# microsoft/UniVL

Measured on NVIDIA H100. Metric: video-text samples/sec, higher is better.
Workload: dtype bf16

## Files before the change

include/univl_b200.h:

```cpp
#ifndef UNIVL_B200_H_
#define UNIVL_B200_H_

#ifdef __cplusplus
extern "C" {
#endif

const char* univl_last_error_string(void);
int univl_abi_version(void);
int univl_set_reserved_sms(int n);
int univl_partials_reduce(const float* part, int nparts, long long rows, long long cols, float* dst, long long ld,
                          void* stream);

int univl_gemm_bf16(const void* A, long long lda, int a_mn_major, const void* B, long long ldb, int b_mn_major,
                    int M, int N, int Kc, void* out, long long ldo, int epilogue, const float* bias,
                    const void* aux_in, long long ld_aux_in, void* aux_out, long long ld_aux_out, float alpha,
                    int block_n, int split_k, void* stream);
int univl_gemm_plan(int M, int N, int Kc, int epilogue, int block_n, int split_k);

int univl_quantize_e4m3_rows(const void* x, long long ldx, void* q, long long ldq, float* scale, int M, int K,
                             void* stream);
int univl_quantize_e4m3_blocks(const float* w, long long ldw, void* q, long long ldq, float* scale, int N, int K,
                               void* stream);
int univl_gemm_fp8(const void* A, long long lda, const float* a_scale, const void* B, long long ldb,
                   const float* b_scale, int M, int N, int Kc, int epilogue, const float* bias, void* out,
                   long long ldo, float* out_scale, void* stream);

int univl_layernorm_fwd(const void* x, const void* res, const float* gamma, const float* beta, void* y, float* mean,
                        float* rstd, int rows, int cols, float eps, float p_drop, int drop_mode,
                        const unsigned long long* rng_state, unsigned long long stream_id, void* stream);
int univl_layernorm_bwd(const void* dy, const void* dy2, const void* x, const void* res, const float* gamma,
                        const float* mean, const float* rstd, void* dx_res, void* dx_dense, float* dgamma,
                        float* dbeta, float* dbias, int rows, int cols, float p_drop, int drop_mode,
                        const unsigned long long* rng_state, unsigned long long stream_id, void* stream);
int univl_layernorm_f32_fwd(const float* x, const float* gamma, const float* beta, void* y, float* mean, float* rstd,
                            int rows, int cols, float eps, void* stream);
int univl_layernorm_f32_bwd(const void* dy, const float* x, const float* gamma, const float* mean, const float* rstd,
                            float* dgamma, float* dbeta, int rows, int cols, void* stream);

int univl_embed_text_fwd(const long long* ids, const long long* type_ids, const float* word, const float* pos,
                         const float* type, const float* gamma, const float* beta, void* y, float* mean, float* rstd,
                         int n_seq, int S, int H, int vocab, float eps, float p_drop, const unsigned long long* rng_state,
                         unsigned long long stream_id, void* stream);
int univl_embed_text_bwd(const void* dy, const long long* ids, const long long* type_ids, const float* word,
                         const float* pos, const float* type, const float* gamma, const float* mean,
                         const float* rstd, float* dword, float* dpos, float* dtype, float* dgamma, float* dbeta,
                         int n_seq, int S, int H, int vocab, float p_drop, const unsigned long long* rng_state,
                         unsigned long long stream_id, void* stream);
int univl_embed_src_fwd(const void* a, const void* b, const float* pos, const float* type, const float* gamma,
                        const float* beta, void* y, float* mean, float* rstd, int Na, int Wa, int Nb, int Fb,
                        int all_pairs, int H, float eps, float p_drop, const unsigned long long* rng_state,
                        unsigned long long stream_id, void* stream);
int univl_embed_src_bwd(const void* dy, const void* a, const void* b, const float* pos, const float* type,
                        const float* gamma, const float* mean, const float* rstd, void* da, void* db, float* dpos,
                        float* dtype, float* dgamma, float* dbeta, int Na, int Wa, int Nb, int Fb, int all_pairs,
                        int H, float p_drop, const unsigned long long* rng_state, unsigned long long stream_id, void* stream);

int univl_attention_fwd(const void* q, long long ldq, const void* k, long long ldk, const void* v, long long ldv,
                        void* o, long long ldo, float* lse, const long long* mask_a, const long long* mask_b, int Wa,
                        int Fb, int Nb, int all_pairs, int n_seq, int heads, int Sq, int Sk, int causal, float scale,
                        float p_drop, const unsigned long long* rng_state, unsigned long long stream_id, void* stream);
int univl_attention_bwd(const void* q, long long ldq, const void* k, long long ldk, const void* v, long long ldv,
                        const void* o, long long ldo, const float* lse, const void* d_o, long long lddo, void* dq,
                        long long lddq, void* dk, long long lddk, void* dv, long long lddv, const long long* mask_a,
                        const long long* mask_b, int Wa, int Fb, int Nb, int all_pairs, int n_seq, int heads, int Sq,
                        int Sk, int causal, float scale, float p_drop, const unsigned long long* rng_state,
                        unsigned long long stream_id, int rng_layout, float* dbq, float* dbk, float* dbv, void* stream);
int univl_attention_long_fwd(const void* q, long long ldq, const void* k, long long ldk, const void* v, long long ldv,
                             void* o, long long ldo, float* lse, const long long* mask_a, const long long* mask_b,
                             int Wa, int Fb, int Nb, int all_pairs, int n_seq, int heads, int Sq, int Sk, int causal,
                             float scale, float p_drop, const unsigned long long* rng_state,
                             unsigned long long stream_id, void* stream);
int univl_attention_long_bwd(const void* q, long long ldq, const void* k, long long ldk, const void* v, long long ldv,
                             const void* o, long long ldo, const float* lse, const void* d_o, long long lddo, void* dq,
                             long long lddq, void* dk, long long lddk, void* dv, long long lddv,
                             const long long* mask_a, const long long* mask_b, int Wa, int Fb, int Nb, int all_pairs,
                             int n_seq, int heads, int Sq, int Sk, int causal, float scale, float p_drop,
                             const unsigned long long* rng_state, unsigned long long stream_id, int rng_layout,
                             float* dbq, float* dbk, float* dbv, void* stream);
int univl_attention_pair_fwd(const void* qa, long long ldqa, const void* ka, long long ldka, const void* va,
                             long long ldva, const void* qb, long long ldqb, const void* kb, long long ldkb,
                             const void* vb, long long ldvb, void* o, long long ldo, float* lse,
                             const long long* mask_a, const long long* mask_b, int Na, int Wa, int Nb, int Fb,
                             int heads, int Sq, float scale, void* stream);
int univl_fused_qkv_attention_supported(int n_seq, int heads, int S, int H);
int univl_fused_qkv_attention_fwd(const void* x, long long ldx, const void* wqkv, long long ldw, const float* bias,
                                  void* qkv_out, long long ld_qkv, void* o, long long ldo, float* lse,
                                  const long long* mask_a, const long long* mask_b, int Wa, int Fb, int Nb,
                                  int all_pairs, int n_seq, int heads, int S, int causal, float scale, float p_drop,
                                  const unsigned long long* rng_state, unsigned long long stream_id, void* stream);
int univl_fused_attention_bwd(const void* qkv, long long ld_qkv, const void* o, long long ldo, const float* lse,
                              const void* d_o, long long lddo, void* dqkv, long long ld_dqkv, float* dbias,
                              const long long* mask_a, const long long* mask_b, int Wa, int Fb, int Nb, int all_pairs,
                              int n_seq, int heads, int S, int causal, float scale, float p_drop,
                              const unsigned long long* rng_state, unsigned long long stream_id, void* stream);

int univl_colsum_bf16(const void* x, long long ld, float* out, int rows, int cols, void* stream);
int univl_cast_f32_to_bf16(const float* src, void* dst, long long n, void* stream);
int univl_cast_bf16_to_f32(const void* src, float* dst, long long n, void* stream);
int univl_multi_cast_f32_to_bf16(const unsigned long long* device_table, int n_tensors, int blocks_per_tensor,
                                 void* stream);
int univl_fill_f32(float* p, float value, long long n, void* stream);
int univl_rng_advance(unsigned long long* rng_state, void* stream);
int univl_gelu_fwd_bf16(const void* x, void* out, long long n, void* stream);
int univl_gelu_bwd_bf16(const void* dy, const void* pre, void* out, long long n, void* stream);
int univl_tanh_fwd_bf16(const void* x, void* out, long long n, void* stream);
int univl_tanh_bwd_bf16(const void* dy, const void* y, void* out, long long n, void* stream);
int univl_scale_f32(float* dst, const float* src, long long n, const float* gscale, void* stream);

int univl_meanpool_fwd(const void* x, const long long* mask, float* out, float* norm_out, int N, int S, int H,
                       int skip_first, int guard_zero, int l2norm, void* stream);
int univl_meanpool_bwd(const float* dy, const float* y, const float* norm, const long long* mask, void* dx, int N,
                       int S, int H, int skip_first, int guard_zero, int l2norm, void* stream);
int univl_sim_matmul_fwd(const float* t, const float* v, float* sim, int Bt, int Bv, int H, int groups, void* stream);
int univl_sim_matmul_bwd(const float* dsim, const float* t, const float* v, float* dt, float* dv, int Bt, int Bv,
                         int H, int groups, void* stream);
int univl_maxmargin_loss(const float* sim, float* loss, float* dsim, int B, float margin, int n_pair, float w_same,
                         float w_diff, int groups, void* stream);
int univl_crossen_loss(const float* sim, float* loss, float* dsim, int B, int groups, void* stream);
int univl_milnce_loss(const float* sim, float* loss, float* dsim, int batch_size, int n_pair, int groups,
                      void* stream);
int univl_softmax_xent_fwd(const float* logits, long long ld, const long long* labels, const long long* pair_mask,
                           float* lse, float* sum_count, float* loss, int T, int V, int target_mode,
                           long long ignore_index, int groups, void* stream);
int univl_softmax_xent_bwd(const float* logits, long long ld, const long long* labels, const long long* pair_mask,
                           const float* lse, const float* sum_count, const float* gscale, void* dlogits,
                           long long ld_d, int T, int V, int target_mode, long long ignore_index, int groups,
                           void* stream);
int univl_vocab_xent_workspace(int T, int V);
int univl_vocab_xent_fwd(const void* x, long long ldx, const void* w, long long ldw, const float* bias,
                         const long long* labels, float* lse, float* sum_count, float* loss, void* workspace,
                         long long workspace_bytes, int T, int V, int Kc, int groups, void* stream);
int univl_vocab_xent_bwd(const void* x, long long ldx, const void* w, long long ldw, const float* bias,
                         const long long* labels, const float* lse, const float* sum_count, const float* gscale,
                         void* dlogits, long long ld_d, int T, int V, int Kc, int groups, void* stream);
int univl_pooler_sim_fwd(const void* u, const float* w, const float* b, float* out, int N, int H, void* stream);
int univl_pooler_sim_bwd(const void* u, const float* w, const float* dout, void* du, float* dw, float* db, int N,
                         int H, void* stream);

int univl_bert_adam_step(float* p, const float* g, float* m, float* v, void* p_bf16, const void* segs, int n_chunks,
                         int n_tensors, float* scratch, long long* step, float b1, float b2, float eps,
                         float max_grad_norm, float global_clip_norm, float warmup, long long t_total,
                         float grad_scale, void* stream);
int univl_bert_adam_step_bf16grad(float* p, const void* g_bf16, float* m, float* v, void* p_bf16, const void* segs,
                                  int n_chunks, int n_tensors, float* scratch, long long* step, float b1, float b2,
                                  float eps, float max_grad_norm, float global_clip_norm, float warmup,
                                  long long t_total, float grad_scale, void* stream);

#ifdef __cplusplus
}
#endif
#endif
```

univl_b200/csrc/gemm_wgmma.cu:

```cuda
#include "common.cuh"
#include "fp8.cuh"
#include "pipeline.cuh"
#include "tmap.cuh"

#include <stdio.h>
#include <type_traits>

namespace univl {

enum GemmEpilogue : int {
  EPI_BIAS_BF16 = 0,
  EPI_BIAS_GELU_BF16 = 1,
  EPI_GELU_BWD_BF16 = 2,
  EPI_ADD_BF16 = 3,
  EPI_BIAS_F32 = 4,
  EPI_ATOMIC_F32 = 5,
};

struct GemmParams {
  int M, N, Kc;
  int k_blocks_per_split;
  int epilogue;
  float alpha;
  void* out;
  long long ldo;
  const float* bias;
  const bf16* aux_in;
  long long ld_aux_in;
  bf16* aux_out;
  long long ld_aux_out;
  int vec2;
  int vec8;
  float* slots;
  unsigned* arrived;
  int splits;
  int kb_seg;
};

constexpr int BLOCK_M = 128;
constexpr int BLOCK_K = 64;
constexpr int PLAN_SMS = 132;
constexpr int SPLIT_MIN_K = 4096;

template <int BLOCK_N, int STAGES>
struct GemmSmem {
  static constexpr int A_BYTES = BLOCK_M * BLOCK_K * 2;
  static constexpr int B_BYTES = BLOCK_N * BLOCK_K * 2;
  static constexpr int STAGE_BYTES = A_BYTES + B_BYTES;
  static constexpr int BAR_OFFSET = STAGES * STAGE_BYTES;
  static constexpr int TOTAL = BAR_OFFSET + 2 * STAGES * 8;
  static constexpr int DYN_BYTES = TOTAL + 1024;
  static_assert(DYN_BYTES <= 227 * 1024, "shared memory per block");
};

struct WorkItem {
  int m0, n0, kb_begin, num_kb;
};
__device__ __forceinline__ WorkItem decode_work(int w, int m_tiles, int n_tiles, int total_kb, int kb_per, int bn) {
  const int tiles = m_tiles * n_tiles;
  const int split = w / tiles;
  const int rem = w - split * tiles;
  int m_blk, n_blk;
  if (kb_per >= total_kb) {
    m_blk = rem / n_tiles;
    n_blk = rem - m_blk * n_tiles;
  } else {
    n_blk = rem / m_tiles;
    m_blk = rem - n_blk * m_tiles;
  }
  WorkItem it;
  it.m0 = m_blk * BLOCK_M;
  it.n0 = n_blk * bn;
  it.kb_begin = split * kb_per;
  it.num_kb = min(total_kb, it.kb_begin + kb_per) - it.kb_begin;
  return it;
}

__device__ __forceinline__ void epi_pair(const GemmParams& p, float alpha, int row, int col, float v0, float v1) {
  if (row >= p.M || col >= p.N) return;
  const bool two = col + 1 < p.N;
  const bool vec = two && p.vec2;
  const int epi = p.epilogue;
  v0 *= alpha;
  v1 *= alpha;
  if (p.bias != nullptr && (epi == EPI_BIAS_BF16 || epi == EPI_BIAS_GELU_BF16 || epi == EPI_BIAS_F32)) {
    v0 += __ldg(p.bias + col);
    if (two) v1 += __ldg(p.bias + col + 1);
  }
  if (epi == EPI_ATOMIC_F32 || epi == EPI_BIAS_F32) {
    float* o = reinterpret_cast<float*>(p.out) + (long long)row * p.ldo + col;
    if (epi == EPI_ATOMIC_F32) {
      if (vec) {
        float2 a = *reinterpret_cast<float2*>(o);
        *reinterpret_cast<float2*>(o) = make_float2(a.x + v0, a.y + v1);
      } else {
        o[0] += v0;
        if (two) o[1] += v1;
      }
    } else {
      if (vec) *reinterpret_cast<float2*>(o) = make_float2(v0, v1);
      else {
        o[0] = v0;
        if (two) o[1] = v1;
      }
    }
    return;
  }
  if (epi == EPI_GELU_BWD_BF16 || epi == EPI_ADD_BF16) {
    const bf16* a = p.aux_in + (long long)row * p.ld_aux_in + col;
    float x0, x1 = 0.f;
    if (vec) {
      const float2 f = unpack_bf16x2(*reinterpret_cast<const uint32_t*>(a));
      x0 = f.x;
      x1 = f.y;
    } else {
      x0 = __bfloat162float(a[0]);
      if (two) x1 = __bfloat162float(a[1]);
    }
    if (epi == EPI_GELU_BWD_BF16) {
      v0 *= gelu_erf_grad(x0);
      v1 *= gelu_erf_grad(x1);
    } else {
      v0 += x0;
      v1 += x1;
    }
  }
  if (epi == EPI_BIAS_GELU_BF16) {
    bf16* ao = p.aux_out + (long long)row * p.ld_aux_out + col;
    if (vec) *reinterpret_cast<uint32_t*>(ao) = pack_bf16x2(v0, v1);
    else {
      ao[0] = __float2bfloat16(v0);
      if (two) ao[1] = __float2bfloat16(v1);
    }
    v0 = gelu_erf(v0);
    v1 = gelu_erf(v1);
  }
  bf16* o = reinterpret_cast<bf16*>(p.out) + (long long)row * p.ldo + col;
  if (vec) *reinterpret_cast<uint32_t*>(o) = pack_bf16x2(v0, v1);
  else {
    o[0] = __float2bfloat16(v0);
    if (two) o[1] = __float2bfloat16(v1);
  }
}

constexpr int EPI_CHUNK = 8;

__device__ __forceinline__ uint4 quad_transpose(uint32_t w0, uint32_t w1, uint32_t w2, uint32_t w3, int q) {
  const bool odd = q & 1;
  uint32_t r0 = __shfl_xor_sync(0xffffffffu, odd ? w0 : w1, 1);
  uint32_t r1 = __shfl_xor_sync(0xffffffffu, odd ? w2 : w3, 1);
  if (odd) {
    w0 = r0;
    w2 = r1;
  } else {
    w1 = r0;
    w3 = r1;
  }
  const bool hi = q & 2;
  r0 = __shfl_xor_sync(0xffffffffu, hi ? w0 : w2, 2);
  r1 = __shfl_xor_sync(0xffffffffu, hi ? w1 : w3, 2);
  if (hi) {
    w0 = r0;
    w1 = r1;
  } else {
    w2 = r0;
    w3 = r1;
  }
  return make_uint4(w0, w1, w2, w3);
}

template <int EPI, bool BIAS, int BLOCK_N, bool WIDE = false>
__device__ __forceinline__ void epi_tile(const GemmParams& p, float alpha, int row, int col0,
                                         const float (&acc)[BLOCK_N / 2]) {
  constexpr int GROUPS = BLOCK_N / 8;
  constexpr int CHUNK = WIDE ? 4 : (GROUPS < EPI_CHUNK ? GROUPS : EPI_CHUNK);
  static_assert(CHUNK % 4 == 0, "a chunk holds whole quads of 8-column groups");
  constexpr bool AUX = EPI == EPI_GELU_BWD_BF16 || EPI == EPI_ADD_BF16;
  constexpr bool OUT_F32 = EPI == EPI_BIAS_F32 || EPI == EPI_ATOMIC_F32;
  static_assert(!(WIDE && OUT_F32), "16-byte stores are for the bf16 outputs");
  constexpr bool ACCUM = EPI == EPI_ATOMIC_F32;
  const int q = threadIdx.x & 3;
  const float* bias = p.bias + col0;
  const bf16* ax = p.aux_in + (long long)row * p.ld_aux_in + col0;
  const long long ax8 = 8 * p.ld_aux_in;
  bf16* ao = p.aux_out + (long long)row * p.ld_aux_out + col0;
  const long long ao8 = 8 * p.ld_aux_out;
  const long long o8 = 8 * p.ldo;
  float* of = reinterpret_cast<float*>(p.out) + (long long)row * p.ldo + col0;
  bf16* ob = reinterpret_cast<bf16*>(p.out) + (long long)row * p.ldo + col0;
  float b[2][CHUNK][2];
  uint32_t x[2][CHUNK][2];
  float2 a[2][CHUNK][2];
  auto load = [&](int j0, int s) {
#pragma unroll
    for (int j = 0; j < CHUNK; ++j) {
      const int c = (j0 + j) * 8;
      if constexpr (BIAS) {
        b[s][j][0] = __ldg(bias + c);
        b[s][j][1] = __ldg(bias + c + 1);
      }
#pragma unroll
      for (int h = 0; h < 2; ++h) {
        if constexpr (AUX) x[s][j][h] = *reinterpret_cast<const uint32_t*>(ax + h * ax8 + c);
        if constexpr (ACCUM) a[s][j][h] = *reinterpret_cast<const float2*>(of + h * o8 + c);
      }
    }
  };
  load(0, 0);
#pragma unroll
  for (int j0 = 0; j0 < GROUPS; j0 += CHUNK) {
    const int s = (j0 / CHUNK) & 1;
    if (j0 + CHUNK < GROUPS) load(j0 + CHUNK, s ^ 1);
#pragma unroll
    for (int jq = 0; jq < CHUNK; jq += 4) {
#pragma unroll
      for (int h = 0; h < 2; ++h) {
        uint32_t wo[4], wa[4];
#pragma unroll
        for (int jj = 0; jj < 4; ++jj) {
          const int j = jq + jj;
          const int c = (j0 + j) * 8;
          float v0 = __fmul_rn(acc[4 * (j0 + j) + 2 * h], alpha);
          float v1 = __fmul_rn(acc[4 * (j0 + j) + 2 * h + 1], alpha);
          if constexpr (BIAS) {
            v0 = __fadd_rn(v0, b[s][j][0]);
            v1 = __fadd_rn(v1, b[s][j][1]);
          }
          if constexpr (AUX) {
            const float2 f = unpack_bf16x2(x[s][j][h]);
            if constexpr (EPI == EPI_GELU_BWD_BF16) {
              v0 = __fmul_rn(v0, gelu_erf_grad(f.x));
              v1 = __fmul_rn(v1, gelu_erf_grad(f.y));
            } else {
              v0 = __fadd_rn(v0, f.x);
              v1 = __fadd_rn(v1, f.y);
            }
          }
          if constexpr (OUT_F32) {
            if constexpr (ACCUM) {
              v0 = __fadd_rn(a[s][j][h].x, v0);
              v1 = __fadd_rn(a[s][j][h].y, v1);
            }
            *reinterpret_cast<float2*>(of + h * o8 + c) = make_float2(v0, v1);
          } else {
            if constexpr (EPI == EPI_BIAS_GELU_BF16) {
              const uint32_t w = pack_bf16x2(v0, v1);
              if constexpr (WIDE) wa[jj] = w;
              else *reinterpret_cast<uint32_t*>(ao + h * ao8 + c) = w;
              v0 = gelu_erf(v0);
              v1 = gelu_erf(v1);
            }
            const uint32_t w = pack_bf16x2(v0, v1);
            if constexpr (WIDE) wo[jj] = w;
            else *reinterpret_cast<uint32_t*>(ob + h * o8 + c) = w;
          }
        }
        if constexpr (WIDE) {
          const int c = (j0 + jq) * 8 + 6 * q;
          if constexpr (EPI == EPI_BIAS_GELU_BF16)
            *reinterpret_cast<uint4*>(ao + h * ao8 + c) = quad_transpose(wa[0], wa[1], wa[2], wa[3], q);
          *reinterpret_cast<uint4*>(ob + h * o8 + c) = quad_transpose(wo[0], wo[1], wo[2], wo[3], q);
        }
      }
    }
  }
}

template <int BLOCK_N>
__device__ __forceinline__ void epilogue_block(const GemmParams& p, bool inside, float alpha, int n0, int row,
                                               int col0, const float (&acc)[BLOCK_N / 2]) {
  if (inside) {
    const bool bias = p.bias != nullptr;
    const bool wide = p.vec8;
    switch (p.epilogue) {
      case EPI_BIAS_BF16:
        if (wide) {
          if (bias) epi_tile<EPI_BIAS_BF16, true, BLOCK_N, true>(p, alpha, row, col0, acc);
          else epi_tile<EPI_BIAS_BF16, false, BLOCK_N, true>(p, alpha, row, col0, acc);
        } else {
          if (bias) epi_tile<EPI_BIAS_BF16, true, BLOCK_N>(p, alpha, row, col0, acc);
          else epi_tile<EPI_BIAS_BF16, false, BLOCK_N>(p, alpha, row, col0, acc);
        }
        break;
      case EPI_BIAS_GELU_BF16:
        if (wide) {
          if (bias) epi_tile<EPI_BIAS_GELU_BF16, true, BLOCK_N, true>(p, alpha, row, col0, acc);
          else epi_tile<EPI_BIAS_GELU_BF16, false, BLOCK_N, true>(p, alpha, row, col0, acc);
        } else {
          if (bias) epi_tile<EPI_BIAS_GELU_BF16, true, BLOCK_N>(p, alpha, row, col0, acc);
          else epi_tile<EPI_BIAS_GELU_BF16, false, BLOCK_N>(p, alpha, row, col0, acc);
        }
        break;
      case EPI_GELU_BWD_BF16:
        if (wide) epi_tile<EPI_GELU_BWD_BF16, false, BLOCK_N, true>(p, alpha, row, col0, acc);
        else epi_tile<EPI_GELU_BWD_BF16, false, BLOCK_N>(p, alpha, row, col0, acc);
        break;
      case EPI_ADD_BF16:
        if (wide) epi_tile<EPI_ADD_BF16, false, BLOCK_N, true>(p, alpha, row, col0, acc);
        else epi_tile<EPI_ADD_BF16, false, BLOCK_N>(p, alpha, row, col0, acc);
        break;
      case EPI_BIAS_F32:
        if (bias) epi_tile<EPI_BIAS_F32, true, BLOCK_N>(p, alpha, row, col0, acc);
        else epi_tile<EPI_BIAS_F32, false, BLOCK_N>(p, alpha, row, col0, acc);
        break;
      default:
        epi_tile<EPI_ATOMIC_F32, false, BLOCK_N>(p, alpha, row, col0, acc);
    }
  } else {
#pragma unroll
    for (int j = 0; j < BLOCK_N / 8; ++j) {
      if (n0 + j * 8 >= p.N) break;
      epi_pair(p, alpha, row, col0 + j * 8, acc[4 * j], acc[4 * j + 1]);
      epi_pair(p, alpha, row + 8, col0 + j * 8, acc[4 * j + 2], acc[4 * j + 3]);
    }
  }
}

__device__ __forceinline__ bool tile_inside(const GemmParams& p, const WorkItem& wi, int bn) {
  return p.vec2 && wi.m0 + BLOCK_M <= p.M && wi.n0 + bn <= p.N;
}

template <int BLOCK_N>
__device__ __forceinline__ bool splitk_fixup(const GemmParams& p, int tile, int half, int split, float alpha,
                                             float (&acc)[BLOCK_N / 2]) {
  constexpr int V = BLOCK_N / 8;
  constexpr int CHUNK = BLOCK_N == 256 ? 4 : 8;
  const int t = threadIdx.x & 127;
  const int lane = t & 31;
  const long long slot = 64LL * BLOCK_N;
  float4* base = reinterpret_cast<float4*>(p.slots + ((long long)tile * p.splits * 2 + half) * slot) + t;
  float4* mine = base + split * (2 * slot / 4);
#pragma unroll
  for (int j = 0; j < V; ++j) {
#pragma unroll
    for (int e = 0; e < 4; ++e) acc[4 * j + e] = __fmul_rn(acc[4 * j + e], alpha);
    __stcg(mine + j * 128, make_float4(acc[4 * j], acc[4 * j + 1], acc[4 * j + 2], acc[4 * j + 3]));
  }
  fence_acq_rel_gpu();
  __syncwarp();
  unsigned before = 0;
  if (lane == 0) before = atom_add_acq_rel_gpu(p.arrived + (tile * 2 + half) * 4 + (t >> 5), 1u);
  before = __shfl_sync(0xffffffffu, before, 0);
  if (before != (unsigned)p.splits - 1) return false;
  fence_acq_rel_gpu();
#pragma unroll
  for (int j0 = 0; j0 < V; j0 += CHUNK) {
    float4 s4[CHUNK];
#pragma unroll
    for (int j = 0; j < CHUNK; ++j) s4[j] = make_float4(0.f, 0.f, 0.f, 0.f);
    for (int s = 0; s < p.splits; ++s) {
      float4 v[CHUNK];
      if (s == split) {
#pragma unroll
        for (int j = 0; j < CHUNK; ++j) {
          const int a = 4 * (j0 + j);
          v[j] = make_float4(acc[a], acc[a + 1], acc[a + 2], acc[a + 3]);
        }
      } else {
        const float4* src = base + s * (2 * slot / 4);
#pragma unroll
        for (int j = 0; j < CHUNK; ++j) v[j] = __ldcg(src + (j0 + j) * 128);
      }
#pragma unroll
      for (int j = 0; j < CHUNK; ++j) {
        s4[j].x = __fadd_rn(s4[j].x, v[j].x);
        s4[j].y = __fadd_rn(s4[j].y, v[j].y);
        s4[j].z = __fadd_rn(s4[j].z, v[j].z);
        s4[j].w = __fadd_rn(s4[j].w, v[j].w);
      }
    }
#pragma unroll
    for (int j = 0; j < CHUNK; ++j) {
      const int a = 4 * (j0 + j);
      acc[a] = s4[j].x;
      acc[a + 1] = s4[j].y;
      acc[a + 2] = s4[j].z;
      acc[a + 3] = s4[j].w;
    }
  }
  return true;
}

template <int BLOCK_N>
__device__ __forceinline__ void finish_block(const GemmParams& p, const WorkItem& wi, int n_tiles, int kb_per,
                                             bool inside, float alpha, int half, int row, int col0,
                                             float (&acc)[BLOCK_N / 2]) {
  if (p.slots != nullptr) {
    const int tile = (wi.m0 / BLOCK_M) * n_tiles + wi.n0 / BLOCK_N;
    if (!splitk_fixup<BLOCK_N>(p, tile, half, wi.kb_begin / kb_per, alpha, acc)) return;
    alpha = 1.f;
  }
  epilogue_block<BLOCK_N>(p, inside, alpha, wi.n0, row, col0, acc);
}

constexpr int TURN_BAR = 1;

template <int BLOCK_N, int STAGES, bool A_MN, bool B_MN, int ELEM = 2>
__device__ __forceinline__ void produce_ring(const CUtensorMap* tmap_a, const CUtensorMap* tmap_b, uint8_t* smem,
                                             const Ring<STAGES>& ring, int num_work, int m_tiles, int n_tiles,
                                             int total_kb, int kb_per) {
  using L = GemmSmem<BLOCK_N, STAGES>;
  uint32_t it = 0;
  for (int w = blockIdx.x; w < num_work; w += gridDim.x) {
    const WorkItem wi = decode_work(w, m_tiles, n_tiles, total_kb, kb_per, BLOCK_N);
    for (int i = 0; i < wi.num_kb; ++i, ++it) {
      const int s = ring.acquire(it, L::STAGE_BYTES);
      uint64_t* bar = &ring.full[s];
      uint8_t* sa = smem + s * L::STAGE_BYTES;
      uint8_t* sb = sa + L::A_BYTES;
      const int k_elem = (wi.kb_begin + i) * (128 / ELEM);
      if (!A_MN) {
        tma_load_2d(sa, tmap_a, bar, k_elem, wi.m0);
      } else {
#pragma unroll
        for (int c = 0; c < BLOCK_M / 64; ++c)
          tma_load_2d(sa + c * (BLOCK_K * 128), tmap_a, bar, wi.m0 + c * 64, k_elem);
      }
      if (!B_MN) {
        tma_load_2d(sb, tmap_b, bar, k_elem, wi.n0);
      } else {
#pragma unroll
        for (int c = 0; c < BLOCK_N / 64; ++c)
          tma_load_2d(sb + c * (BLOCK_K * 128), tmap_b, bar, wi.n0 + c * 64, k_elem);
      }
    }
  }
}

template <int BLOCK_N, int STAGES, bool A_MN, bool B_MN>
__global__ void __launch_bounds__(PIPELINE_THREADS, 1)
gemm_wgmma_kernel(const __grid_constant__ CUtensorMap tmap_a, const __grid_constant__ CUtensorMap tmap_b,
                  const GemmParams p, const int num_work) {
  using L = GemmSmem<BLOCK_N, STAGES>;
  constexpr bool PING = BLOCK_N <= 128;
  constexpr bool FOLD = BLOCK_N == 64;
  Ring<STAGES> ring;
  uint8_t* smem = kernel_prologue(ring, L::BAR_OFFSET, PING ? 1 : 2, &tmap_a, &tmap_b);

  const int wg = threadIdx.x >> 7;
  const int m_tiles = (p.M + BLOCK_M - 1) / BLOCK_M;
  const int n_tiles = (p.N + BLOCK_N - 1) / BLOCK_N;
  const int total_kb = (p.Kc + BLOCK_K - 1) / BLOCK_K;
  const int kb_per = p.k_blocks_per_split;

  if (wg == 0) {
    if (producer_regs())
      produce_ring<BLOCK_N, STAGES, A_MN, B_MN>(&tmap_a, &tmap_b, smem, ring, num_work, m_tiles, n_tiles, total_kb,
                                                kb_per);
  } else if constexpr (!PING) {
    consumer_regs();
    const int c = wg - 1;
    const int t = threadIdx.x & 127;
    const int warp = t >> 5, lane = t & 31;
    uint32_t it = 0;
    for (int w = blockIdx.x; w < num_work; w += gridDim.x) {
      const WorkItem wi = decode_work(w, m_tiles, n_tiles, total_kb, kb_per, BLOCK_N);
      float acc[BLOCK_N / 2];
#pragma unroll
      for (int e = 0; e < BLOCK_N / 2; ++e) acc[e] = 0.f;
      const int last = mma_kblocks<BLOCK_N, A_MN, B_MN, L::STAGE_BYTES, L::A_BYTES>(ring, smem, c * (64 * 128), acc,
                                                                                     0, wi.num_kb, it, t == 0);
      mma_drain(ring, last, acc, t == 0);
      const int row = wi.m0 + c * 64 + warp * 16 + (lane >> 2);
      const int col0 = wi.n0 + 2 * (lane & 3);
      finish_block<BLOCK_N>(p, wi, n_tiles, kb_per, tile_inside(p, wi, BLOCK_N), p.alpha, c, row, col0, acc);
    }
  } else {
    consumer_regs();
    const int c = wg - 1;
    const int t = threadIdx.x & 127;
    const int warp = t >> 5, lane = t & 31;
    uint32_t it = 0;
    int j = 0;
    for (int w = blockIdx.x; w < num_work; w += gridDim.x, ++j) {
      const WorkItem wi = decode_work(w, m_tiles, n_tiles, total_kb, kb_per, BLOCK_N);
      if ((j & 1) != c) {
        it += wi.num_kb;
        continue;
      }
      float acc[2][BLOCK_N / 2];
#pragma unroll
      for (int e = 0; e < BLOCK_N / 2; ++e) acc[0][e] = acc[1][e] = 0.f;
      const bool fold = FOLD && p.kb_seg < wi.num_kb;
      const int seg = fold ? p.kb_seg : wi.num_kb;
      float sum[2][FOLD ? BLOCK_N / 2 : 1];
      if constexpr (FOLD) {
#pragma unroll
        for (int e = 0; e < BLOCK_N / 2; ++e) sum[0][e] = sum[1][e] = 0.f;
      }
      if (j > 0) named_bar(TURN_BAR + c, 256);
      for (int i0 = 0; i0 < wi.num_kb; i0 += seg) {
        const int i1 = min(wi.num_kb, i0 + seg);
        const int last =
            mma_kblocks<BLOCK_N, 2, A_MN, B_MN, L::STAGE_BYTES, L::A_BYTES>(ring, smem, 0, acc, i0, i1, it, t == 0);
        if (i1 == wi.num_kb && w + (int)gridDim.x < num_work)
          named_bar_arrive(TURN_BAR + (c ^ 1), 256);
        mma_drain(ring, last, acc, t == 0);
        if constexpr (FOLD) {
          if (fold) {
#pragma unroll
            for (int e = 0; e < BLOCK_N / 2; ++e) {
              sum[0][e] = __fadd_rn(sum[0][e], __fmul_rn(acc[0][e], p.alpha));
              sum[1][e] = __fadd_rn(sum[1][e], __fmul_rn(acc[1][e], p.alpha));
            }
          }
        }
      }
      float alpha = p.alpha;
      if constexpr (FOLD) {
        if (fold) {
#pragma unroll
          for (int e = 0; e < BLOCK_N / 2; ++e) {
            acc[0][e] = sum[0][e];
            acc[1][e] = sum[1][e];
          }
          alpha = 1.f;
        }
      }
      const bool inside = tile_inside(p, wi, BLOCK_N);
      const int row = wi.m0 + warp * 16 + (lane >> 2);
      const int col0 = wi.n0 + 2 * (lane & 3);
      finish_block<BLOCK_N>(p, wi, n_tiles, kb_per, inside, alpha, 0, row, col0, acc[0]);
      finish_block<BLOCK_N>(p, wi, n_tiles, kb_per, inside, alpha, 1, row + 64, col0, acc[1]);
    }
  }
}

template <int BLOCK_N, int STAGES, bool A_MN, bool B_MN>
static int launch_gemm(const CUtensorMap& ta, const CUtensorMap& tb, const GemmParams& p, int splits,
                       cudaStream_t stream) {
  using L = GemmSmem<BLOCK_N, STAGES>;
  auto kern = gemm_wgmma_kernel<BLOCK_N, STAGES, A_MN, B_MN>;
  const char* name = "univl_gemm_bf16";
  if (int rc = persistent_prepare(kern, L::DYN_BYTES, name)) return rc;
  const long long work =
      (long long)((p.M + BLOCK_M - 1) / BLOCK_M) * ((p.N + BLOCK_N - 1) / BLOCK_N) * (long long)splits;
  return persistent_launch(kern, name, work, L::DYN_BYTES, stream, ta, tb, p, (int)work);
}

template <int BLOCK_N, int STAGES>
static int dispatch_major(bool a_mn, bool b_mn, const CUtensorMap& ta, const CUtensorMap& tb, const GemmParams& p,
                          int splits, cudaStream_t stream) {
  if (!a_mn && !b_mn) return launch_gemm<BLOCK_N, STAGES, false, false>(ta, tb, p, splits, stream);
  if (!a_mn && b_mn) return launch_gemm<BLOCK_N, STAGES, false, true>(ta, tb, p, splits, stream);
  if (a_mn && b_mn) return launch_gemm<BLOCK_N, STAGES, true, true>(ta, tb, p, splits, stream);
  return launch_gemm<BLOCK_N, STAGES, true, false>(ta, tb, p, splits, stream);
}

enum Fp8Epilogue : int { FP8_EPI_BIAS_BF16 = 0, FP8_EPI_GELU_E4M3 = 1 };

struct Fp8Params {
  const float* a_scale;
  const float* b_scale;
  uint8_t* out_q;
  float* out_scale;
};

constexpr int FP8_BLOCK_N = 128;
constexpr int FP8_STAGES = 6;

template <int EPI, bool PAIRS>
__global__ void __launch_bounds__(PIPELINE_THREADS, 1)
gemm_fp8_kernel(const __grid_constant__ CUtensorMap tmap_a, const __grid_constant__ CUtensorMap tmap_b,
                const GemmParams p, const Fp8Params f, const int num_work) {
  using L = GemmSmem<FP8_BLOCK_N, FP8_STAGES>;
  Ring<FP8_STAGES> ring;
  uint8_t* smem = kernel_prologue(ring, L::BAR_OFFSET, 2, &tmap_a, &tmap_b);

  const int wg = threadIdx.x >> 7;
  const int m_tiles = (p.M + BLOCK_M - 1) / BLOCK_M;
  const int n_tiles = p.N / FP8_BLOCK_N;
  const int total_kb = p.Kc / 128;

  if (wg == 0) {
    if (producer_regs())
      produce_ring<FP8_BLOCK_N, FP8_STAGES, false, false, 1>(&tmap_a, &tmap_b, smem, ring, num_work, m_tiles, n_tiles,
                                                              total_kb, total_kb);
    return;
  }
  consumer_regs();
  const int c = wg - 1;
  const int t = threadIdx.x & 127;
  const int warp = t >> 5, lane = t & 31;
  const int M = p.M;
  uint32_t it = 0;
  for (int w = blockIdx.x; w < num_work; w += gridDim.x) {
    const WorkItem wi = decode_work(w, m_tiles, n_tiles, total_kb, total_kb, FP8_BLOCK_N);
    const int row = wi.m0 + c * 64 + warp * 16 + (lane >> 2);
    const bool in0 = row < M, in1 = row + 8 < M;
    const float* sa = f.a_scale + row;
    const float* sb = f.b_scale + (long long)(wi.n0 / FP8_BLOCK_N) * total_kb;
    float acc[FP8_BLOCK_N / 2];
#pragma unroll
    for (int e = 0; e < FP8_BLOCK_N / 2; ++e) acc[e] = 0.f;
    auto issue = [&](float (&tmp)[FP8_BLOCK_N / 2], int kb) {
      const int s = ring.wait(it + kb);
      const uint32_t a_s = smem_u32(smem + s * L::STAGE_BYTES) + c * (64 * 128);
      const uint32_t b_s = smem_u32(smem + s * L::STAGE_BYTES) + L::A_BYTES;
      wgmma_fence();
      fence_regs(tmp);
#pragma unroll
      for (int k = 0; k < 4; ++k)
        WgmmaSSE4M3N128::mma(tmp, make_smem_desc_sw128(a_s + k * 32, 16, 1024),
                             make_smem_desc_sw128(b_s + k * 32, 16, 1024), k > 0 ? 1 : 0);
      wgmma_commit();
      fence_regs(tmp);
    };
    auto promote = [&](auto newer, float (&tmp)[FP8_BLOCK_N / 2], int kb) {
      const float bs = __ldg(sb + kb);
      const float s0 = in0 ? __ldg(sa + (long long)kb * M) : 0.f;
      const float s1 = in1 ? __ldg(sa + (long long)kb * M + 8) : 0.f;
      wgmma_wait<decltype(newer)::value>();
      fence_regs(tmp);
      if (t == 0) ring.release(ring.stage(it + kb));
      const float f0 = s0 * bs, f1 = s1 * bs;
#pragma unroll
      for (int j = 0; j < FP8_BLOCK_N / 8; ++j) {
        acc[4 * j] = __fmaf_rn(tmp[4 * j], f0, acc[4 * j]);
        acc[4 * j + 1] = __fmaf_rn(tmp[4 * j + 1], f0, acc[4 * j + 1]);
        acc[4 * j + 2] = __fmaf_rn(tmp[4 * j + 2], f1, acc[4 * j + 2]);
        acc[4 * j + 3] = __fmaf_rn(tmp[4 * j + 3], f1, acc[4 * j + 3]);
      }
    };
    using One = std::integral_constant<int, 1>;
    using None = std::integral_constant<int, 0>;
    float ta[FP8_BLOCK_N / 2];
    if constexpr (PAIRS) {
      float tb[FP8_BLOCK_N / 2];
      issue(ta, 0);
      issue(tb, 1);
      int kb = 0;
      for (; kb + 2 < total_kb; kb += 2) {
        promote(One(), ta, kb);
        issue(ta, kb + 2);
        promote(One(), tb, kb + 1);
        issue(tb, kb + 3);
      }
      promote(One(), ta, kb);
      promote(None(), tb, kb + 1);
    } else {
      for (int kb = 0; kb < total_kb; ++kb) {
        issue(ta, kb);
        promote(None(), ta, kb);
      }
    }
    it += total_kb;
    const int col0 = wi.n0 + 2 * (lane & 3);
    if constexpr (EPI == FP8_EPI_BIAS_BF16) {
      if (tile_inside(p, wi, FP8_BLOCK_N)) {
        if (p.vec8) epi_tile<EPI_BIAS_BF16, true, FP8_BLOCK_N, true>(p, p.alpha, row, col0, acc);
        else epi_tile<EPI_BIAS_BF16, true, FP8_BLOCK_N>(p, p.alpha, row, col0, acc);
      } else {
#pragma unroll
        for (int j = 0; j < FP8_BLOCK_N / 8; ++j) {
          epi_pair(p, p.alpha, row, col0 + j * 8, acc[4 * j], acc[4 * j + 1]);
          epi_pair(p, p.alpha, row + 8, col0 + j * 8, acc[4 * j + 2], acc[4 * j + 3]);
        }
      }
    } else {
      const float* bias = p.bias + col0;
#pragma unroll
      for (int h = 0; h < 2; ++h) {
        float amax = 0.f;
#pragma unroll
        for (int j = 0; j < FP8_BLOCK_N / 8; ++j) {
          const float v0 = gelu_erf(__fadd_rn(acc[4 * j + 2 * h], __ldg(bias + 8 * j)));
          const float v1 = gelu_erf(__fadd_rn(acc[4 * j + 2 * h + 1], __ldg(bias + 8 * j + 1)));
          acc[4 * j + 2 * h] = v0;
          acc[4 * j + 2 * h + 1] = v1;
          amax = fmaxf(amax, fmaxf(fabsf(v0), fabsf(v1)));
        }
        amax = fmaxf(amax, __shfl_xor_sync(0xffffffffu, amax, 1));
        amax = fmaxf(amax, __shfl_xor_sync(0xffffffffu, amax, 2));
        const float sc = e4m3_scale(amax);
        const float inv = e4m3_inv_scale(sc);
        const int r = row + 8 * h;
        if (r < M) {
          uint8_t* q = f.out_q + (long long)r * p.ldo + col0;
#pragma unroll
          for (int j = 0; j < FP8_BLOCK_N / 8; ++j)
            *reinterpret_cast<uint16_t*>(q + 8 * j) =
                e4m3x2(__fmul_rn(acc[4 * j + 2 * h], inv), __fmul_rn(acc[4 * j + 2 * h + 1], inv));
          if ((lane & 3) == 0) f.out_scale[(long long)(wi.n0 / FP8_BLOCK_N) * M + r] = sc;
        }
      }
    }
  }
}

template <int EPI, bool PAIRS>
static int launch_gemm_fp8(const CUtensorMap& ta, const CUtensorMap& tb, const GemmParams& p, const Fp8Params& f,
                           cudaStream_t stream) {
  using L = GemmSmem<FP8_BLOCK_N, FP8_STAGES>;
  auto kern = gemm_fp8_kernel<EPI, PAIRS>;
  const char* name = "univl_gemm_fp8";
  if (int rc = persistent_prepare(kern, L::DYN_BYTES, name)) return rc;
  const long long work = (long long)((p.M + BLOCK_M - 1) / BLOCK_M) * (p.N / FP8_BLOCK_N);
  return persistent_launch(kern, name, work, L::DYN_BYTES, stream, ta, tb, p, f, (int)work);
}

constexpr int VX_BLOCK_N = 128;
constexpr int VX_STAGES = 6;

struct VocabXentParams {
  int T, V, Kc;
  int m_tiles, n_tiles, chunks, chunk_tiles;
  const float* bias;
  const long long* labels;
  float4* part;
  const float* lse;
  const float* count;
  const float* gscale;
  int rows_per_group, groups;
  bf16* dl;
  long long ld_d;
};

template <bool BWD>
__global__ void __launch_bounds__(PIPELINE_THREADS, 1)
vocab_xent_kernel(const __grid_constant__ CUtensorMap tmap_a, const __grid_constant__ CUtensorMap tmap_b,
                  const VocabXentParams p, const int num_work) {
  using L = GemmSmem<VX_BLOCK_N, VX_STAGES>;
  Ring<VX_STAGES> ring;
  uint8_t* smem = kernel_prologue(ring, L::BAR_OFFSET, 2, &tmap_a, &tmap_b);
  const int wg = threadIdx.x >> 7;
  const int total_kb = (p.Kc + BLOCK_K - 1) / BLOCK_K;

  if (wg == 0) {
    if (!producer_regs()) return;
    uint32_t it = 0;
    for (int w = blockIdx.x; w < num_work; w += gridDim.x) {
      const int chunk = w / p.m_tiles;
      const int m0 = (w - chunk * p.m_tiles) * BLOCK_M;
      const int nt1 = min(p.n_tiles, (chunk + 1) * p.chunk_tiles);
      for (int nt = chunk * p.chunk_tiles; nt < nt1; ++nt) {
        for (int kb = 0; kb < total_kb; ++kb, ++it) {
          const int s = ring.acquire(it, L::STAGE_BYTES);
          uint8_t* sa = smem + s * L::STAGE_BYTES;
          tma_load_2d(sa, &tmap_a, &ring.full[s], kb * BLOCK_K, m0);
          tma_load_2d(sa + L::A_BYTES, &tmap_b, &ring.full[s], kb * BLOCK_K, nt * VX_BLOCK_N);
        }
      }
    }
    return;
  }
  consumer_regs();
  const int c = wg - 1;
  const int t = threadIdx.x & 127;
  const int warp = t >> 5, lane = t & 31, q = lane & 3;
  uint32_t it = 0;
  for (int w = blockIdx.x; w < num_work; w += gridDim.x) {
    const int chunk = w / p.m_tiles;
    const int row = (w - chunk * p.m_tiles) * BLOCK_M + c * 64 + warp * 16 + (lane >> 2);
    long long lab[2];
    float m[2], s[2], xt[2], lse[2], g[2];
#pragma unroll
    for (int h = 0; h < 2; ++h) {
      const int r = row + 8 * h;
      lab[h] = r < p.T ? __ldg(p.labels + r) : -1;
      m[h] = -INFINITY;
      s[h] = 0.f;
      xt[h] = 0.f;
      if constexpr (BWD) {
        lse[h] = 0.f;
        g[h] = 0.f;
        if (lab[h] != -1) {
          lse[h] = __ldg(p.lse + r);
          g[h] = ((p.gscale ? __ldg(p.gscale) : 1.f) / (float)p.groups) / __ldg(p.count + r / p.rows_per_group);
        }
      }
    }
    const int nt1 = min(p.n_tiles, (chunk + 1) * p.chunk_tiles);
    for (int nt = chunk * p.chunk_tiles; nt < nt1; ++nt) {
      float acc[VX_BLOCK_N / 2];
#pragma unroll
      for (int e = 0; e < VX_BLOCK_N / 2; ++e) acc[e] = 0.f;
      const int last = mma_kblocks<VX_BLOCK_N, false, false, L::STAGE_BYTES, L::A_BYTES>(ring, smem, c * (64 * 128),
                                                                                          acc, 0, total_kb, it, t == 0);
      mma_drain(ring, last, acc, t == 0);

      const int col0 = nt * VX_BLOCK_N + 2 * q;
#pragma unroll
      for (int j = 0; j < VX_BLOCK_N / 8; ++j) {
#pragma unroll
        for (int e = 0; e < 2; ++e) {
          const int col = col0 + 8 * j + e;
          const float b = (p.bias != nullptr && col < p.V) ? __ldg(p.bias + col) : 0.f;
          acc[4 * j + e] = __fadd_rn(acc[4 * j + e], b);
          acc[4 * j + 2 + e] = __fadd_rn(acc[4 * j + 2 + e], b);
        }
      }
      if constexpr (!BWD) {
#pragma unroll
        for (int h = 0; h < 2; ++h) {
          float tm = -INFINITY;
#pragma unroll
          for (int j = 0; j < VX_BLOCK_N / 8; ++j)
#pragma unroll
            for (int e = 0; e < 2; ++e)
              if (col0 + 8 * j + e < p.V) tm = fmaxf(tm, acc[4 * j + 2 * h + e]);
          if (tm > m[h]) {
            s[h] = s[h] * __expf(m[h] - tm);
            m[h] = tm;
          }
#pragma unroll
          for (int j = 0; j < VX_BLOCK_N / 8; ++j)
#pragma unroll
            for (int e = 0; e < 2; ++e) {
              const int col = col0 + 8 * j + e;
              const float v = acc[4 * j + 2 * h + e];
              if (col < p.V) s[h] += __expf(v - m[h]);
              if (col == lab[h]) xt[h] = v;
            }
        }
      } else {
        const int ncol = min(p.ld_d - (long long)nt * VX_BLOCK_N, (long long)VX_BLOCK_N);
#pragma unroll
        for (int h = 0; h < 2; ++h) {
          const int r = row + 8 * h;
          if (r >= p.T) continue;
          bf16* drow = p.dl + (long long)r * p.ld_d + col0;
          const bool scored = lab[h] != -1;
#pragma unroll
          for (int j = 0; j < VX_BLOCK_N / 8; ++j) {
            if (8 * j + 2 * q >= ncol) break;
            float d[2];
#pragma unroll
            for (int e = 0; e < 2; ++e) {
              const int col = col0 + 8 * j + e;
              d[e] = 0.f;
              if (scored && col < p.V)
                d[e] = (__expf(acc[4 * j + 2 * h + e] - lse[h]) - (col == lab[h] ? 1.f : 0.f)) * g[h];
            }
            *reinterpret_cast<uint32_t*>(drow + 8 * j) = pack_bf16x2(d[0], d[1]);
          }
        }
      }
    }
    if constexpr (!BWD) {
#pragma unroll
      for (int h = 0; h < 2; ++h) {
#pragma unroll
        for (int o = 1; o <= 2; o <<= 1) {
          const float mo = __shfl_xor_sync(0xffffffffu, m[h], o);
          const float so = __shfl_xor_sync(0xffffffffu, s[h], o);
          const float xo = __shfl_xor_sync(0xffffffffu, xt[h], o);
          const float mx = fmaxf(m[h], mo);
          const float a = m[h] == -INFINITY ? 0.f : s[h] * __expf(m[h] - mx);
          const float b = mo == -INFINITY ? 0.f : so * __expf(mo - mx);
          m[h] = mx;
          s[h] = a + b;
          xt[h] += xo;
        }
        const int r = row + 8 * h;
        if (q == 0 && r < p.T) p.part[(long long)r * p.chunks + chunk] = make_float4(m[h], s[h], xt[h], 0.f);
      }
    }
  }
}

__global__ void __launch_bounds__(256)
vocab_xent_rows_kernel(const float4* __restrict__ part, const long long* __restrict__ labels, int T, int V, int chunks,
                       int chunk_cols, float* __restrict__ lse_out, float* __restrict__ nll) {
  const int r = blockIdx.x * blockDim.x + threadIdx.x;
  if (r >= T) return;
  const long long lab = labels[r];
  if (lab == -1) {
    lse_out[r] = 0.f;
    return;
  }
  const float4* pr = part + (long long)r * chunks;
  float4 f = pr[0];
  float m = f.x, s = f.y;
  for (int k = 1; k < chunks; ++k) {
    f = pr[k];
    const float mx = fmaxf(m, f.x);
    s = s * __expf(m - mx) + f.y * __expf(f.x - mx);
    m = mx;
  }
  const float lse = m + __logf(s);
  lse_out[r] = lse;
  nll[r] = (lab >= 0 && lab < V) ? lse - pr[lab / chunk_cols].z : __int_as_float(0x7fc00000);
}

constexpr int VX_GROUP_THREADS = 512;
__global__ void __launch_bounds__(VX_GROUP_THREADS)
vocab_xent_group_kernel(const float* __restrict__ nll, const long long* __restrict__ labels, int rows_per_group,
                        float* __restrict__ sum_count, int groups) {
  __shared__ float red[2][VX_GROUP_THREADS];
  const int grp = blockIdx.x;
  float sum = 0.f, cnt = 0.f;
  for (int i = threadIdx.x; i < rows_per_group; i += VX_GROUP_THREADS) {
    const long long r = (long long)grp * rows_per_group + i;
    if (labels[r] == -1) continue;
    sum += nll[r];
    cnt += 1.f;
  }
  red[0][threadIdx.x] = sum;
  red[1][threadIdx.x] = cnt;
  __syncthreads();
  for (int o = VX_GROUP_THREADS / 2; o > 0; o >>= 1) {
    if (threadIdx.x < o) {
      red[0][threadIdx.x] += red[0][threadIdx.x + o];
      red[1][threadIdx.x] += red[1][threadIdx.x + o];
    }
    __syncthreads();
  }
  if (threadIdx.x == 0) {
    sum_count[grp] = red[0][0];
    sum_count[groups + grp] = red[1][0];
  }
}

__global__ void vocab_xent_mean_kernel(const float* __restrict__ sum_count, int groups, float* __restrict__ out) {
  float acc = sum_count[0] / sum_count[groups];
  for (int g = 1; g < groups; ++g) acc += sum_count[g] / sum_count[groups + g];
  *out = groups > 1 ? acc / (float)groups : acc;
}

template <bool BWD>
static int launch_vocab_xent(const CUtensorMap& ta, const CUtensorMap& tb, const VocabXentParams& p,
                             cudaStream_t stream) {
  const long long work = (long long)p.m_tiles * p.chunks;
  return persistent_launch(vocab_xent_kernel<BWD>, BWD ? "univl_vocab_xent_bwd" : "univl_vocab_xent_fwd", work,
                           GemmSmem<VX_BLOCK_N, VX_STAGES>::DYN_BYTES, stream, ta, tb, p, (int)work);
}

}

using namespace univl;

namespace {
struct GemmPlan {
  int bn, splits, kb_per, kb_seg;
};
int plan_gemm(int M, int N, int Kc, int epilogue, int block_n, int split_k, GemmPlan* plan) {
  const int total_kb = (Kc + BLOCK_K - 1) / BLOCK_K;
  const int m_tiles = (M + BLOCK_M - 1) / BLOCK_M;
  int bn = block_n;
  if (bn == 0) {
    bn = 256;
    if (epilogue != EPI_ATOMIC_F32) {
      const auto tiles = [&](int w) { return (long long)m_tiles * ((N + w - 1) / w); };
      if (tiles(256) < 2 * PLAN_SMS) bn = 128;
      if (tiles(128) < PLAN_SMS) bn = 64;
    }
    if (N <= 64) bn = 64;
    else if (N <= 128 && bn > 128) bn = 128;
  }
  UNIVL_CHECK_ARG(bn == 64 || bn == 128 || bn == 256, "gemm: block_n must be 64/128/256");
  const int n_tiles = (N + bn - 1) / bn;
  int splits = 1;
  if (epilogue == EPI_ATOMIC_F32) {
    splits = split_k;
    if (splits == 0) {
      const long long tiles = (long long)m_tiles * n_tiles;
      splits = (int)((2 * PLAN_SMS + tiles - 1) / tiles);
      if (splits > total_kb / 2) splits = total_kb / 2;
      if (splits < 1) splits = 1;
    }
    if (splits > total_kb) splits = total_kb;
  }
  int kb_per = (total_kb + splits - 1) / splits;
  splits = (total_kb + kb_per - 1) / kb_per;
  int kb_seg = kb_per;
  if (epilogue == EPI_ATOMIC_F32 && block_n == 0 && split_k == 0 && Kc < SPLIT_MIN_K && splits > 1) {
    bn = 64;
    splits = 1;
    kb_per = total_kb;
  }
  plan->bn = bn; plan->splits = splits; plan->kb_per = kb_per; plan->kb_seg = kb_seg;
  return UNIVL_OK;
}

GemmParams gemm_params(int M, int N, int Kc, int kb_per, int epilogue, float alpha, void* out, long long ldo,
                       const float* bias, const void* aux_in, long long ld_aux_in, void* aux_out,
                       long long ld_aux_out) {
  GemmParams p;
  p.M = M; p.N = N; p.Kc = Kc;
  p.k_blocks_per_split = kb_per;
  p.epilogue = epilogue;
  p.alpha = alpha;
  p.out = out; p.ldo = ldo;
  p.bias = bias;
  p.aux_in = reinterpret_cast<const bf16*>(aux_in); p.ld_aux_in = ld_aux_in;
  p.aux_out = reinterpret_cast<bf16*>(aux_out); p.ld_aux_out = ld_aux_out;
  const bool out_f32 = epilogue == EPI_BIAS_F32 || epilogue == EPI_ATOMIC_F32;
  bool vec2 = ((uintptr_t)out % (out_f32 ? 8 : 4)) == 0 && (ldo % 2) == 0;
  if (aux_in != nullptr) vec2 = vec2 && ((uintptr_t)aux_in % 4) == 0 && (ld_aux_in % 2) == 0;
  if (aux_out != nullptr) vec2 = vec2 && ((uintptr_t)aux_out % 4) == 0 && (ld_aux_out % 2) == 0;
  p.vec2 = vec2 ? 1 : 0;
  bool vec8 = !out_f32 && ((uintptr_t)out % 16) == 0 && (ldo % 8) == 0;
  if (aux_out != nullptr) vec8 = vec8 && ((uintptr_t)aux_out % 16) == 0 && (ld_aux_out % 8) == 0;
  p.vec8 = vec8 ? 1 : 0;
  p.slots = nullptr;
  p.arrived = nullptr;
  p.splits = 1;
  p.kb_seg = kb_per;
  return p;
}
}

extern "C" int univl_gemm_plan(int M, int N, int Kc, int epilogue, int block_n, int split_k) {
  GemmPlan plan;
  if (int rc = plan_gemm(M, N, Kc, epilogue, block_n, split_k, &plan)) return rc;
  return 1;
}

extern "C" int univl_gemm_bf16(const void* A, long long lda, int a_mn_major, const void* B, long long ldb,
                               int b_mn_major, int M, int N, int Kc, void* out, long long ldo, int epilogue,
                               const float* bias, const void* aux_in, long long ld_aux_in, void* aux_out,
                               long long ld_aux_out, float alpha, int block_n, int split_k, void* stream_) {
  cudaStream_t stream = reinterpret_cast<cudaStream_t>(stream_);
  UNIVL_CHECK_ARG(M > 0 && N > 0 && Kc > 0, "gemm: empty problem M=%d N=%d K=%d", M, N, Kc);
  UNIVL_CHECK_ARG(A && B && out, "gemm: null operand");
  UNIVL_CHECK_ARG((lda % 8) == 0 && (ldb % 8) == 0, "gemm: lda/ldb must be multiples of 8 elements (got %lld, %lld)",
                  lda, ldb);
  UNIVL_CHECK_ARG(((uintptr_t)A & 15) == 0 && ((uintptr_t)B & 15) == 0, "gemm: operands must be 16-byte aligned");
  UNIVL_CHECK_ARG(epilogue >= 0 && epilogue <= 5, "gemm: unknown epilogue %d", epilogue);
  if (epilogue == EPI_GELU_BWD_BF16 || epilogue == EPI_ADD_BF16)
    UNIVL_CHECK_ARG(aux_in != nullptr, "gemm: epilogue %d needs aux_in", epilogue);
  if (epilogue == EPI_BIAS_GELU_BF16) UNIVL_CHECK_ARG(aux_out != nullptr, "gemm: gelu epilogue needs aux_out");
  UNIVL_CHECK_ARG(split_k >= 0, "gemm: bad split_k");
  if (epilogue != EPI_ATOMIC_F32) UNIVL_CHECK_ARG(split_k <= 1, "gemm: split_k>1 needs the atomic epilogue");

  GemmPlan plan;
  if (int prc = plan_gemm(M, N, Kc, epilogue, block_n, split_k, &plan)) return prc;
  const int bn = plan.bn;

  CUtensorMap ta, tb;
  int rc;
  if (!a_mn_major) rc = make_tmap(&ta, A, M, Kc, lda, BLOCK_M);
  else             rc = make_tmap(&ta, A, Kc, M, lda, BLOCK_K);
  if (rc) return rc;
  if (!b_mn_major) rc = make_tmap(&tb, B, N, Kc, ldb, bn);
  else             rc = make_tmap(&tb, B, Kc, N, ldb, BLOCK_K);
  if (rc) return rc;

  GemmParams p = gemm_params(M, N, Kc, plan.kb_per, epilogue, alpha, out, ldo, bias, aux_in, ld_aux_in, aux_out,
                             ld_aux_out);
  p.splits = plan.splits;
  p.kb_seg = plan.kb_seg;
  if (plan.splits > 1) {
    const long long tiles = (long long)((M + BLOCK_M - 1) / BLOCK_M) * ((N + bn - 1) / bn);
    const size_t slot_bytes = (size_t)tiles * plan.splits * BLOCK_M * bn * sizeof(float);
    const size_t counter_bytes = (size_t)tiles * 8 * sizeof(unsigned);
    if ((rc = scratch_alloc((void**)&p.slots, slot_bytes + counter_bytes, stream))) return rc;
    p.arrived = reinterpret_cast<unsigned*>(p.slots + slot_bytes / sizeof(float));
    const cudaError_t e = cudaMemsetAsync(p.arrived, 0, counter_bytes, stream);
    if (e != cudaSuccess) {
      cudaFreeAsync(p.slots, stream);
      return set_error(UNIVL_ERR_CUDA, "gemm split-K counters: %s", cudaGetErrorString(e));
    }
  }

  const bool amn = a_mn_major != 0, bmn = b_mn_major != 0;
  if (bn == 256) rc = dispatch_major<256, 4>(amn, bmn, ta, tb, p, plan.splits, stream);
  else if (bn == 128) rc = dispatch_major<128, 6>(amn, bmn, ta, tb, p, plan.splits, stream);
  else rc = dispatch_major<64, 8>(amn, bmn, ta, tb, p, plan.splits, stream);
  if (p.slots != nullptr) cudaFreeAsync(p.slots, stream);
  return rc;
}

extern "C" int univl_gemm_fp8(const void* A, long long lda, const float* a_scale, const void* B, long long ldb,
                              const float* b_scale, int M, int N, int Kc, int epilogue, const float* bias, void* out,
                              long long ldo, float* out_scale, void* stream_) {
  cudaStream_t stream = reinterpret_cast<cudaStream_t>(stream_);
  UNIVL_CHECK_ARG(M > 0 && N > 0 && Kc > 0, "univl_gemm_fp8: empty problem M=%d N=%d K=%d", M, N, Kc);
  UNIVL_CHECK_ARG(Kc % 128 == 0, "univl_gemm_fp8: K=%d must be a multiple of 128 (one scale per 128 columns)", Kc);
  UNIVL_CHECK_ARG(N % 128 == 0, "univl_gemm_fp8: N=%d must be a multiple of 128 (one scale per 128 x 128 block)", N);
  UNIVL_CHECK_ARG(epilogue == FP8_EPI_BIAS_BF16 || epilogue == FP8_EPI_GELU_E4M3,
                  "univl_gemm_fp8: unknown epilogue %d", epilogue);
  UNIVL_CHECK_ARG(A && B && a_scale && b_scale && bias && out, "univl_gemm_fp8: null operand, scale, bias or output");
  UNIVL_CHECK_ARG(lda >= Kc && ldb >= Kc && (lda % 16) == 0 && (ldb % 16) == 0,
                  "univl_gemm_fp8: lda/ldb must be >= K and multiples of 16 (got %lld, %lld, K=%d)", lda, ldb, Kc);
  UNIVL_CHECK_ARG(((uintptr_t)A & 15) == 0 && ((uintptr_t)B & 15) == 0,
                  "univl_gemm_fp8: A and B must be 16-byte aligned");
  UNIVL_CHECK_ARG(ldo >= N, "univl_gemm_fp8: ldo=%lld must be >= N=%d", ldo, N);
  if (epilogue == FP8_EPI_GELU_E4M3) {
    UNIVL_CHECK_ARG(out_scale != nullptr, "univl_gemm_fp8: the GELU epilogue needs out_scale");
    UNIVL_CHECK_ARG(((uintptr_t)out & 15) == 0 && (ldo % 16) == 0,
                    "univl_gemm_fp8: the e4m3 output must be 16-byte aligned with ldo a multiple of 16 (got %lld)",
                    ldo);
  }

  CUtensorMap ta, tb;
  int rc;
  if ((rc = make_tmap(&ta, A, M, Kc, lda, BLOCK_M, true))) return rc;
  if ((rc = make_tmap(&tb, B, N, Kc, ldb, FP8_BLOCK_N, true))) return rc;

  const GemmParams p = gemm_params(M, N, Kc, Kc / 128, EPI_BIAS_BF16, 1.f, out, ldo, bias, nullptr, 0, nullptr, 0);
  Fp8Params f;
  f.a_scale = a_scale;
  f.b_scale = b_scale;
  f.out_q = reinterpret_cast<uint8_t*>(out);
  f.out_scale = out_scale;
  const bool pairs = (Kc / 128) % 2 == 0;
  if (epilogue == FP8_EPI_BIAS_BF16)
    return pairs ? launch_gemm_fp8<FP8_EPI_BIAS_BF16, true>(ta, tb, p, f, stream)
                 : launch_gemm_fp8<FP8_EPI_BIAS_BF16, false>(ta, tb, p, f, stream);
  return pairs ? launch_gemm_fp8<FP8_EPI_GELU_E4M3, true>(ta, tb, p, f, stream)
               : launch_gemm_fp8<FP8_EPI_GELU_E4M3, false>(ta, tb, p, f, stream);
}

namespace {
constexpr int VX_MIN_CHUNK_TILES = 8;
struct VxPlan {
  int m_tiles, n_tiles, chunks, chunk_tiles;
};
VxPlan vx_plan(int T, int V) {
  VxPlan pl;
  pl.m_tiles = (T + BLOCK_M - 1) / BLOCK_M;
  pl.n_tiles = (V + VX_BLOCK_N - 1) / VX_BLOCK_N;
  long long best = -1;
  for (int c = 1; c <= pl.n_tiles; ++c) {
    const int ct = (pl.n_tiles + c - 1) / c;
    if (ct < VX_MIN_CHUNK_TILES && c > 1) break;
    if (c > 1 && ct == (pl.n_tiles + c - 2) / (c - 1)) continue;
    const int chunks = (pl.n_tiles + ct - 1) / ct;
    const long long rounds = ((long long)pl.m_tiles * chunks + PLAN_SMS - 1) / PLAN_SMS;
    if (best < 0 || rounds * ct < best) {
      best = rounds * ct;
      pl.chunks = chunks;
      pl.chunk_tiles = ct;
    }
  }
  return pl;
}

int vx_check(const char* name, const void* x, long long ldx, const void* w, long long ldw, const long long* labels,
             int T, int V, int Kc, int groups) {
  UNIVL_CHECK_ARG(T > 0 && V > 0 && Kc > 0, "%s: empty problem T=%d V=%d K=%d", name, T, V, Kc);
  UNIVL_CHECK_ARG(x && w && labels, "%s: null x, W or labels", name);
  UNIVL_CHECK_ARG(ldx >= Kc && ldw >= Kc && (ldx % 8) == 0 && (ldw % 8) == 0,
                  "%s: ldx/ldw must be >= K and multiples of 8 (got %lld, %lld, K=%d)", name, ldx, ldw, Kc);
  UNIVL_CHECK_ARG(((uintptr_t)x & 15) == 0 && ((uintptr_t)w & 15) == 0, "%s: x and W must be 16-byte aligned", name);
  UNIVL_CHECK_ARG(groups > 0 && T % groups == 0, "%s: %d groups must divide T=%d", name, groups, T);
  return UNIVL_OK;
}

template <bool BWD>
int vx_params(const void* x, long long ldx, const void* w, long long ldw, int T, int V, int Kc, CUtensorMap* ta,
              CUtensorMap* tb, VocabXentParams* p) {
  if (int rc = persistent_prepare(vocab_xent_kernel<BWD>, GemmSmem<VX_BLOCK_N, VX_STAGES>::DYN_BYTES,
                                  BWD ? "univl_vocab_xent_bwd" : "univl_vocab_xent_fwd"))
    return rc;
  const VxPlan pl = vx_plan(T, V);
  int rc;
  if ((rc = make_tmap(ta, x, T, Kc, ldx, BLOCK_M))) return rc;
  if ((rc = make_tmap(tb, w, V, Kc, ldw, VX_BLOCK_N))) return rc;
  *p = VocabXentParams{};
  p->T = T; p->V = V; p->Kc = Kc;
  p->m_tiles = pl.m_tiles; p->n_tiles = pl.n_tiles; p->chunks = pl.chunks; p->chunk_tiles = pl.chunk_tiles;
  return UNIVL_OK;
}


long long vx_workspace_bytes(int T, int V) {
  return (long long)T * vx_plan(T, V).chunks * (long long)sizeof(float4) + ((long long)T * 4 + 15) / 16 * 16;
}
}

extern "C" int univl_vocab_xent_workspace(int T, int V) {
  UNIVL_CHECK_ARG(T > 0 && V > 0, "univl_vocab_xent_workspace: empty problem T=%d V=%d", T, V);
  const long long bytes = vx_workspace_bytes(T, V);
  UNIVL_CHECK_ARG(bytes <= 0x7fffffffLL, "univl_vocab_xent_workspace: T=%d V=%d needs over 2 GiB", T, V);
  return (int)bytes;
}

extern "C" int univl_vocab_xent_fwd(const void* x, long long ldx, const void* w, long long ldw, const float* bias,
                                    const long long* labels, float* lse, float* sum_count, float* loss,
                                    void* workspace, long long workspace_bytes, int T, int V, int Kc, int groups,
                                    void* stream_) {
  const char* name = "univl_vocab_xent_fwd";
  if (int rc = vx_check(name, x, ldx, w, ldw, labels, T, V, Kc, groups)) return rc;
  UNIVL_CHECK_ARG(lse && sum_count && loss && workspace, "%s: null lse, sum_count, loss or workspace", name);
  UNIVL_CHECK_ARG(((uintptr_t)workspace & 15) == 0, "%s: the workspace must be 16-byte aligned", name);
  const long long need = vx_workspace_bytes(T, V);
  UNIVL_CHECK_ARG(workspace_bytes >= need, "%s: workspace of %lld bytes, needs %lld (univl_vocab_xent_workspace)",
                  name, workspace_bytes, need);
  cudaStream_t stream = reinterpret_cast<cudaStream_t>(stream_);
  CUtensorMap ta, tb;
  VocabXentParams p;
  if (int rc = vx_params<false>(x, ldx, w, ldw, T, V, Kc, &ta, &tb, &p)) return rc;
  p.bias = bias;
  p.labels = labels;
  p.part = reinterpret_cast<float4*>(workspace);
  if (int rc = launch_vocab_xent<false>(ta, tb, p, stream)) return rc;
  float* nll = reinterpret_cast<float*>(p.part + (long long)T * p.chunks);
  vocab_xent_rows_kernel<<<(T + 255) / 256, 256, 0, stream>>>(p.part, labels, T, V, p.chunks,
                                                               p.chunk_tiles * VX_BLOCK_N, lse, nll);
  vocab_xent_group_kernel<<<groups, VX_GROUP_THREADS, 0, stream>>>(nll, labels, T / groups, sum_count, groups);
  vocab_xent_mean_kernel<<<1, 1, 0, stream>>>(sum_count, groups, loss);
  UNIVL_CHECK_LAUNCH(name);
  return UNIVL_OK;
}

extern "C" int univl_vocab_xent_bwd(const void* x, long long ldx, const void* w, long long ldw, const float* bias,
                                    const long long* labels, const float* lse, const float* sum_count,
                                    const float* gscale, void* dlogits, long long ld_d, int T, int V, int Kc,
                                    int groups, void* stream_) {
  const char* name = "univl_vocab_xent_bwd";
  if (int rc = vx_check(name, x, ldx, w, ldw, labels, T, V, Kc, groups)) return rc;
  UNIVL_CHECK_ARG(lse && sum_count && dlogits, "%s: null lse, sum_count or dlogits", name);
  const long long cols = (long long)vx_plan(T, V).n_tiles * VX_BLOCK_N;
  UNIVL_CHECK_ARG(ld_d >= V && ld_d <= cols && (ld_d % 2) == 0 && ((uintptr_t)dlogits & 3) == 0,
                  "%s: ld_d=%lld must be even, >= V=%d and <= V rounded up to 128, with dlogits 4-byte aligned", name,
                  ld_d, V);
  cudaStream_t stream = reinterpret_cast<cudaStream_t>(stream_);
  CUtensorMap ta, tb;
  VocabXentParams p;
  if (int rc = vx_params<true>(x, ldx, w, ldw, T, V, Kc, &ta, &tb, &p)) return rc;
  p.bias = bias;
  p.labels = labels;
  p.lse = lse;
  p.count = sum_count + groups;
  p.gscale = gscale;
  p.rows_per_group = T / groups;
  p.groups = groups;
  p.dl = reinterpret_cast<bf16*>(dlogits);
  p.ld_d = ld_d;
  return launch_vocab_xent<true>(ta, tb, p, stream);
}
```

univl_b200/csrc/layernorm.cu:

```cuda
#include "common.cuh"

namespace univl {

constexpr int LN_WARPS = 8;
constexpr int LN_MAX_VEC = 4;

__device__ __forceinline__ void load8(const bf16* p, float (&v)[8]) {
  const uint4 u = *reinterpret_cast<const uint4*>(p);
  const uint32_t w[4] = {u.x, u.y, u.z, u.w};
#pragma unroll
  for (int j = 0; j < 4; ++j) {
    const float2 f = unpack_bf16x2(w[j]);
    v[2 * j] = f.x;
    v[2 * j + 1] = f.y;
  }
}
__device__ __forceinline__ void load8(const float* p, float (&v)[8]) {
  const float4 a = *reinterpret_cast<const float4*>(p);
  const float4 b = *reinterpret_cast<const float4*>(p + 4);
  v[0] = a.x; v[1] = a.y; v[2] = a.z; v[3] = a.w;
  v[4] = b.x; v[5] = b.y; v[6] = b.z; v[7] = b.w;
}
template <typename T> struct Raw8;
template <> struct Raw8<bf16> { uint4 u; };
template <> struct Raw8<float> { float4 a, b; };
__device__ __forceinline__ void raw_load(const bf16* p, Raw8<bf16>& r) {
  asm volatile("ld.global.nc.L1::no_allocate.v4.u32 {%0, %1, %2, %3}, [%4];"
               : "=r"(r.u.x), "=r"(r.u.y), "=r"(r.u.z), "=r"(r.u.w) : "l"(p));
}
__device__ __forceinline__ void raw_load(const float* p, Raw8<float>& r) {
  r.a = __ldg(reinterpret_cast<const float4*>(p));
  r.b = __ldg(reinterpret_cast<const float4*>(p + 4));
}
__device__ __forceinline__ void raw_unpack(const Raw8<bf16>& r, float (&v)[8]) {
  const uint32_t w[4] = {r.u.x, r.u.y, r.u.z, r.u.w};
#pragma unroll
  for (int j = 0; j < 4; ++j) {
    const float2 f = unpack_bf16x2(w[j]);
    v[2 * j] = f.x;
    v[2 * j + 1] = f.y;
  }
}
__device__ __forceinline__ void raw_unpack(const Raw8<float>& r, float (&v)[8]) {
  v[0] = r.a.x; v[1] = r.a.y; v[2] = r.a.z; v[3] = r.a.w;
  v[4] = r.b.x; v[5] = r.b.y; v[6] = r.b.z; v[7] = r.b.w;
}
__device__ __forceinline__ void store8(bf16* p, const float (&v)[8]) {
  uint4 u;
  u.x = pack_bf16x2(v[0], v[1]);
  u.y = pack_bf16x2(v[2], v[3]);
  u.z = pack_bf16x2(v[4], v[5]);
  u.w = pack_bf16x2(v[6], v[7]);
  *reinterpret_cast<uint4*>(p) = u;
}

struct DropCfg {
  int mode;
  uint32_t threshold;
  float scale;
  uint64_t seed, stream;
  const unsigned long long* rng;
};
__device__ __forceinline__ DropCfg resolve_drop(DropCfg d) {
  if (d.mode != 0 && d.rng != nullptr) {
    d.seed = d.rng[0];
    d.stream += d.rng[1] << 20;
  }
  return d;
}

__device__ __forceinline__ uint32_t keep8_mask(const DropCfg& d, uint64_t idx0) {
  return dropout_keep8(d.seed, d.stream, idx0, d.threshold);
}

template <typename TIn, int NVEC>
__global__ void __launch_bounds__(LN_WARPS * 32, NVEC <= 3 ? 3 : 2)
layernorm_fwd_kernel(const TIn* __restrict__ x, const bf16* __restrict__ res, const float* __restrict__ gamma,
                     const float* __restrict__ beta, bf16* __restrict__ y, float* __restrict__ mean_out,
                     float* __restrict__ rstd_out, int rows, float eps, DropCfg drop_in) {
  pdl_trigger();
  pdl_wait();
  const DropCfg drop = resolve_drop(drop_in);
  constexpr int cols = NVEC * 256;
  const int warp = threadIdx.x >> 5, lane = threadIdx.x & 31;
  const float inv_cols = 1.0f / (float)cols;
  const long long stride = (long long)gridDim.x * LN_WARPS;
  long long row = (long long)blockIdx.x * LN_WARPS + warp;
  Raw8<TIn> nx[NVEC];
  Raw8<bf16> nr[NVEC];
  if (row < rows) {
#pragma unroll
    for (int i = 0; i < NVEC; ++i) {
      const long long off = row * cols + (i * 32 + lane) * 8;
      raw_load(x + off, nx[i]);
      if (res != nullptr) raw_load(res + off, nr[i]);
    }
  }
  for (; row < rows; row += stride) {
    float z[NVEC][8];
    float s = 0.f;
#pragma unroll
    for (int i = 0; i < NVEC; ++i) {
      const int c = (i * 32 + lane) * 8;
      raw_unpack(nx[i], z[i]);
      if (drop.mode == 1) {
        const uint32_t keep = keep8_mask(drop, (uint64_t)row * cols + c);
#pragma unroll
        for (int j = 0; j < 8; ++j) z[i][j] = ((keep >> j) & 1u) ? z[i][j] * drop.scale : 0.f;
      }
      if (res != nullptr) {
        float r[8];
        raw_unpack(nr[i], r);
#pragma unroll
        for (int j = 0; j < 8; ++j) z[i][j] += r[j];
      }
#pragma unroll
      for (int j = 0; j < 8; ++j) s += z[i][j];
    }
    const long long next = row + stride;
    if (next < rows) {
#pragma unroll
      for (int i = 0; i < NVEC; ++i) {
        const long long off = next * cols + (i * 32 + lane) * 8;
        raw_load(x + off, nx[i]);
        if (res != nullptr) raw_load(res + off, nr[i]);
      }
    }
    const float mean = warp_sum(s) * inv_cols;
    float q = 0.f;
#pragma unroll
    for (int i = 0; i < NVEC; ++i)
#pragma unroll
      for (int j = 0; j < 8; ++j) {
        const float d = z[i][j] - mean;
        q += d * d;
      }
    const float var = warp_sum(q) * inv_cols;
    const float rstd = 1.0f / sqrtf(var + eps);
    if (lane == 0) {
      if (mean_out) mean_out[row] = mean;
      if (rstd_out) rstd_out[row] = rstd;
    }
#pragma unroll
    for (int i = 0; i < NVEC; ++i) {
      const int c = (i * 32 + lane) * 8;
      float g[8], b[8], o[8];
      load8(gamma + c, g);
      load8(beta + c, b);
#pragma unroll
      for (int j = 0; j < 8; ++j) o[j] = g[j] * ((z[i][j] - mean) * rstd) + b[j];
      if (drop.mode == 2) {
        const uint32_t keep = keep8_mask(drop, (uint64_t)row * cols + c);
#pragma unroll
        for (int j = 0; j < 8; ++j) o[j] = ((keep >> j) & 1u) ? o[j] * drop.scale : 0.f;
      }
      store8(y + row * cols + c, o);
    }
  }
}

template <typename TIn>
static void launch_ln_fwd(int grid, cudaStream_t st, const TIn* x, const bf16* res, const float* gamma,
                          const float* beta, bf16* y, float* mean, float* rstd, int rows, int cols, float eps,
                          DropCfg drop) {
  const dim3 g(grid), b(LN_WARPS * 32);
  switch (cols >> 8) {
    case 1: launch_kernel(layernorm_fwd_kernel<TIn, 1>, g, b, 0, st, x, res, gamma, beta, y, mean, rstd, rows, eps, drop); break;
    case 2: launch_kernel(layernorm_fwd_kernel<TIn, 2>, g, b, 0, st, x, res, gamma, beta, y, mean, rstd, rows, eps, drop); break;
    case 3: launch_kernel(layernorm_fwd_kernel<TIn, 3>, g, b, 0, st, x, res, gamma, beta, y, mean, rstd, rows, eps, drop); break;
    default: launch_kernel(layernorm_fwd_kernel<TIn, 4>, g, b, 0, st, x, res, gamma, beta, y, mean, rstd, rows, eps, drop); break;
  }
}


template <typename TIn>
__device__ __forceinline__ void ln_bwd_load(const bf16* dy, const bf16* dy2, const TIn* x, const bf16* res,
                                            long long off, const DropCfg& drop, float (&z)[8], float (&d)[8],
                                            uint32_t& keep) {
  load8(x + off, z);
  keep = 0xffu;
  if (drop.mode != 0) keep = keep8_mask(drop, (uint64_t)off);
  if (drop.mode == 1) {
#pragma unroll
    for (int j = 0; j < 8; ++j) z[j] = ((keep >> j) & 1u) ? z[j] * drop.scale : 0.f;
  }
  if (res != nullptr) {
    float r[8];
    load8(res + off, r);
#pragma unroll
    for (int j = 0; j < 8; ++j) z[j] += r[j];
  }
  load8(dy + off, d);
  if (dy2 != nullptr) {
    float d2[8];
    load8(dy2 + off, d2);
#pragma unroll
    for (int j = 0; j < 8; ++j) d[j] += d2[j];
  }
  if (drop.mode == 2) {
#pragma unroll
    for (int j = 0; j < 8; ++j) d[j] = ((keep >> j) & 1u) ? d[j] * drop.scale : 0.f;
  }
}

constexpr int LNB_WARPS = 4;
__device__ __forceinline__ void acc8_add(float* p, const float (&v)[8]) {
  float4 a = *reinterpret_cast<float4*>(p), b = *reinterpret_cast<float4*>(p + 4);
  a.x += v[0]; a.y += v[1]; a.z += v[2]; a.w += v[3];
  b.x += v[4]; b.y += v[5]; b.z += v[6]; b.w += v[7];
  *reinterpret_cast<float4*>(p) = a;
  *reinterpret_cast<float4*>(p + 4) = b;
}
template <typename TIn, int NVEC>
__global__ void __launch_bounds__(LNB_WARPS * 32, NVEC <= 3 ? 5 : 3)
layernorm_bwd_kernel(const bf16* __restrict__ dy, const bf16* __restrict__ dy2, const TIn* __restrict__ x,
                     const bf16* __restrict__ res, const float* __restrict__ gamma, const float* __restrict__ mean_in,
                     const float* __restrict__ rstd_in, bf16* __restrict__ dx_res, bf16* __restrict__ dx_dense,
                     float* __restrict__ dgamma, float* __restrict__ dbeta, float* __restrict__ dbias, int rows,
                     DropCfg drop_in) {
  pdl_trigger();
  pdl_wait();
  const DropCfg drop = resolve_drop(drop_in);
  extern __shared__ __align__(16) float lnb_acc[];
  constexpr int cols = NVEC * 256;
  const int warp = threadIdx.x >> 5, lane = threadIdx.x & 31;
  const float inv_cols = 1.0f / (float)cols;
  const bool emit = dx_res != nullptr || dx_dense != nullptr || dbias != nullptr;
  float* my = lnb_acc + warp * 3 * cols;
  for (int k = lane * 4; k < 3 * cols; k += 128) *reinterpret_cast<float4*>(my + k) = make_float4(0.f, 0.f, 0.f, 0.f);
  __syncwarp();

  for (long long row = (long long)blockIdx.x * LNB_WARPS + warp; row < rows; row += (long long)gridDim.x * LNB_WARPS) {
    const float mean = mean_in[row], rstd = rstd_in[row];
    const float nm = -mean * rstd;
    float xh[NVEC][8], g[NVEC][8];
    uint32_t keep[NVEC];
    float s1 = 0.f, s2 = 0.f;
#pragma unroll
    for (int i = 0; i < NVEC; ++i) {
      const int c = (i * 32 + lane) * 8;
      float d[8], gm[8], dh[8];
      ln_bwd_load(dy, dy2, x, res, row * cols + c, drop, xh[i], d, keep[i]);
      load8(gamma + c, gm);
#pragma unroll
      for (int j = 0; j < 8; ++j) {
        const float h = fmaf(xh[i][j], rstd, nm);
        const float gg = d[j] * gm[j];
        s1 += gg;
        s2 = fmaf(gg, h, s2);
        dh[j] = d[j] * h;
        xh[i][j] = h;
        g[i][j] = gg;
      }
      acc8_add(my + c, dh);
      acc8_add(my + cols + c, d);
    }
    if (!emit) continue;
    s1 = warp_sum(s1);
    s2 = warp_sum(s2);
    const float a = -s1 * inv_cols * rstd, b = -s2 * inv_cols * rstd;
#pragma unroll
    for (int i = 0; i < NVEC; ++i) {
      const int c = (i * 32 + lane) * 8;
      float dz[8], dd[8];
#pragma unroll
      for (int j = 0; j < 8; ++j) {
        dz[j] = fmaf(xh[i][j], b, fmaf(g[i][j], rstd, a));
        dd[j] = (drop.mode == 1) ? (((keep[i] >> j) & 1u) ? dz[j] * drop.scale : 0.f) : dz[j];
      }
      if (dbias != nullptr) acc8_add(my + 2 * cols + c, dd);
      if (dx_res != nullptr) store8(dx_res + row * cols + c, dz);
      if (dx_dense != nullptr && dx_dense != dx_res) store8(dx_dense + row * cols + c, dd);
    }
  }
  __syncthreads();
  for (int which = 0; which < 3; ++which) {
    float* dst = which == 0 ? dgamma : which == 1 ? dbeta : dbias;
    if (dst == nullptr) continue;
    for (int e = threadIdx.x; e < cols; e += LNB_WARPS * 32) {
      float t = 0.f;
#pragma unroll
      for (int w = 0; w < LNB_WARPS; ++w) t += lnb_acc[(w * 3 + which) * cols + e];
      dst[(long long)blockIdx.x * cols + e] = t;
    }
  }
}

template <typename TIn>
static int launch_ln_bwd(int grid, cudaStream_t st, const bf16* dy, const bf16* dy2, const TIn* x, const bf16* res,
                         const float* gamma, const float* mean, const float* rstd, bf16* dx_res, bf16* dx_dense,
                         float* dgamma_out, float* dbeta_out, float* dbias_out, int rows, int cols, DropCfg drop) {
  const size_t smem = (size_t)LNB_WARPS * 3 * cols * sizeof(float);
  float* outs[3] = {dgamma_out, dbeta_out, dbias_out};
  float* parts[3] = {nullptr, nullptr, nullptr};
  for (int w = 0; w < 3; ++w)
    if (outs[w] != nullptr)
      if (int rc = scratch_alloc((void**)&parts[w], (size_t)grid * cols * sizeof(float), st)) return rc;
  float *dgamma = parts[0], *dbeta = parts[1], *dbias = parts[2];
  switch (cols >> 8) {
    case 1: launch_kernel(layernorm_bwd_kernel<TIn, 1>, dim3(grid), dim3(LNB_WARPS * 32), smem, st, dy, dy2, x, res, gamma, mean, rstd, dx_res, dx_dense, dgamma, dbeta, dbias, rows, drop); break;
    case 2: launch_kernel(layernorm_bwd_kernel<TIn, 2>, dim3(grid), dim3(LNB_WARPS * 32), smem, st, dy, dy2, x, res, gamma, mean, rstd, dx_res, dx_dense, dgamma, dbeta, dbias, rows, drop); break;
    case 3: launch_kernel(layernorm_bwd_kernel<TIn, 3>, dim3(grid), dim3(LNB_WARPS * 32), smem, st, dy, dy2, x, res, gamma, mean, rstd, dx_res, dx_dense, dgamma, dbeta, dbias, rows, drop); break;
    default: launch_kernel(layernorm_bwd_kernel<TIn, 4>, dim3(grid), dim3(LNB_WARPS * 32), smem, st, dy, dy2, x, res, gamma, mean, rstd, dx_res, dx_dense, dgamma, dbeta, dbias, rows, drop); break;
  }
  UNIVL_CHECK_LAUNCH("layernorm_bwd");
  for (int w = 0; w < 3; ++w)
    if (parts[w] != nullptr)
      if (int rc = partials_reduce(parts[w], grid, 1, cols, outs[w], cols, st)) return rc;
  return UNIVL_OK;
}

static int check_ln_shape(const char* what, int rows, int cols) {
  UNIVL_CHECK_ARG(rows >= 0 && cols > 0 && (cols % 256) == 0 && cols <= 256 * LN_MAX_VEC,
                  "%s: cols must be a multiple of 256 and <= %d (got rows=%d cols=%d)", what, 256 * LN_MAX_VEC, rows,
                  cols);
  return UNIVL_OK;
}

static DropCfg make_drop(int mode, float p, const unsigned long long* rng, unsigned long long stream) {
  DropCfg d;
  d.mode = (p > 0.f) ? mode : 0;
  d.threshold = dropout_threshold16(p);
  d.scale = (p > 0.f) ? 1.0f / (1.0f - p) : 1.0f;
  d.seed = 0;
  d.stream = stream;
  d.rng = rng;
  return d;
}

static int lnb_grid(int rows) {
  long long blocks = ((long long)rows + LNB_WARPS - 1) / LNB_WARPS;
  const long long cap = (long long)device_sms() * 5;
  return (int)(blocks < 1 ? 1 : (blocks > cap ? cap : blocks));
}
static int ln_grid(int rows) {
  long long blocks = ((long long)rows + LN_WARPS - 1) / LN_WARPS;
  const long long cap = (long long)device_sms() * 8;
  return (int)(blocks < 1 ? 1 : (blocks > cap ? cap : blocks));
}

}

using namespace univl;

extern "C" int univl_layernorm_fwd(const void* x, const void* res, const float* gamma, const float* beta, void* y,
                                   float* mean, float* rstd, int rows, int cols, float eps, float p_drop,
                                   int drop_mode, const unsigned long long* rng_state,
                                   unsigned long long stream_id, void* stream) {
  if (int rc = check_ln_shape("layernorm_fwd", rows, cols)) return rc;
  UNIVL_CHECK_ARG(x && gamma && beta && y, "layernorm_fwd: null pointer");
  UNIVL_CHECK_ARG(p_drop == 0.f || rng_state != nullptr, "layernorm_fwd: dropout needs rng_state");
  UNIVL_CHECK_ARG(p_drop >= 0.f && p_drop < 1.f && drop_mode >= 0 && drop_mode <= 2, "layernorm_fwd: bad dropout");
  if (rows == 0) return UNIVL_OK;
  launch_ln_fwd<bf16>(ln_grid(rows), (cudaStream_t)stream, (const bf16*)x, (const bf16*)res, gamma, beta, (bf16*)y, mean,
                      rstd, rows, cols, eps, make_drop(drop_mode, p_drop, rng_state, stream_id));
  UNIVL_CHECK_LAUNCH("layernorm_fwd");
  return UNIVL_OK;
}

extern "C" int univl_layernorm_bwd(const void* dy, const void* dy2, const void* x, const void* res,
                                   const float* gamma, const float* mean, const float* rstd, void* dx_res,
                                   void* dx_dense, float* dgamma, float* dbeta, float* dbias, int rows, int cols,
                                   float p_drop, int drop_mode, const unsigned long long* rng_state,
                                   unsigned long long stream_id, void* stream) {
  if (int rc = check_ln_shape("layernorm_bwd", rows, cols)) return rc;
  UNIVL_CHECK_ARG(dy && x && gamma && mean && rstd, "layernorm_bwd: null pointer");
  UNIVL_CHECK_ARG(p_drop == 0.f || rng_state != nullptr, "layernorm_bwd: dropout needs rng_state");
  UNIVL_CHECK_ARG(p_drop >= 0.f && p_drop < 1.f && drop_mode >= 0 && drop_mode <= 2, "layernorm_bwd: bad dropout");
  if (rows == 0) return UNIVL_OK;
  return launch_ln_bwd<bf16>(lnb_grid(rows), (cudaStream_t)stream, (const bf16*)dy, (const bf16*)dy2, (const bf16*)x,
                             (const bf16*)res, gamma, mean, rstd, (bf16*)dx_res, (bf16*)dx_dense, dgamma, dbeta, dbias,
                             rows, cols, make_drop(drop_mode, p_drop, rng_state, stream_id));
}

extern "C" int univl_layernorm_f32_fwd(const float* x, const float* gamma, const float* beta, void* y, float* mean,
                                       float* rstd, int rows, int cols, float eps, void* stream) {
  if (int rc = check_ln_shape("layernorm_f32_fwd", rows, cols)) return rc;
  UNIVL_CHECK_ARG(x && gamma && beta && y, "layernorm_f32_fwd: null pointer");
  if (rows == 0) return UNIVL_OK;
  launch_ln_fwd<float>(ln_grid(rows), (cudaStream_t)stream, x, (const bf16*)nullptr, gamma, beta, (bf16*)y, mean, rstd,
                       rows, cols, eps, make_drop(0, 0.f, nullptr, 0));
  UNIVL_CHECK_LAUNCH("layernorm_f32_fwd");
  return UNIVL_OK;
}

extern "C" int univl_layernorm_f32_bwd(const void* dy, const float* x, const float* gamma, const float* mean,
                                       const float* rstd, float* dgamma, float* dbeta, int rows, int cols,
                                       void* stream) {
  if (int rc = check_ln_shape("layernorm_f32_bwd", rows, cols)) return rc;
  UNIVL_CHECK_ARG(dy && x && gamma && mean && rstd && dgamma && dbeta, "layernorm_f32_bwd: null pointer");
  if (rows == 0) return UNIVL_OK;
  return launch_ln_bwd<float>(lnb_grid(rows), (cudaStream_t)stream, (const bf16*)dy, nullptr, x, nullptr, gamma, mean,
                              rstd, nullptr, nullptr, dgamma, dbeta, nullptr, rows, cols, make_drop(0, 0.f, nullptr, 0));
}
```

univl_b200/modules/transformer.py:

```python
import torch
from torch import nn

from .. import ops
from .until_module import LayerNorm


def check_config(config):
    if config.hidden_size != 768 or config.num_attention_heads != 12 or config.intermediate_size % 256 != 0:
        raise ValueError("univl_b200 kernels are specialised for hidden_size 768 / 12 heads of 64 (got %d / %d)"
                         % (config.hidden_size, config.num_attention_heads))
    if config.hidden_size % config.num_attention_heads != 0:
        raise ValueError("The hidden size (%d) is not a multiple of the number of attention heads (%d)"
                         % (config.hidden_size, config.num_attention_heads))
    act = config.hidden_act
    if not (isinstance(act, str) and act == "gelu"):
        raise ValueError("univl_b200 fuses erf-GELU into the FFN GEMM: hidden_act must be 'gelu' (got %r)" % (act,))


class SelfAttentionParams(nn.Module):

    def __init__(self, config):
        super(SelfAttentionParams, self).__init__()
        check_config(config)
        self.num_attention_heads = config.num_attention_heads
        self.attention_head_size = config.hidden_size // config.num_attention_heads
        self.all_head_size = config.hidden_size
        self.query = nn.Linear(config.hidden_size, self.all_head_size)
        self.key = nn.Linear(config.hidden_size, self.all_head_size)
        self.value = nn.Linear(config.hidden_size, self.all_head_size)
        self.dropout = nn.Dropout(config.attention_probs_dropout_prob)

    def _qkv_modules(self):
        return self.query, self.key, self.value


class DenseNormParams(nn.Module):

    def __init__(self, in_features, config):
        super(DenseNormParams, self).__init__()
        self.dense = nn.Linear(in_features, config.hidden_size)
        self.LayerNorm = LayerNorm(config.hidden_size, eps=1e-12)
        self.dropout = nn.Dropout(config.hidden_dropout_prob)


class IntermediateParams(nn.Module):

    def __init__(self, config):
        super(IntermediateParams, self).__init__()
        self.dense = nn.Linear(config.hidden_size, config.intermediate_size)


class AttentionParams(nn.Module):

    def __init__(self, config):
        super(AttentionParams, self).__init__()
        self.self = SelfAttentionParams(config)
        self.output = DenseNormParams(config.hidden_size, config)


def attention_param_list(self_mod, out_mod):
    return (self_mod.query.weight, self_mod.query.bias, self_mod.key.weight, self_mod.key.bias,
            self_mod.value.weight, self_mod.value.bias, out_mod.dense.weight, out_mod.dense.bias,
            out_mod.LayerNorm.weight, out_mod.LayerNorm.bias)


def ffn_param_list(intermediate, output):
    return (intermediate.dense.weight, intermediate.dense.bias, output.dense.weight, output.dense.bias,
            output.LayerNorm.weight, output.LayerNorm.bias)


class EncoderLayer(nn.Module):

    def __init__(self, config):
        super(EncoderLayer, self).__init__()
        self.attention = AttentionParams(config)
        self.intermediate = IntermediateParams(config)
        self.output = DenseNormParams(config.intermediate_size, config)
        self.p_hidden = config.hidden_dropout_prob
        self.p_attn = config.attention_probs_dropout_prob

    def run(self, x2d, n_seq, S, mask):
        params = attention_param_list(self.attention.self, self.attention.output) + \
            ffn_param_list(self.intermediate, self.output)
        return ops.EncoderLayerFn.apply(x2d, n_seq, S, mask, self.attention.output.dropout.p,
                                        self.attention.self.dropout.p, self.training, *params)


def _layer_params(layer):
    return attention_param_list(layer.attention.self, layer.attention.output) + \
        ffn_param_list(layer.intermediate, layer.output)


class EncoderStack(nn.Module):

    def __init__(self, config):
        super(EncoderStack, self).__init__()
        self.layer = nn.ModuleList([EncoderLayer(config) for _ in range(config.num_hidden_layers)])

    def run(self, x2d, n_seq, S, mask, keep_all=False):
        outs = []
        cuts = self.__dict__.get("_cut_layers")
        for i, layer in enumerate(self.layer):
            if cuts and i in cuts and x2d.requires_grad:
                leaf = x2d.detach().requires_grad_(True)
                self.__dict__.setdefault("_cut_pairs", []).append((i, x2d, leaf))
                x2d = leaf
            x2d = layer.run(x2d, n_seq, S, mask)
            if keep_all:
                outs.append(x2d)
        return outs if keep_all else x2d

    def run_first_token(self, x2d, n_seq, S, mask, start=0):
        for layer in self.layer[start:-1]:
            x2d = layer.run(x2d, n_seq, S, mask)
        last = self.layer[-1]
        return ops.EncoderLayerClsFn.apply(x2d, n_seq, S, mask, last.attention.output.dropout.p,
                                           last.attention.self.dropout.p, last.training, *_layer_params(last))


class Pooler(nn.Module):

    def __init__(self, config):
        super(Pooler, self).__init__()
        self.dense = nn.Linear(config.hidden_size, config.hidden_size)
        self.activation = nn.Tanh()

    def pre_activation(self, h2d, n_seq, S):
        first = h2d.view(n_seq, S, -1)[:, 0]
        return ops.LinearFn.apply(first, self.dense.weight, self.dense.bias, False, True)

    def run(self, h2d, n_seq, S):
        return ops.TanhFn.apply(self.pre_activation(h2d, n_seq, S))


class HeadTransform(nn.Module):

    def __init__(self, config):
        super(HeadTransform, self).__init__()
        self.dense = nn.Linear(config.hidden_size, config.hidden_size)
        self.LayerNorm = LayerNorm(config.hidden_size, eps=1e-12)

    def run(self, x2d):
        t = ops.LinearFn.apply(x2d, self.dense.weight, self.dense.bias, True, True)
        return ops.LayerNormFn.apply(t, self.LayerNorm.weight, self.LayerNorm.bias)


def as_rows(t3d):
    n, s, h = t3d.shape
    return t3d.to(torch.bfloat16).contiguous().view(n * s, h)


def hidden_list(outs, n_seq, S):
    return [o.view(n_seq, S, -1) for o in outs]
```

univl_b200/ops.py:

```python
import math
import os

import torch

from . import lib
from . import runtime as rt
from .runtime import call, ptr

BF16 = torch.bfloat16
F32 = torch.float32
LN_EPS = 1e-12
HEADS = 12
LD_VOCAB_ALIGN = 64

EPI_BIAS, EPI_GELU, EPI_GELU_BWD, EPI_ADD, EPI_F32, EPI_ATOMIC = 0, 1, 2, 3, 4, 5


def _empty(shape, dtype, like):
    return torch.empty(shape, dtype=dtype, device=like.device)


def _zeros(shape, dtype, like):
    return torch.zeros(shape, dtype=dtype, device=like.device)


def _check2d(t, name):
    if t.dim() != 2 or t.stride(1) != 1:
        raise RuntimeError("univl_b200: %s must be a row-major 2-D tensor (got shape %s strides %s)"
                           % (name, tuple(t.shape), t.stride()))


class GradSink:

    def __init__(self):
        self.flat = rt.current_sink()

    def one(self, param):
        if param is None:
            return None, None
        if self.flat is not None and self.flat.has(param):
            return self.flat.grad_view(param), None
        t = torch.zeros(param.shape, dtype=F32, device=param.device)
        return t, t

    def packed(self, params):
        if self.flat is not None and all(self.flat.has(p) for p in params):
            v = self.flat.grad_view_packed(params)
            if v is not None:
                return v, [None] * len(params)
        rows = sum(p.shape[0] for p in params)
        t = torch.zeros((rows,) + tuple(params[0].shape[1:]), dtype=F32, device=params[0].device)
        outs, r = [], 0
        for p in params:
            outs.append(t[r:r + p.shape[0]])
            r += p.shape[0]
        return t, outs


def gemm(a, b, M, N, K, out, epi=EPI_BIAS, bias=None, aux_in=None, aux_out=None, a_mn=False, b_mn=False, alpha=1.0,
         block_n=0, split_k=0):
    _check2d(a, "gemm A"); _check2d(b, "gemm B"); _check2d(out, "gemm out")
    call("univl_gemm_bf16", a.data_ptr(), a.stride(0), int(a_mn), b.data_ptr(), b.stride(0), int(b_mn), M, N, K,
         out.data_ptr(), out.stride(0), epi, ptr(bias), ptr(aux_in), aux_in.stride(0) if aux_in is not None else 0,
         ptr(aux_out), aux_out.stride(0) if aux_out is not None else 0, float(alpha), block_n, split_k)
    return out


def linear_fwd(x, w16, bias, epi=EPI_BIAS, aux_out=None, out_dtype=BF16, ld_out=None):
    T, K = x.shape
    N = w16.shape[0]
    if ld_out is None:
        out = _empty((T, N), out_dtype, x)
    else:
        out = _empty((T, ld_out), out_dtype, x)[:, :N]
    return gemm(x, w16, T, N, K, out, epi=epi, bias=bias, aux_out=aux_out)


def linear_dgrad(dy, w16, epi=EPI_BIAS, aux_in=None):
    T, N = dy.shape
    K = w16.shape[1]
    out = _empty((T, K), BF16, dy)
    return gemm(dy, w16, T, K, N, out, epi=epi, aux_in=aux_in, b_mn=True)


def linear_wgrad(dy, x, dw=None):
    T, N = dy.shape
    K = x.shape[1]
    if dw is None:
        dw = _zeros((N, K), F32, dy)
    return gemm(dy, x, N, K, T, dw, epi=EPI_ATOMIC, a_mn=True, b_mn=True)


def colsum(x, out=None):
    rows, cols = x.shape
    if out is None:
        out = _zeros((cols,), F32, x)
    call("univl_colsum_bf16", x.data_ptr(), x.stride(0), out.data_ptr(), rows, cols)
    return out


def layernorm_fwd(x, res, gamma, beta, p=0.0, mode=0, seed=0, stream=0):
    rows, cols = x.shape
    y = _empty((rows, cols), BF16, x)
    mean = _empty((rows,), F32, x)
    rstd = _empty((rows,), F32, x)
    call("univl_layernorm_fwd", x.data_ptr(), ptr(res), gamma.data_ptr(), beta.data_ptr(), y.data_ptr(),
         mean.data_ptr(), rstd.data_ptr(), rows, cols, LN_EPS, float(p), mode, seed, stream)
    return y, mean, rstd


def layernorm_bwd(dy, dy2, x, res, gamma, mean, rstd, p=0.0, mode=0, seed=0, stream=0, want_dbias=True,
                  want_dx=True, dgamma=None, dbeta=None, dbias=None):
    rows, cols = x.shape
    dx_res = _empty((rows, cols), BF16, x) if want_dx else None
    dx_dense = _empty((rows, cols), BF16, x) if (want_dx and p > 0.0 and mode == 1) else dx_res
    dgamma = _zeros((cols,), F32, x) if dgamma is None else dgamma
    dbeta = _zeros((cols,), F32, x) if dbeta is None else dbeta
    if dbias is None and want_dbias:
        dbias = _zeros((cols,), F32, x)
    call("univl_layernorm_bwd", dy.data_ptr(), ptr(dy2), x.data_ptr(), ptr(res), gamma.data_ptr(), mean.data_ptr(),
         rstd.data_ptr(), ptr(dx_res), ptr(dx_dense), dgamma.data_ptr(), dbeta.data_ptr(), ptr(dbias), rows, cols,
         float(p), mode, seed, stream)
    return dx_res, dx_dense, dgamma, dbeta, dbias


class MaskSpec:

    def __init__(self, mask_a=None, mask_b=None, all_pairs=False, causal=False):
        self.a = mask_a.contiguous() if mask_a is not None else None
        self.b = mask_b.contiguous() if mask_b is not None else None
        self.all_pairs = int(all_pairs)
        self.causal = bool(causal)
        for m in (self.a, self.b):
            if m is not None and m.dtype != torch.int64:
                raise RuntimeError("univl_b200: masks must be int64 (as the reference dataloaders emit them)")

    @property
    def Wa(self):
        return self.a.shape[1] if self.a is not None else 0

    @property
    def Fb(self):
        return self.b.shape[1] if self.b is not None else 0

    @property
    def Nb(self):
        return self.b.shape[0] if self.b is not None else 0


SHORT_ATTN_MAX_S = 256


def _attention_entry(kind, Sq, Sk):
    if Sq > SHORT_ATTN_MAX_S or Sk > SHORT_ATTN_MAX_S:
        return "univl_attention_long_" + kind
    return "univl_attention_" + kind


def attention_fwd(q, k, v, n_seq, Sq, Sk, mask, p=0.0, seed=0, stream=0):
    o = _empty((n_seq * Sq, HEADS * 64), BF16, q)
    lse = _empty((n_seq * HEADS * Sq,), F32, q)
    call(_attention_entry("fwd", Sq, Sk), q.data_ptr(), q.stride(0), k.data_ptr(), k.stride(0), v.data_ptr(),
         v.stride(0), o.data_ptr(), o.stride(0), lse.data_ptr(), ptr(mask.a), ptr(mask.b), mask.Wa, mask.Fb, mask.Nb,
         int(mask.all_pairs), n_seq, HEADS, Sq, Sk, int(mask.causal), 1.0 / math.sqrt(64.0), float(p), seed, stream)
    return o, lse


def fused_attention_supported(n_seq, S, H):
    if os.environ.get("UNIVL_FUSED_ATTN", "1") == "0":
        return False
    from . import lib
    return bool(lib.load().univl_fused_qkv_attention_supported(int(n_seq), HEADS, int(S), int(H)))


def fused_qkv_attention_fwd(x, wqkv, bqkv, n_seq, S, mask, p=0.0, seed=0, stream=0, save_qkv=True):
    T, H = x.shape
    _check2d(x, "fused attention x"); _check2d(wqkv, "fused attention wqkv")
    o = _empty((T, H), BF16, x)
    lse = _empty((n_seq * HEADS * S,), F32, x)
    qkv = _empty((T, 3 * H), BF16, x) if save_qkv else None
    call("univl_fused_qkv_attention_fwd", x.data_ptr(), x.stride(0), wqkv.data_ptr(), wqkv.stride(0), bqkv.data_ptr(),
         ptr(qkv), 3 * H, o.data_ptr(), o.stride(0), lse.data_ptr(), ptr(mask.a), ptr(mask.b), mask.Wa, mask.Fb,
         mask.Nb, int(mask.all_pairs), n_seq, HEADS, S, int(mask.causal), 1.0 / math.sqrt(64.0), float(p), seed, stream)
    return o, lse, qkv


def fused_attention_bwd(qkv, o, lse, d_o, dqkv, n_seq, S, mask, p=0.0, seed=0, stream=0, dbias=None):
    call("univl_fused_attention_bwd", qkv.data_ptr(), qkv.stride(0), o.data_ptr(), o.stride(0), lse.data_ptr(),
         d_o.data_ptr(), d_o.stride(0), dqkv.data_ptr(), dqkv.stride(0), ptr(dbias), ptr(mask.a), ptr(mask.b), mask.Wa,
         mask.Fb, mask.Nb, int(mask.all_pairs), n_seq, HEADS, S, int(mask.causal), 1.0 / math.sqrt(64.0), float(p), seed,
         stream)


def attention_bwd(q, k, v, o, lse, d_o, dq, dk, dv, n_seq, Sq, Sk, mask, p=0.0, seed=0, stream=0, dbias=None,
                  rng_layout=0):
    dbq, dbk, dbv = dbias if dbias is not None else (None, None, None)
    entry = _attention_entry("bwd", Sq, Sk)
    assert rng_layout == 0 or entry == "univl_attention_bwd", (rng_layout, Sq, Sk)
    call(entry, q.data_ptr(), q.stride(0), k.data_ptr(), k.stride(0), v.data_ptr(), v.stride(0),
         o.data_ptr(), o.stride(0), lse.data_ptr(), d_o.data_ptr(), d_o.stride(0), dq.data_ptr(), dq.stride(0),
         dk.data_ptr(), dk.stride(0), dv.data_ptr(), dv.stride(0), ptr(mask.a), ptr(mask.b), mask.Wa, mask.Fb,
         mask.Nb, int(mask.all_pairs), n_seq, HEADS, Sq, Sk, int(mask.causal), 1.0 / math.sqrt(64.0), float(p), seed,
         stream, int(rng_layout), ptr(dbq), ptr(dbk), ptr(dbv))


def attention_pair_fwd(qkv_a, qkv_b, Na, Nb, Sq, mask):
    H = HEADS * 64
    o = _empty((Na * Nb * Sq, H), BF16, qkv_a)
    call("univl_attention_pair_fwd", qkv_a.data_ptr(), qkv_a.stride(0), qkv_a[:, H:].data_ptr(), qkv_a.stride(0),
         qkv_a[:, 2 * H:].data_ptr(), qkv_a.stride(0), qkv_b.data_ptr(), qkv_b.stride(0), qkv_b[:, H:].data_ptr(),
         qkv_b.stride(0), qkv_b[:, 2 * H:].data_ptr(), qkv_b.stride(0), o.data_ptr(), o.stride(0), None, ptr(mask.a),
         ptr(mask.b), Na, mask.Wa, Nb, mask.Fb, HEADS, Sq, 1.0 / math.sqrt(64.0))
    return o


def embed_src_rows_eval(a, N, W, pos, type_w, gamma, beta, out):
    mean = _empty((N * W,), F32, a)
    rstd = _empty((N * W,), F32, a)
    call("univl_embed_src_fwd", a.data_ptr(), None, pos.data_ptr(), type_w.data_ptr(), gamma.data_ptr(),
         beta.data_ptr(), out.data_ptr(), mean.data_ptr(), rstd.data_ptr(), N, W, 0, 0, 0, a.shape[1], LN_EPS, 0.0,
         None, 0)
    return out


def pair_layer_eval(x, qkv_a, qkv_b, Na, Nb, S, mask, params, first_token):
    arena = rt.current()
    wa = dict(zip(ATT_KEYS, params[:10]))
    wf = dict(zip(FFN_KEYS, params[10:16]))
    drop = _Drop(0.0, 0.0, False)
    n_seq = Na * Nb
    ctx = attention_pair_fwd(qkv_a, qkv_b, Na, Nb, 1 if first_token else S, mask)
    xq = x.view(n_seq, S, -1)[:, 0].contiguous() if first_token else x
    ao = linear_fwd(ctx, arena.bf16(wa["o"]), wa["bo"])
    y, _, _ = layernorm_fwd(ao, xq, wa["gamma"], wa["beta"], 0.0, 1, drop.seed, drop.stream())
    return ffn_block_fwd(y, wf, drop)[0]


E4M3 = torch.float8_e4m3fn
FP8_EPI_BIAS, FP8_EPI_GELU = 0, 1


def quantize_e4m3_rows(x):
    _check2d(x, "quantize_e4m3_rows x")
    M, K = x.shape
    q = _empty((M, K), E4M3, x)
    s = _empty((K // 128, M), F32, x)
    call("univl_quantize_e4m3_rows", x.data_ptr(), x.stride(0), q.data_ptr(), q.stride(0), s.data_ptr(), M, K)
    return q, s


def quantize_e4m3_blocks(w, q=None, s=None):
    _check2d(w, "quantize_e4m3_blocks w")
    N, K = w.shape
    q = _empty((N, K), E4M3, w) if q is None else q
    s = _empty((N // 128, K // 128), F32, w) if s is None else s
    call("univl_quantize_e4m3_blocks", w.data_ptr(), w.stride(0), q.data_ptr(), q.stride(0), s.data_ptr(), N, K)
    return q, s


def gemm_fp8(a, a_scale, b, b_scale, bias, gelu=False):
    _check2d(a, "gemm_fp8 A"); _check2d(b, "gemm_fp8 B")
    M, K = a.shape
    N = b.shape[0]
    if gelu:
        out = _empty((M, N), E4M3, a)
        out_s = _empty((N // 128, M), F32, a)
    else:
        out = _empty((M, N), BF16, a)
        out_s = None
    call("univl_gemm_fp8", a.data_ptr(), a.stride(0), a_scale.data_ptr(), b.data_ptr(), b.stride(0),
         b_scale.data_ptr(), M, N, K, FP8_EPI_GELU if gelu else FP8_EPI_BIAS, bias.data_ptr(), out.data_ptr(),
         out.stride(0), ptr(out_s))
    return (out, out_s) if gelu else out


def fp8_layer_weights(params, names):
    wa = dict(zip(ATT_KEYS, params[:10]))
    wf = dict(zip(FFN_KEYS, params[10:16]))
    H = wa["q"].shape[1]

    def stacked(ws):
        q = _empty((len(ws) * H, H), E4M3, ws[0])
        s = _empty((len(ws) * H // 128, H // 128), F32, ws[0])
        for i, w in enumerate(ws):
            quantize_e4m3_blocks(w, q[i * H:(i + 1) * H], s[i * H // 128:(i + 1) * H // 128])
        return q, s

    make = {"qkv": lambda: stacked((wa["q"], wa["k"], wa["v"])), "kv": lambda: stacked((wa["k"], wa["v"])),
            "o": lambda: quantize_e4m3_blocks(wa["o"]), "w1": lambda: quantize_e4m3_blocks(wf["w1"]),
            "w2": lambda: quantize_e4m3_blocks(wf["w2"])}
    return {n: make[n]() for n in names}


def _fp8_layer_tail(ctx, x, params, qw):
    wa = dict(zip(ATT_KEYS, params[:10]))
    wf = dict(zip(FFN_KEYS, params[10:16]))
    drop = _Drop(0.0, 0.0, False)
    ao = gemm_fp8(*quantize_e4m3_rows(ctx), *qw["o"], wa["bo"])
    y, _, _ = layernorm_fwd(ao, x, wa["gamma"], wa["beta"], 0.0, 1, drop.seed, drop.stream())
    h, hs = gemm_fp8(*quantize_e4m3_rows(y), *qw["w1"], wf["b1"], gelu=True)
    fo = gemm_fp8(h, hs, *qw["w2"], wf["b2"])
    out, _, _ = layernorm_fwd(fo, y, wf["gamma"], wf["beta"], 0.0, 1, drop.seed, drop.stream())
    return out


def pair_layer_eval_fp8(x, qkv_a, qkv_b, Na, Nb, S, mask, params, qw):
    ctx = attention_pair_fwd(qkv_a, qkv_b, Na, Nb, S, mask)
    return _fp8_layer_tail(ctx, x, params, qw)


def encoder_layer_eval_fp8(x, n_seq, S, mask, params, qw):
    wa = dict(zip(ATT_KEYS, params[:10]))
    H = x.shape[1]
    qkv = gemm_fp8(*quantize_e4m3_rows(x), *qw["qkv"], rt.packed_bias(wa["bq"], wa["bk"], wa["bv"]))
    drop = _Drop(0.0, 0.0, False)
    ctx, _ = attention_fwd(qkv[:, :H], qkv[:, H:2 * H], qkv[:, 2 * H:], n_seq, S, S, mask, 0.0, drop.seed,
                           drop.stream())
    return _fp8_layer_tail(ctx, x, params, qw)


def cls_layer_eval_fp8(x, n_seq, S, mask, params, qw):
    arena = rt.current()
    wa = dict(zip(ATT_KEYS, params[:10]))
    wf = dict(zip(FFN_KEYS, params[10:16]))
    drop = _Drop(0.0, 0.0, False)
    H = x.shape[1]
    x0 = x.view(n_seq, S, H)[:, 0].contiguous()
    kv = gemm_fp8(*quantize_e4m3_rows(x), *qw["kv"], rt.packed_bias(wa["bk"], wa["bv"]))
    q = linear_fwd(x0, arena.bf16_qkv(wa["q"], wa["k"], wa["v"])[:H], wa["bq"])
    ctx, _ = attention_fwd(q, kv[:, :H], kv[:, H:], n_seq, 1, S, mask, 0.0, drop.seed, drop.stream())
    ao = linear_fwd(ctx, arena.bf16(wa["o"]), wa["bo"])
    y, _, _ = layernorm_fwd(ao, x0, wa["gamma"], wa["beta"], 0.0, 1, drop.seed, drop.stream())
    return ffn_block_fwd(y, wf, drop)[0]


class _Drop:

    def __init__(self, p_hidden, p_attn, training):
        arena = rt.current()
        self.ph = float(p_hidden) if training else 0.0
        self.pa = float(p_attn) if training else 0.0
        self.seed = arena.seed
        self.arena = arena
        self.epoch = arena.epoch_host

    def stream(self):
        return self.arena.next_stream()


def attn_block_fwd(xq, xkv, n_seq, Sq, Sk, mask, w, drop, need_bwd=True):
    arena = rt.current()
    H = xq.shape[1]
    self_attn = xkv is xq
    sv = {"self": self_attn, "fused": False}
    wqkv = arena.bf16_qkv(w["q"], w["k"], w["v"])
    ctx = None
    if self_attn and fused_attention_supported(n_seq, Sq, H):
        sa, sd = drop.stream(), drop.stream()
        ctx, lse, qkv = fused_qkv_attention_fwd(xq, wqkv, rt.packed_bias(w["bq"], w["bk"], w["bv"]), n_seq, Sq, mask,
                                                drop.pa, drop.seed, sa, save_qkv=need_bwd)
        sv["qkv"] = qkv
        sv["fused"] = True
    elif self_attn:
        qkv = linear_fwd(xq, wqkv, rt.packed_bias(w["bq"], w["bk"], w["bv"]))
        q, k, v = qkv[:, :H], qkv[:, H:2 * H], qkv[:, 2 * H:]
        sv["qkv"] = qkv
    else:
        q = linear_fwd(xq, wqkv[:H], w["bq"])
        kv = linear_fwd(xkv, wqkv[H:], rt.packed_bias(w["bk"], w["bv"]))
        k, v = kv[:, :H], kv[:, H:]
        sv["q"], sv["kv"] = q, kv
    if ctx is None:
        sa, sd = drop.stream(), drop.stream()
        ctx, lse = attention_fwd(q, k, v, n_seq, Sq, Sk, mask, drop.pa, drop.seed, sa)
    ao = linear_fwd(ctx, arena.bf16(w["o"]), w["bo"])
    y, mean, rstd = layernorm_fwd(ao, xq, w["gamma"], w["beta"], drop.ph, 1, drop.seed, sd)
    sv.update(xq=xq, xkv=xkv, ctx=ctx, lse=lse, ao=ao, mean=mean, rstd=rstd, sa=sa, sd=sd, n_seq=n_seq, Sq=Sq, Sk=Sk,
              mask=mask, pa=drop.pa, ph=drop.ph, seed=drop.seed, wqkv=wqkv, wo=arena.bf16(w["o"]),
              gamma=w["gamma"], w=w, sink=GradSink(), arena=arena, epoch=drop.epoch)
    return y, sv


def attn_block_bwd(dy, dy2, sv, need_dxkv=True):
    H = sv["xq"].shape[1]
    sv["arena"].check_epoch(sv["epoch"], max(sv["pa"], sv["ph"]))
    w, sink = sv["w"], sv["sink"]
    dgamma, r_gamma = sink.one(w["gamma"])
    dbeta, r_beta = sink.one(w["beta"])
    dbo, r_bo = sink.one(w["bo"])
    g, gd, _, _, _ = layernorm_bwd(dy, dy2, sv["ao"], sv["xq"], sv["gamma"], sv["mean"], sv["rstd"], sv["ph"], 1,
                                   sv["seed"], sv["sd"], dgamma=dgamma, dbeta=dbeta, dbias=dbo)
    dwo, r_o = sink.one(w["o"])
    linear_wgrad(gd, sv["ctx"], dwo)
    dctx = linear_dgrad(gd, sv["wo"])
    T, Tk = sv["xq"].shape[0], sv["xkv"].shape[0]
    dwqkv, r_w = sink.packed((w["q"], w["k"], w["v"]))
    dbqkv, r_b = sink.packed((w["bq"], w["bk"], w["bv"]))
    if sv["self"]:
        qkv = sv["qkv"]
        dqkv = _empty((T, 3 * H), BF16, dy)
        if sv["fused"] and os.environ.get("UNIVL_FUSED_ATTN_BWD", "1") != "0":
            fused_attention_bwd(qkv, sv["ctx"], sv["lse"], dctx, dqkv, sv["n_seq"], sv["Sq"], sv["mask"], sv["pa"],
                                sv["seed"], sv["sa"], dbias=dbqkv)
        else:
            attention_bwd(qkv[:, :H], qkv[:, H:2 * H], qkv[:, 2 * H:], sv["ctx"], sv["lse"], dctx, dqkv[:, :H],
                          dqkv[:, H:2 * H], dqkv[:, 2 * H:], sv["n_seq"], sv["Sq"], sv["Sk"], sv["mask"], sv["pa"],
                          sv["seed"], sv["sa"], dbias=(dbqkv[:H], dbqkv[H:2 * H], dbqkv[2 * H:]),
                          rng_layout=1 if sv["fused"] else 0)
        linear_wgrad(dqkv, sv["xq"], dwqkv)
        dxq = linear_dgrad(dqkv, sv["wqkv"], epi=EPI_ADD, aux_in=g)
        dxkv = None
    else:
        q, kv = sv["q"], sv["kv"]
        dq = _empty((T, H), BF16, dy)
        dkv = _empty((Tk, 2 * H), BF16, dy)
        attention_bwd(q, kv[:, :H], kv[:, H:], sv["ctx"], sv["lse"], dctx, dq, dkv[:, :H], dkv[:, H:], sv["n_seq"],
                      sv["Sq"], sv["Sk"], sv["mask"], sv["pa"], sv["seed"], sv["sa"],
                      dbias=(dbqkv[:H], dbqkv[H:2 * H], dbqkv[2 * H:]))
        linear_wgrad(dq, sv["xq"], dwqkv[:H])
        linear_wgrad(dkv, sv["xkv"], dwqkv[H:])
        dxq = linear_dgrad(dq, sv["wqkv"][:H], epi=EPI_ADD, aux_in=g)
        dxkv = linear_dgrad(dkv, sv["wqkv"][H:]) if need_dxkv else None
    rets = {"q": r_w[0], "k": r_w[1], "v": r_w[2], "bq": r_b[0], "bk": r_b[1], "bv": r_b[2], "o": r_o, "bo": r_bo,
            "gamma": r_gamma, "beta": r_beta}
    return dxq, dxkv, rets


def ffn_block_fwd(x, w, drop):
    arena = rt.current()
    w1, w2 = arena.bf16(w["w1"]), arena.bf16(w["w2"])
    T = x.shape[0]
    pre = _empty((T, w1.shape[0]), BF16, x)
    h = linear_fwd(x, w1, w["b1"], epi=EPI_GELU, aux_out=pre)
    fo = linear_fwd(h, w2, w["b2"])
    sd = drop.stream()
    y, mean, rstd = layernorm_fwd(fo, x, w["gamma"], w["beta"], drop.ph, 1, drop.seed, sd)
    sv = dict(x=x, pre=pre, h=h, fo=fo, mean=mean, rstd=rstd, sd=sd, ph=drop.ph, seed=drop.seed, w1=w1, w2=w2,
              gamma=w["gamma"], w=w, sink=GradSink(), arena=arena, epoch=drop.epoch)
    return y, sv


def ffn_block_bwd(dy, sv):
    w, sink = sv["w"], sv["sink"]
    sv["arena"].check_epoch(sv["epoch"], sv["ph"])
    dgamma, r_gamma = sink.one(w["gamma"])
    dbeta, r_beta = sink.one(w["beta"])
    db2, r_b2 = sink.one(w["b2"])
    g, gd, _, _, _ = layernorm_bwd(dy, None, sv["fo"], sv["x"], sv["gamma"], sv["mean"], sv["rstd"], sv["ph"], 1,
                                   sv["seed"], sv["sd"], dgamma=dgamma, dbeta=dbeta, dbias=db2)
    dw2, r_w2 = sink.one(w["w2"])
    linear_wgrad(gd, sv["h"], dw2)
    dpre = linear_dgrad(gd, sv["w2"], epi=EPI_GELU_BWD, aux_in=sv["pre"])
    db1, r_b1 = sink.one(w["b1"])
    colsum(dpre, db1)
    dw1, r_w1 = sink.one(w["w1"])
    linear_wgrad(dpre, sv["x"], dw1)
    dx = linear_dgrad(dpre, sv["w1"])
    return g, dx, {"w1": r_w1, "b1": r_b1, "w2": r_w2, "b2": r_b2, "gamma": r_gamma, "beta": r_beta}


ATT_KEYS = ("q", "bq", "k", "bk", "v", "bv", "o", "bo", "gamma", "beta")
FFN_KEYS = ("w1", "b1", "w2", "b2", "gamma", "beta")


class EncoderLayerFn(torch.autograd.Function):

    @staticmethod
    def forward(ctx, x, n_seq, S, mask, p_hidden, p_attn, training, *params):
        wa = dict(zip(ATT_KEYS, params[:10]))
        wf = dict(zip(FFN_KEYS, params[10:16]))
        drop = _Drop(p_hidden, p_attn, training)
        y1, sva = attn_block_fwd(x, x, n_seq, S, S, mask, wa, drop, need_bwd=any(ctx.needs_input_grad))
        y2, svf = ffn_block_fwd(y1, wf, drop)
        ctx.sva, ctx.svf = sva, svf
        return y2

    @staticmethod
    def backward(ctx, dy):
        dy = dy.contiguous()
        g2, dy1, gf = ffn_block_bwd(dy, ctx.svf)
        dx, _, ga = attn_block_bwd(dy1, g2, ctx.sva)
        ctx.sva = ctx.svf = None
        return (dx, None, None, None, None, None, None) + tuple(ga[k] for k in ATT_KEYS) + \
            tuple(gf[k] for k in FFN_KEYS)


class EncoderLayerClsFn(torch.autograd.Function):

    @staticmethod
    def forward(ctx, x, n_seq, S, mask, p_hidden, p_attn, training, *params):
        wa = dict(zip(ATT_KEYS, params[:10]))
        wf = dict(zip(FFN_KEYS, params[10:16]))
        drop = _Drop(p_hidden, p_attn, training)
        H = x.shape[1]
        xq = x.view(n_seq, S, H)[:, 0].contiguous()
        y1, sva = attn_block_fwd(xq, x, n_seq, 1, S, mask, wa, drop)
        y2, svf = ffn_block_fwd(y1, wf, drop)
        ctx.sva, ctx.svf = sva, svf
        ctx.shape = (n_seq, S, H)
        return y2

    @staticmethod
    def backward(ctx, dy):
        dy = dy.contiguous()
        n_seq, S, H = ctx.shape
        g2, dy1, gf = ffn_block_bwd(dy, ctx.svf)
        dxq, dxkv, ga = attn_block_bwd(dy1, g2, ctx.sva)
        dxkv.view(n_seq, S, H)[:, 0].add_(dxq)
        ctx.sva = ctx.svf = None
        return (dxkv, None, None, None, None, None, None) + tuple(ga[k] for k in ATT_KEYS) + \
            tuple(gf[k] for k in FFN_KEYS)


class DecoderLayerFn(torch.autograd.Function):

    @staticmethod
    def forward(ctx, x, enc, n_seq, L, Se, slf_mask, enc_mask, p_hidden, p_attn, training, *params):
        ws = dict(zip(ATT_KEYS, params[:10]))
        we = dict(zip(ATT_KEYS, params[10:20]))
        wf = dict(zip(FFN_KEYS, params[20:26]))
        drop = _Drop(p_hidden, p_attn, training)
        s, svs = attn_block_fwd(x, x, n_seq, L, L, slf_mask, ws, drop, need_bwd=any(ctx.needs_input_grad))
        d, sve = attn_block_fwd(s, enc, n_seq, L, Se, enc_mask, we, drop)
        y, svf = ffn_block_fwd(d, wf, drop)
        ctx.svs, ctx.sve, ctx.svf = svs, sve, svf
        ctx.need_enc = enc.requires_grad
        return y

    @staticmethod
    def backward(ctx, dy):
        dy = dy.contiguous()
        g3, dd, gf = ffn_block_bwd(dy, ctx.svf)
        ds, denc, ge = attn_block_bwd(dd, g3, ctx.sve, need_dxkv=ctx.need_enc)
        dx, _, gs = attn_block_bwd(ds, None, ctx.svs)
        ctx.svs = ctx.sve = ctx.svf = None
        return (dx, denc) + (None,) * 8 + tuple(gs[k] for k in ATT_KEYS) + tuple(ge[k] for k in ATT_KEYS) + \
            tuple(gf[k] for k in FFN_KEYS)


class VideoNormFn(torch.autograd.Function):

    @staticmethod
    def forward(ctx, video, gamma, beta):
        x = video.reshape(-1, video.shape[-1])
        rows, cols = x.shape
        y = _empty((rows, cols), BF16, x)
        mean = _empty((rows,), F32, x)
        rstd = _empty((rows,), F32, x)
        call("univl_layernorm_f32_fwd", x.data_ptr(), gamma.data_ptr(), beta.data_ptr(), y.data_ptr(),
             mean.data_ptr(), rstd.data_ptr(), rows, cols, LN_EPS)
        ctx.save_for_backward(x, gamma, beta, mean, rstd)
        ctx.sink = GradSink()
        return y.view(video.shape)

    @staticmethod
    def backward(ctx, dy):
        x, gamma, beta, mean, rstd = ctx.saved_tensors
        dy = dy.contiguous().view(x.shape)
        dgamma, r_g = ctx.sink.one(gamma)
        dbeta, r_b = ctx.sink.one(beta)
        call("univl_layernorm_f32_bwd", dy.data_ptr(), x.data_ptr(), gamma.data_ptr(), mean.data_ptr(),
             rstd.data_ptr(), dgamma.data_ptr(), dbeta.data_ptr(), x.shape[0], x.shape[1])
        return None, r_g, r_b


class EmbedTextFn(torch.autograd.Function):

    @staticmethod
    def forward(ctx, ids, type_ids, word, pos, type_w, gamma, beta, p, training):
        n_seq, S = ids.shape
        H = word.shape[1]
        arena = rt.current()
        p = float(p) if training else 0.0
        stream = arena.next_stream()
        ids = ids.contiguous()
        type_ids = type_ids.contiguous() if type_ids is not None else None
        y = _empty((n_seq * S, H), BF16, word)
        mean = _empty((n_seq * S,), F32, word)
        rstd = _empty((n_seq * S,), F32, word)
        call("univl_embed_text_fwd", ids.data_ptr(), ptr(type_ids), word.data_ptr(), pos.data_ptr(), ptr(type_w),
             gamma.data_ptr(), beta.data_ptr(), y.data_ptr(), mean.data_ptr(), rstd.data_ptr(), n_seq, S, H,
             word.shape[0], LN_EPS, p, arena.seed, stream)
        ctx.save_for_backward(ids, type_ids, word, pos, type_w, gamma, beta, mean, rstd)
        ctx.cfg = (n_seq, S, H, p, arena.seed, stream)
        ctx.sink = GradSink()
        return y

    @staticmethod
    def backward(ctx, dy):
        ids, type_ids, word, pos, type_w, gamma, beta, mean, rstd = ctx.saved_tensors
        n_seq, S, H, p, seed, stream = ctx.cfg
        dy = dy.contiguous()
        dword, r_word = ctx.sink.one(word)
        dpos, r_pos = ctx.sink.one(pos)
        dtype, r_type = ctx.sink.one(type_w)
        dgamma, r_g = ctx.sink.one(gamma)
        dbeta, r_b = ctx.sink.one(beta)
        call("univl_embed_text_bwd", dy.data_ptr(), ids.data_ptr(), ptr(type_ids), word.data_ptr(), pos.data_ptr(),
             ptr(type_w), gamma.data_ptr(), mean.data_ptr(), rstd.data_ptr(), dword.data_ptr(), dpos.data_ptr(),
             ptr(dtype), dgamma.data_ptr(), dbeta.data_ptr(), n_seq, S, H, word.shape[0], p, seed, stream)
        return None, None, r_word, r_pos, r_type, r_g, r_b, None, None


class EmbedSrcFn(torch.autograd.Function):

    @staticmethod
    def forward(ctx, a, b, Na, Wa, Nb, Fb, all_pairs, pos, type_w, gamma, beta, p, training):
        arena = rt.current()
        H = a.shape[1]
        p = float(p) if training else 0.0
        stream = arena.next_stream()
        all_pairs = int(all_pairs)
        n_seq = Na * Nb // all_pairs if (all_pairs and Fb > 0) else Na
        rows = n_seq * (Wa + Fb)
        y = _empty((rows, H), BF16, a)
        mean = _empty((rows,), F32, a)
        rstd = _empty((rows,), F32, a)
        call("univl_embed_src_fwd", a.data_ptr(), ptr(b), pos.data_ptr(), ptr(type_w), gamma.data_ptr(),
             beta.data_ptr(), y.data_ptr(), mean.data_ptr(), rstd.data_ptr(), Na, Wa, Nb, Fb, all_pairs, H,
             LN_EPS, p, arena.seed, stream)
        ctx.save_for_backward(a, b, pos, type_w, gamma, beta, mean, rstd)
        ctx.cfg = (Na, Wa, Nb, Fb, all_pairs, H, p, arena.seed, stream)
        ctx.sink = GradSink()
        return y

    @staticmethod
    def backward(ctx, dy):
        a, b, pos, type_w, gamma, beta, mean, rstd = ctx.saved_tensors
        Na, Wa, Nb, Fb, all_pairs, H, p, seed, stream = ctx.cfg
        dy = dy.contiguous()
        da = _empty(a.shape, BF16, a)
        db = _empty(b.shape, BF16, a) if b is not None else None
        dpos, r_pos = ctx.sink.one(pos)
        dtype, r_type = ctx.sink.one(type_w)
        dgamma, r_g = ctx.sink.one(gamma)
        dbeta, r_b = ctx.sink.one(beta)
        call("univl_embed_src_bwd", dy.data_ptr(), a.data_ptr(), ptr(b), pos.data_ptr(), ptr(type_w),
             gamma.data_ptr(), mean.data_ptr(), rstd.data_ptr(), da.data_ptr(), ptr(db), dpos.data_ptr(),
             ptr(dtype), dgamma.data_ptr(), dbeta.data_ptr(), Na, Wa, Nb, Fb, all_pairs, H, p, seed, stream)
        return da, db, None, None, None, None, None, r_pos, r_type, r_g, r_b, None, None


class LinearFn(torch.autograd.Function):

    @staticmethod
    def forward(ctx, x, weight, bias, gelu, needs_dx):
        arena = rt.current()
        w16 = arena.bf16(weight)
        T = x.shape[0]
        pre = None
        if gelu:
            pre = _empty((T, w16.shape[0]), BF16, x)
            y = linear_fwd(x, w16, bias, epi=EPI_GELU, aux_out=pre)
        else:
            y = linear_fwd(x, w16, bias)
        ctx.save_for_backward(x, w16, pre, weight, bias)
        ctx.needs_dx = needs_dx
        ctx.sink = GradSink()
        return y

    @staticmethod
    def backward(ctx, dy):
        x, w16, pre, weight, bias = ctx.saved_tensors
        dy = dy.contiguous()
        if pre is not None:
            dy = gelu_bwd(dy, pre)
        db, r_b = ctx.sink.one(bias)
        if db is not None:
            colsum(dy, db)
        dw, r_w = ctx.sink.one(weight)
        linear_wgrad(dy, x, dw)
        dx = linear_dgrad(dy, w16) if ctx.needs_dx else None
        return dx, r_w, r_b, None, None


class LinearTFn(torch.autograd.Function):

    @staticmethod
    def forward(ctx, x, weight, bias):
        w16 = rt.current().bf16(weight)
        T, K = x.shape
        N = w16.shape[1]
        y = _empty((T, N), BF16, x)
        gemm(x, w16, T, N, K, y, bias=bias, b_mn=True)
        ctx.save_for_backward(x, w16, weight, bias)
        ctx.sink = GradSink()
        return y

    @staticmethod
    def backward(ctx, dy):
        x, w16, weight, bias = ctx.saved_tensors
        dy = dy.contiguous()
        T, K = x.shape
        N = w16.shape[1]
        dx = _empty((T, K), BF16, x)
        gemm(dy, w16, T, K, N, dx)
        dw, r_w = ctx.sink.one(weight)
        gemm(x, dy, K, N, T, dw, epi=EPI_ATOMIC, a_mn=True, b_mn=True)
        db, r_b = ctx.sink.one(bias)
        colsum(dy, db)
        return dx, r_w, r_b


def gelu_bwd(dy, pre):
    out = _empty(dy.shape, BF16, dy)
    call("univl_gelu_bwd_bf16", dy.data_ptr(), pre.data_ptr(), out.data_ptr(), dy.numel())
    return out


class TanhFn(torch.autograd.Function):

    @staticmethod
    def forward(ctx, x):
        x = x.contiguous()
        y = _empty(x.shape, BF16, x)
        call("univl_tanh_fwd_bf16", x.data_ptr(), y.data_ptr(), x.numel())
        ctx.save_for_backward(y)
        return y

    @staticmethod
    def backward(ctx, dy):
        (y,) = ctx.saved_tensors
        out = _empty(y.shape, BF16, y)
        dy = dy.contiguous()
        call("univl_tanh_bwd_bf16", dy.data_ptr(), y.data_ptr(), out.data_ptr(), y.numel())
        return out


class LayerNormFn(torch.autograd.Function):

    @staticmethod
    def forward(ctx, x, gamma, beta):
        y, mean, rstd = layernorm_fwd(x, None, gamma, beta)
        ctx.save_for_backward(x, gamma, beta, mean, rstd)
        ctx.sink = GradSink()
        return y

    @staticmethod
    def backward(ctx, dy):
        x, gamma, beta, mean, rstd = ctx.saved_tensors
        dgamma, r_g = ctx.sink.one(gamma)
        dbeta, r_b = ctx.sink.one(beta)
        dx, _, _, _, _ = layernorm_bwd(dy.contiguous(), None, x, None, gamma, mean, rstd, want_dbias=False,
                                       dgamma=dgamma, dbeta=dbeta)
        return dx, r_g, r_b


def _ld_pad(n):
    return (n + LD_VOCAB_ALIGN - 1) // LD_VOCAB_ALIGN * LD_VOCAB_ALIGN


VOCAB_LOSS_MODES = ("logits", "fused")


def vocab_loss_mode():
    value = os.environ.get("UNIVL_VOCAB_LOSS", "logits")
    if value not in VOCAB_LOSS_MODES:
        raise ValueError("UNIVL_VOCAB_LOSS must be one of %s, got %r" % ("/".join(VOCAB_LOSS_MODES), value))
    return value


def vocab_xent_fwd(x, w16, bias, labels, groups):
    _check2d(x, "vocab_xent x"); _check2d(w16, "vocab_xent W")
    T, K = x.shape
    V = w16.shape[0]
    nbytes = lib.load().univl_vocab_xent_workspace(T, V)
    if nbytes < 0:
        raise RuntimeError("univl_vocab_xent_workspace failed: %s" % lib.load().univl_last_error_string().decode())
    ws = _empty((nbytes,), torch.uint8, x)
    lse = _empty((T,), F32, x)
    sc = _empty((2 * groups,), F32, x)
    loss = _empty((), F32, x)
    call("univl_vocab_xent_fwd", x.data_ptr(), x.stride(0), w16.data_ptr(), w16.stride(0), ptr(bias),
         labels.data_ptr(), lse.data_ptr(), sc.data_ptr(), loss.data_ptr(), ws.data_ptr(), ws.numel(), T, V, K, groups)
    return loss, lse, sc


def vocab_xent_bwd(x, w16, bias, labels, lse, sc, g, groups):
    T, K = x.shape
    V = w16.shape[0]
    ld = _ld_pad(V)
    dl = _empty((T, ld), BF16, x)
    call("univl_vocab_xent_bwd", x.data_ptr(), x.stride(0), w16.data_ptr(), w16.stride(0), ptr(bias),
         labels.data_ptr(), lse.data_ptr(), sc.data_ptr(), ptr(g), dl.data_ptr(), ld, T, V, K, groups)
    return dl


class ProjXentFn(torch.autograd.Function):

    @staticmethod
    def forward(ctx, x, W, bias, labels, pair_mask, target_mode, w_is_param, return_logits, groups):
        arena = rt.current()
        w16 = arena.bf16(W) if w_is_param else W
        T, K = x.shape
        fused = vocab_loss_mode() == "fused" and target_mode == 0 and pair_mask is None and not return_logits
        if fused:
            labels = labels.contiguous()
            loss, lse, sc = vocab_xent_fwd(x, w16, bias, labels, groups)
            ctx.save_for_backward(x, w16, None, labels, None, lse, sc, W if w_is_param else None, bias)
            ctx.cfg = (target_mode, w_is_param, bias is not None, groups, False)
            ctx.sink = GradSink()
            return loss
        windowed = target_mode == 1 and groups > 1
        if windowed and (w_is_param or w16.shape[0] != T or T % groups):
            raise ValueError("grouped NCE needs one frame row per scored row and T divisible by the %d groups" % groups)
        V = T // groups if windowed else w16.shape[0]
        ld = _ld_pad(V)
        logits = _empty((T, ld), F32, x)[:, :V]
        if windowed:
            for g in range(groups):
                rows = slice(g * V, (g + 1) * V)
                gemm(x[rows], w16[rows], V, V, K, logits[rows], epi=EPI_F32, bias=bias)
        else:
            gemm(x, w16, T, V, K, logits, epi=EPI_F32, bias=bias)
        labels = labels.contiguous()
        lse = _empty((T,), F32, x)
        sc = _empty((2 * groups,), F32, x)
        loss = _empty((), F32, x)
        call("univl_softmax_xent_fwd", logits.data_ptr(), logits.stride(0), labels.data_ptr(), ptr(pair_mask),
             lse.data_ptr(), sc.data_ptr(), loss.data_ptr(), T, V, target_mode, -1, groups)
        ctx.save_for_backward(x, w16, logits, labels, pair_mask, lse, sc, W if w_is_param else None, bias)
        ctx.cfg = (target_mode, w_is_param, bias is not None, groups, windowed)
        ctx.sink = GradSink()
        if return_logits:
            return loss, logits
        return loss

    @staticmethod
    def backward(ctx, g, *unused):
        x, w16, logits, labels, pair_mask, lse, sc, W, bias = ctx.saved_tensors
        target_mode, w_is_param, has_bias, groups, windowed = ctx.cfg
        T, K = x.shape
        g = g.contiguous().to(F32)
        if logits is None:
            V = w16.shape[0]
            dl = vocab_xent_bwd(x, w16, bias, labels, lse, sc, g, groups)
        else:
            V = logits.shape[1]
            ld = _ld_pad(V)
            dl = _empty((T, ld), BF16, x)
            call("univl_softmax_xent_bwd", logits.data_ptr(), logits.stride(0), labels.data_ptr(), ptr(pair_mask),
                 lse.data_ptr(), sc.data_ptr(), g.data_ptr(), dl.data_ptr(), ld, T, V, target_mode, -1, groups)
        dlv = dl[:, :V]
        dx = _empty((T, K), BF16, x)
        if windowed:
            dW = _empty((T, K), BF16, x)
            tmp = _zeros((T, K), F32, x)
            for gi in range(groups):
                rows = slice(gi * V, (gi + 1) * V)
                gemm(dlv[rows], w16[rows], V, K, V, dx[rows], b_mn=True)
                gemm(dl[rows], x[rows], V, K, V, tmp[rows], epi=EPI_ATOMIC, a_mn=True, b_mn=True)
            call("univl_cast_f32_to_bf16", tmp.data_ptr(), dW.data_ptr(), tmp.numel())
            db = None
            if has_bias:
                dbbuf, db = ctx.sink.one(bias)
                colsum(dlv, dbbuf)
            return dx, dW, db, None, None, None, None, None, None
        gemm(dlv, w16, T, K, V, dx, b_mn=True)
        if w_is_param:
            dWbuf, dW = ctx.sink.one(W)
            gemm(dl, x, V, K, T, dWbuf, epi=EPI_ATOMIC, a_mn=True, b_mn=True)
        else:
            dW = _empty((V, K), BF16, x)
            tmp = _zeros((V, K), F32, x)
            gemm(dl, x, V, K, T, tmp, epi=EPI_ATOMIC, a_mn=True, b_mn=True)
            call("univl_cast_f32_to_bf16", tmp.data_ptr(), dW.data_ptr(), tmp.numel())
        db = None
        if has_bias:
            dbbuf, db = ctx.sink.one(bias)
            colsum(dlv, dbbuf)
        return dx, dW, db, None, None, None, None, None, None


class MeanPoolFn(torch.autograd.Function):

    @staticmethod
    def forward(ctx, x, mask, N, S, skip_first, guard_zero, l2norm):
        H = x.shape[1]
        mask = mask.contiguous()
        out = _empty((N, H), F32, x)
        norm = _empty((N,), F32, x)
        call("univl_meanpool_fwd", x.data_ptr(), mask.data_ptr(), out.data_ptr(), norm.data_ptr(), N, S, H,
             int(skip_first), int(guard_zero), int(l2norm))
        ctx.save_for_backward(out, norm, mask)
        ctx.cfg = (N, S, H, int(skip_first), int(guard_zero), int(l2norm))
        return out

    @staticmethod
    def backward(ctx, dy):
        out, norm, mask = ctx.saved_tensors
        N, S, H, sf, gz, l2 = ctx.cfg
        dx = _empty((N * S, H), BF16, out)
        dy = dy.contiguous()
        call("univl_meanpool_bwd", dy.data_ptr(), out.data_ptr(), norm.data_ptr(), mask.data_ptr(), dx.data_ptr(), N,
             S, H, sf, gz, l2)
        return dx, None, None, None, None, None, None


class SimMatmulFn(torch.autograd.Function):

    @staticmethod
    def forward(ctx, t, v, groups):
        bt, bv = t.shape[0] // groups, v.shape[0] // groups
        sim = _empty((t.shape[0], v.shape[0]) if groups == 1 else (groups, bt, bv), F32, t)
        call("univl_sim_matmul_fwd", t.data_ptr(), v.data_ptr(), sim.data_ptr(), bt, bv, t.shape[1], groups)
        ctx.save_for_backward(t, v)
        ctx.groups = groups
        return sim

    @staticmethod
    def backward(ctx, ds):
        t, v = ctx.saved_tensors
        G = ctx.groups
        dt = _empty(t.shape, F32, t)
        dv = _empty(v.shape, F32, t)
        ds = ds.contiguous()
        call("univl_sim_matmul_bwd", ds.data_ptr(), t.data_ptr(), v.data_ptr(), dt.data_ptr(), dv.data_ptr(),
             t.shape[0] // G, v.shape[0] // G, t.shape[1], G)
        return dt, dv, None


class SimLossFn(torch.autograd.Function):

    @staticmethod
    def forward(ctx, sim, kind, args):
        sim = sim.contiguous()
        B = sim.shape[-1]
        G = sim.shape[0] if sim.dim() == 3 else 1
        loss = _empty((), F32, sim)
        dsim = _empty(sim.shape, F32, sim)
        if kind == "maxmargin":
            margin, n_pair, w_same, w_diff = args
            call("univl_maxmargin_loss", sim.data_ptr(), loss.data_ptr(), dsim.data_ptr(), B, float(margin), n_pair,
                 float(w_same), float(w_diff), G)
        elif kind == "crossen":
            call("univl_crossen_loss", sim.data_ptr(), loss.data_ptr(), dsim.data_ptr(), B, G)
        elif kind == "milnce":
            bs, n_pair = args
            if bs * n_pair != B:
                raise RuntimeError("MILNCELoss: sim matrix is %dx%d but batch_size*n_pair = %d" % (B, B, bs * n_pair))
            call("univl_milnce_loss", sim.data_ptr(), loss.data_ptr(), dsim.data_ptr(), bs, n_pair, G)
        else:
            raise ValueError(kind)
        ctx.save_for_backward(dsim)
        return loss

    @staticmethod
    def backward(ctx, g):
        (dsim,) = ctx.saved_tensors
        out = _empty(dsim.shape, F32, dsim)
        g = g.contiguous().to(F32)
        call("univl_scale_f32", out.data_ptr(), dsim.data_ptr(), dsim.numel(), g.data_ptr())
        return out, None, None


class PoolerSimFn(torch.autograd.Function):

    @staticmethod
    def forward(ctx, u, w, b):
        N, H = u.shape
        out = _empty((N,), F32, u)
        call("univl_pooler_sim_fwd", u.data_ptr(), w.data_ptr(), b.data_ptr(), out.data_ptr(), N, H)
        ctx.save_for_backward(u, w, b)
        ctx.sink = GradSink()
        return out

    @staticmethod
    def backward(ctx, dout):
        u, w, b = ctx.saved_tensors
        N, H = u.shape
        du = _empty((N, H), BF16, u)
        dw, r_w = ctx.sink.one(w)
        db, r_b = ctx.sink.one(b)
        dout = dout.contiguous()
        call("univl_pooler_sim_bwd", u.data_ptr(), w.data_ptr(), dout.data_ptr(), du.data_ptr(), dw.data_ptr(),
             db.data_ptr(), N, H)
        return du, r_w, r_b
```

Baseline: 1443.

## Compact padded token rows so encoder GEMMs and layernorms skip masked positions

New measurement: 1485 (median of 6 runs). 2.9% higher.

```diff
diff --git a/include/univl_b200.h b/include/univl_b200.h
--- a/include/univl_b200.h
+++ b/include/univl_b200.h
@@ -15,6 +15,10 @@
                     int M, int N, int Kc, void* out, long long ldo, int epilogue, const float* bias,
                     const void* aux_in, long long ld_aux_in, void* aux_out, long long ld_aux_out, float alpha,
                     int block_n, int split_k, void* stream);
+int univl_gemm_bf16_rows(const void* A, long long lda, int a_mn_major, const void* B, long long ldb, int b_mn_major,
+                         int M, int N, int Kc, void* out, long long ldo, int epilogue, const float* bias,
+                         const void* aux_in, long long ld_aux_in, void* aux_out, long long ld_aux_out, float alpha,
+                         int block_n, int split_k, const int* rows_dev, void* stream);
 int univl_gemm_plan(int M, int N, int Kc, int epilogue, int block_n, int split_k);
 
 int univl_quantize_e4m3_rows(const void* x, long long ldx, void* q, long long ldq, float* scale, int M, int K,
@@ -32,6 +36,15 @@
                         const float* mean, const float* rstd, void* dx_res, void* dx_dense, float* dgamma,
                         float* dbeta, float* dbias, int rows, int cols, float p_drop, int drop_mode,
                         const unsigned long long* rng_state, unsigned long long stream_id, void* stream);
+int univl_layernorm_fwd_rows(const void* x, const void* res, const float* gamma, const float* beta, void* y,
+                             float* mean, float* rstd, int rows, int cols, float eps, float p_drop, int drop_mode,
+                             const unsigned long long* rng_state, unsigned long long stream_id, const int* rows_dev,
+                             const int* row_map, void* stream);
+int univl_layernorm_bwd_rows(const void* dy, const void* dy2, const void* x, const void* res, const float* gamma,
+                             const float* mean, const float* rstd, void* dx_res, void* dx_dense, float* dgamma,
+                             float* dbeta, float* dbias, int rows, int cols, float p_drop, int drop_mode,
+                             const unsigned long long* rng_state, unsigned long long stream_id, const int* row_map,
+                             void* stream);
 int univl_layernorm_f32_fwd(const float* x, const float* gamma, const float* beta, void* y, float* mean, float* rstd,
                             int rows, int cols, float eps, void* stream);
 int univl_layernorm_f32_bwd(const void* dy, const float* x, const float* gamma, const float* mean, const float* rstd,
@@ -94,6 +107,13 @@
                               int n_seq, int heads, int S, int causal, float scale, float p_drop,
                               const unsigned long long* rng_state, unsigned long long stream_id, void* stream);
 
+int univl_row_map(const long long* mask_a, const long long* mask_b, int Wa, int Fb, int Na, int Nb, int all_pairs,
+                  int n_seq, int* seq_off, int* to_compact, int* to_dense, int* first, int* counts, void* stream);
+int univl_rows_gather_bf16(const void* src, long long ld_src, const int* map, void* dst, long long ld_dst, int n_rows,
+                           int cols, const int* rows_dev, void* stream);
+int univl_rows_add_bf16(void* dst, long long ld_dst, const int* map, const void* src, long long ld_src, int n_rows,
+                        int cols, void* stream);
+
 int univl_colsum_bf16(const void* x, long long ld, float* out, int rows, int cols, void* stream);
 int univl_cast_f32_to_bf16(const float* src, void* dst, long long n, void* stream);
 int univl_cast_bf16_to_f32(const void* src, float* dst, long long n, void* stream);
diff --git a/univl_b200/csrc/gemm_wgmma.cu b/univl_b200/csrc/gemm_wgmma.cu
--- a/univl_b200/csrc/gemm_wgmma.cu
+++ b/univl_b200/csrc/gemm_wgmma.cu
@@ -35,12 +35,21 @@
   unsigned* arrived;
   int splits;
   int kb_seg;
+  const int* extent;
 };
 
 constexpr int BLOCK_M = 128;
 constexpr int BLOCK_K = 64;
 constexpr int PLAN_SMS = 132;
 constexpr int SPLIT_MIN_K = 4096;
+
+__device__ __forceinline__ void publish_extent(const GemmParams& p, int num_work, int n_tiles, volatile int* sh) {
+  if (threadIdx.x == 0) {
+    if (p.extent != nullptr) num_work = min(num_work, ((*p.extent + BLOCK_M - 1) / BLOCK_M) * n_tiles);
+    *sh = num_work;
+  }
+  __syncthreads();
+}
 
 template <int BLOCK_N, int STAGES>
 struct GemmSmem {
@@ -430,7 +439,8 @@
 template <int BLOCK_N, int STAGES, bool A_MN, bool B_MN>
 __global__ void __launch_bounds__(PIPELINE_THREADS, 1)
 gemm_wgmma_kernel(const __grid_constant__ CUtensorMap tmap_a, const __grid_constant__ CUtensorMap tmap_b,
-                  const GemmParams p, const int num_work) {
+                  const GemmParams p, const int planned_work) {
+  __shared__ int work_sh;
   using L = GemmSmem<BLOCK_N, STAGES>;
   constexpr bool PING = BLOCK_N <= 128;
   constexpr bool FOLD = BLOCK_N == 64;
@@ -442,18 +452,20 @@
   const int n_tiles = (p.N + BLOCK_N - 1) / BLOCK_N;
   const int total_kb = (p.Kc + BLOCK_K - 1) / BLOCK_K;
   const int kb_per = p.k_blocks_per_split;
+  volatile int* num_work = &work_sh;
+  publish_extent(p, planned_work, n_tiles, num_work);
 
   if (wg == 0) {
     if (producer_regs())
-      produce_ring<BLOCK_N, STAGES, A_MN, B_MN>(&tmap_a, &tmap_b, smem, ring, num_work, m_tiles, n_tiles, total_kb,
-                                                kb_per);
+      produce_ring<BLOCK_N, STAGES, A_MN, B_MN>(&tmap_a, &tmap_b, smem, ring, *num_work, m_tiles, n_tiles,
+                                                total_kb, kb_per);
   } else if constexpr (!PING) {
     consumer_regs();
     const int c = wg - 1;
     const int t = threadIdx.x & 127;
     const int warp = t >> 5, lane = t & 31;
     uint32_t it = 0;
-    for (int w = blockIdx.x; w < num_work; w += gridDim.x) {
+    for (int w = blockIdx.x; w < *num_work; w += gridDim.x) {
       const WorkItem wi = decode_work(w, m_tiles, n_tiles, total_kb, kb_per, BLOCK_N);
       float acc[BLOCK_N / 2];
 #pragma unroll
@@ -472,7 +484,7 @@
     const int warp = t >> 5, lane = t & 31;
     uint32_t it = 0;
     int j = 0;
-    for (int w = blockIdx.x; w < num_work; w += gridDim.x, ++j) {
+    for (int w = blockIdx.x; w < *num_work; w += gridDim.x, ++j) {
       const WorkItem wi = decode_work(w, m_tiles, n_tiles, total_kb, kb_per, BLOCK_N);
       if ((j & 1) != c) {
         it += wi.num_kb;
@@ -493,7 +505,7 @@
         const int i1 = min(wi.num_kb, i0 + seg);
         const int last =
             mma_kblocks<BLOCK_N, 2, A_MN, B_MN, L::STAGE_BYTES, L::A_BYTES>(ring, smem, 0, acc, i0, i1, it, t == 0);
-        if (i1 == wi.num_kb && w + (int)gridDim.x < num_work)
+        if (i1 == wi.num_kb && w + (int)gridDim.x < *num_work)
           named_bar_arrive(TURN_BAR + (c ^ 1), 256);
         mma_drain(ring, last, acc, t == 0);
         if constexpr (FOLD) {
@@ -997,6 +1009,7 @@
   p.arrived = nullptr;
   p.splits = 1;
   p.kb_seg = kb_per;
+  p.extent = nullptr;
   return p;
 }
 }
@@ -1007,10 +1020,11 @@
   return 1;
 }
 
-extern "C" int univl_gemm_bf16(const void* A, long long lda, int a_mn_major, const void* B, long long ldb,
-                               int b_mn_major, int M, int N, int Kc, void* out, long long ldo, int epilogue,
-                               const float* bias, const void* aux_in, long long ld_aux_in, void* aux_out,
-                               long long ld_aux_out, float alpha, int block_n, int split_k, void* stream_) {
+extern "C" int univl_gemm_bf16_rows(const void* A, long long lda, int a_mn_major, const void* B, long long ldb,
+                                    int b_mn_major, int M, int N, int Kc, void* out, long long ldo, int epilogue,
+                                    const float* bias, const void* aux_in, long long ld_aux_in, void* aux_out,
+                                    long long ld_aux_out, float alpha, int block_n, int split_k, const int* rows_dev,
+                                    void* stream_) {
   cudaStream_t stream = reinterpret_cast<cudaStream_t>(stream_);
   UNIVL_CHECK_ARG(M > 0 && N > 0 && Kc > 0, "gemm: empty problem M=%d N=%d K=%d", M, N, Kc);
   UNIVL_CHECK_ARG(A && B && out, "gemm: null operand");
@@ -1041,6 +1055,11 @@
                              ld_aux_out);
   p.splits = plan.splits;
   p.kb_seg = plan.kb_seg;
+  if (rows_dev != nullptr) {
+    UNIVL_CHECK_ARG(plan.splits == 1 && plan.kb_per >= (Kc + BLOCK_K - 1) / BLOCK_K,
+                    "gemm: a row extent needs an unsplit launch");
+    p.extent = rows_dev;
+  }
   if (plan.splits > 1) {
     const long long tiles = (long long)((M + BLOCK_M - 1) / BLOCK_M) * ((N + bn - 1) / bn);
     const size_t slot_bytes = (size_t)tiles * plan.splits * BLOCK_M * bn * sizeof(float);
@@ -1060,6 +1079,14 @@
   else rc = dispatch_major<64, 8>(amn, bmn, ta, tb, p, plan.splits, stream);
   if (p.slots != nullptr) cudaFreeAsync(p.slots, stream);
   return rc;
+}
+
+extern "C" int univl_gemm_bf16(const void* A, long long lda, int a_mn_major, const void* B, long long ldb,
+                               int b_mn_major, int M, int N, int Kc, void* out, long long ldo, int epilogue,
+                               const float* bias, const void* aux_in, long long ld_aux_in, void* aux_out,
+                               long long ld_aux_out, float alpha, int block_n, int split_k, void* stream_) {
+  return univl_gemm_bf16_rows(A, lda, a_mn_major, B, ldb, b_mn_major, M, N, Kc, out, ldo, epilogue, bias, aux_in,
+                              ld_aux_in, aux_out, ld_aux_out, alpha, block_n, split_k, nullptr, stream_);
 }
 
 extern "C" int univl_gemm_fp8(const void* A, long long lda, const float* a_scale, const void* B, long long ldb,
diff --git a/univl_b200/csrc/layernorm.cu b/univl_b200/csrc/layernorm.cu
--- a/univl_b200/csrc/layernorm.cu
+++ b/univl_b200/csrc/layernorm.cu
@@ -77,9 +77,11 @@
 __global__ void __launch_bounds__(LN_WARPS * 32, NVEC <= 3 ? 3 : 2)
 layernorm_fwd_kernel(const TIn* __restrict__ x, const bf16* __restrict__ res, const float* __restrict__ gamma,
                      const float* __restrict__ beta, bf16* __restrict__ y, float* __restrict__ mean_out,
-                     float* __restrict__ rstd_out, int rows, float eps, DropCfg drop_in) {
+                     float* __restrict__ rstd_out, int rows, float eps, DropCfg drop_in,
+                     const int* __restrict__ rows_dev, const int* __restrict__ row_map) {
   pdl_trigger();
   pdl_wait();
+  if (rows_dev != nullptr) rows = min(rows, *rows_dev);
   const DropCfg drop = resolve_drop(drop_in);
   constexpr int cols = NVEC * 256;
   const int warp = threadIdx.x >> 5, lane = threadIdx.x & 31;
@@ -97,6 +99,7 @@
     }
   }
   for (; row < rows; row += stride) {
+    const long long drow = (drop.mode != 0 && row_map != nullptr) ? row_map[row] : row;
     float z[NVEC][8];
     float s = 0.f;
 #pragma unroll
@@ -104,7 +107,7 @@
       const int c = (i * 32 + lane) * 8;
       raw_unpack(nx[i], z[i]);
       if (drop.mode == 1) {
-        const uint32_t keep = keep8_mask(drop, (uint64_t)row * cols + c);
+        const uint32_t keep = keep8_mask(drop, (uint64_t)drow * cols + c);
 #pragma unroll
         for (int j = 0; j < 8; ++j) z[i][j] = ((keep >> j) & 1u) ? z[i][j] * drop.scale : 0.f;
       }
@@ -150,7 +153,7 @@
 #pragma unroll
       for (int j = 0; j < 8; ++j) o[j] = g[j] * ((z[i][j] - mean) * rstd) + b[j];
       if (drop.mode == 2) {
-        const uint32_t keep = keep8_mask(drop, (uint64_t)row * cols + c);
+        const uint32_t keep = keep8_mask(drop, (uint64_t)drow * cols + c);
 #pragma unroll
         for (int j = 0; j < 8; ++j) o[j] = ((keep >> j) & 1u) ? o[j] * drop.scale : 0.f;
       }
@@ -162,24 +165,24 @@
 template <typename TIn>
 static void launch_ln_fwd(int grid, cudaStream_t st, const TIn* x, const bf16* res, const float* gamma,
                           const float* beta, bf16* y, float* mean, float* rstd, int rows, int cols, float eps,
-                          DropCfg drop) {
+                          DropCfg drop, const int* rows_dev = nullptr, const int* row_map = nullptr) {
   const dim3 g(grid), b(LN_WARPS * 32);
   switch (cols >> 8) {
-    case 1: launch_kernel(layernorm_fwd_kernel<TIn, 1>, g, b, 0, st, x, res, gamma, beta, y, mean, rstd, rows, eps, drop); break;
-    case 2: launch_kernel(layernorm_fwd_kernel<TIn, 2>, g, b, 0, st, x, res, gamma, beta, y, mean, rstd, rows, eps, drop); break;
-    case 3: launch_kernel(layernorm_fwd_kernel<TIn, 3>, g, b, 0, st, x, res, gamma, beta, y, mean, rstd, rows, eps, drop); break;
-    default: launch_kernel(layernorm_fwd_kernel<TIn, 4>, g, b, 0, st, x, res, gamma, beta, y, mean, rstd, rows, eps, drop); break;
+    case 1: launch_kernel(layernorm_fwd_kernel<TIn, 1>, g, b, 0, st, x, res, gamma, beta, y, mean, rstd, rows, eps, drop, rows_dev, row_map); break;
+    case 2: launch_kernel(layernorm_fwd_kernel<TIn, 2>, g, b, 0, st, x, res, gamma, beta, y, mean, rstd, rows, eps, drop, rows_dev, row_map); break;
+    case 3: launch_kernel(layernorm_fwd_kernel<TIn, 3>, g, b, 0, st, x, res, gamma, beta, y, mean, rstd, rows, eps, drop, rows_dev, row_map); break;
+    default: launch_kernel(layernorm_fwd_kernel<TIn, 4>, g, b, 0, st, x, res, gamma, beta, y, mean, rstd, rows, eps, drop, rows_dev, row_map); break;
   }
 }
 
 
 template <typename TIn>
 __device__ __forceinline__ void ln_bwd_load(const bf16* dy, const bf16* dy2, const TIn* x, const bf16* res,
-                                            long long off, const DropCfg& drop, float (&z)[8], float (&d)[8],
-                                            uint32_t& keep) {
+                                            long long off, uint64_t drop_idx, const DropCfg& drop, float (&z)[8],
+                                            float (&d)[8], uint32_t& keep) {
   load8(x + off, z);
   keep = 0xffu;
-  if (drop.mode != 0) keep = keep8_mask(drop, (uint64_t)off);
+  if (drop.mode != 0) keep = keep8_mask(drop, drop_idx);
   if (drop.mode == 1) {
 #pragma unroll
     for (int j = 0; j < 8; ++j) z[j] = ((keep >> j) & 1u) ? z[j] * drop.scale : 0.f;
@@ -217,7 +220,7 @@
                      const bf16* __restrict__ res, const float* __restrict__ gamma, const float* __restrict__ mean_in,
                      const float* __restrict__ rstd_in, bf16* __restrict__ dx_res, bf16* __restrict__ dx_dense,
                      float* __restrict__ dgamma, float* __restrict__ dbeta, float* __restrict__ dbias, int rows,
-                     DropCfg drop_in) {
+                     DropCfg drop_in, const int* __restrict__ row_map) {
   pdl_trigger();
   pdl_wait();
   const DropCfg drop = resolve_drop(drop_in);
@@ -230,7 +233,10 @@
   for (int k = lane * 4; k < 3 * cols; k += 128) *reinterpret_cast<float4*>(my + k) = make_float4(0.f, 0.f, 0.f, 0.f);
   __syncwarp();
 
-  for (long long row = (long long)blockIdx.x * LNB_WARPS + warp; row < rows; row += (long long)gridDim.x * LNB_WARPS) {
+  for (long long drow = (long long)blockIdx.x * LNB_WARPS + warp; drow < rows;
+       drow += (long long)gridDim.x * LNB_WARPS) {
+    const long long row = row_map != nullptr ? row_map[drow] : drow;
+    if (row < 0) continue;
     const float mean = mean_in[row], rstd = rstd_in[row];
     const float nm = -mean * rstd;
     float xh[NVEC][8], g[NVEC][8];
@@ -240,7 +246,7 @@
     for (int i = 0; i < NVEC; ++i) {
       const int c = (i * 32 + lane) * 8;
       float d[8], gm[8], dh[8];
-      ln_bwd_load(dy, dy2, x, res, row * cols + c, drop, xh[i], d, keep[i]);
+      ln_bwd_load(dy, dy2, x, res, row * cols + c, (uint64_t)(drow * cols + c), drop, xh[i], d, keep[i]);
       load8(gamma + c, gm);
 #pragma unroll
       for (int j = 0; j < 8; ++j) {
@@ -289,7 +295,8 @@
 template <typename TIn>
 static int launch_ln_bwd(int grid, cudaStream_t st, const bf16* dy, const bf16* dy2, const TIn* x, const bf16* res,
                          const float* gamma, const float* mean, const float* rstd, bf16* dx_res, bf16* dx_dense,
-                         float* dgamma_out, float* dbeta_out, float* dbias_out, int rows, int cols, DropCfg drop) {
+                         float* dgamma_out, float* dbeta_out, float* dbias_out, int rows, int cols, DropCfg drop,
+                         const int* row_map = nullptr) {
   const size_t smem = (size_t)LNB_WARPS * 3 * cols * sizeof(float);
   float* outs[3] = {dgamma_out, dbeta_out, dbias_out};
   float* parts[3] = {nullptr, nullptr, nullptr};
@@ -298,10 +305,10 @@
       if (int rc = scratch_alloc((void**)&parts[w], (size_t)grid * cols * sizeof(float), st)) return rc;
   float *dgamma = parts[0], *dbeta = parts[1], *dbias = parts[2];
   switch (cols >> 8) {
-    case 1: launch_kernel(layernorm_bwd_kernel<TIn, 1>, dim3(grid), dim3(LNB_WARPS * 32), smem, st, dy, dy2, x, res, gamma, mean, rstd, dx_res, dx_dense, dgamma, dbeta, dbias, rows, drop); break;
-    case 2: launch_kernel(layernorm_bwd_kernel<TIn, 2>, dim3(grid), dim3(LNB_WARPS * 32), smem, st, dy, dy2, x, res, gamma, mean, rstd, dx_res, dx_dense, dgamma, dbeta, dbias, rows, drop); break;
-    case 3: launch_kernel(layernorm_bwd_kernel<TIn, 3>, dim3(grid), dim3(LNB_WARPS * 32), smem, st, dy, dy2, x, res, gamma, mean, rstd, dx_res, dx_dense, dgamma, dbeta, dbias, rows, drop); break;
-    default: launch_kernel(layernorm_bwd_kernel<TIn, 4>, dim3(grid), dim3(LNB_WARPS * 32), smem, st, dy, dy2, x, res, gamma, mean, rstd, dx_res, dx_dense, dgamma, dbeta, dbias, rows, drop); break;
+    case 1: launch_kernel(layernorm_bwd_kernel<TIn, 1>, dim3(grid), dim3(LNB_WARPS * 32), smem, st, dy, dy2, x, res, gamma, mean, rstd, dx_res, dx_dense, dgamma, dbeta, dbias, rows, drop, row_map); break;
+    case 2: launch_kernel(layernorm_bwd_kernel<TIn, 2>, dim3(grid), dim3(LNB_WARPS * 32), smem, st, dy, dy2, x, res, gamma, mean, rstd, dx_res, dx_dense, dgamma, dbeta, dbias, rows, drop, row_map); break;
+    case 3: launch_kernel(layernorm_bwd_kernel<TIn, 3>, dim3(grid), dim3(LNB_WARPS * 32), smem, st, dy, dy2, x, res, gamma, mean, rstd, dx_res, dx_dense, dgamma, dbeta, dbias, rows, drop, row_map); break;
+    default: launch_kernel(layernorm_bwd_kernel<TIn, 4>, dim3(grid), dim3(LNB_WARPS * 32), smem, st, dy, dy2, x, res, gamma, mean, rstd, dx_res, dx_dense, dgamma, dbeta, dbias, rows, drop, row_map); break;
   }
   UNIVL_CHECK_LAUNCH("layernorm_bwd");
   for (int w = 0; w < 3; ++w)
@@ -343,26 +350,34 @@
 
 using namespace univl;
 
-extern "C" int univl_layernorm_fwd(const void* x, const void* res, const float* gamma, const float* beta, void* y,
-                                   float* mean, float* rstd, int rows, int cols, float eps, float p_drop,
-                                   int drop_mode, const unsigned long long* rng_state,
-                                   unsigned long long stream_id, void* stream) {
+extern "C" int univl_layernorm_fwd_rows(const void* x, const void* res, const float* gamma, const float* beta, void* y,
+                                        float* mean, float* rstd, int rows, int cols, float eps, float p_drop,
+                                        int drop_mode, const unsigned long long* rng_state,
+                                        unsigned long long stream_id, const int* rows_dev, const int* row_map,
+                                        void* stream) {
   if (int rc = check_ln_shape("layernorm_fwd", rows, cols)) return rc;
   UNIVL_CHECK_ARG(x && gamma && beta && y, "layernorm_fwd: null pointer");
   UNIVL_CHECK_ARG(p_drop == 0.f || rng_state != nullptr, "layernorm_fwd: dropout needs rng_state");
   UNIVL_CHECK_ARG(p_drop >= 0.f && p_drop < 1.f && drop_mode >= 0 && drop_mode <= 2, "layernorm_fwd: bad dropout");
   if (rows == 0) return UNIVL_OK;
   launch_ln_fwd<bf16>(ln_grid(rows), (cudaStream_t)stream, (const bf16*)x, (const bf16*)res, gamma, beta, (bf16*)y, mean,
-                      rstd, rows, cols, eps, make_drop(drop_mode, p_drop, rng_state, stream_id));
+                      rstd, rows, cols, eps, make_drop(drop_mode, p_drop, rng_state, stream_id), rows_dev, row_map);
   UNIVL_CHECK_LAUNCH("layernorm_fwd");
   return UNIVL_OK;
 }
-
-extern "C" int univl_layernorm_bwd(const void* dy, const void* dy2, const void* x, const void* res,
-                                   const float* gamma, const float* mean, const float* rstd, void* dx_res,
-                                   void* dx_dense, float* dgamma, float* dbeta, float* dbias, int rows, int cols,
-                                   float p_drop, int drop_mode, const unsigned long long* rng_state,
+extern "C" int univl_layernorm_fwd(const void* x, const void* res, const float* gamma, const float* beta, void* y,
+                                   float* mean, float* rstd, int rows, int cols, float eps, float p_drop,
+                                   int drop_mode, const unsigned long long* rng_state,
                                    unsigned long long stream_id, void* stream) {
+  return univl_layernorm_fwd_rows(x, res, gamma, beta, y, mean, rstd, rows, cols, eps, p_drop, drop_mode, rng_state,
+                                  stream_id, nullptr, nullptr, stream);
+}
+
+extern "C" int univl_layernorm_bwd_rows(const void* dy, const void* dy2, const void* x, const void* res,
+                                        const float* gamma, const float* mean, const float* rstd, void* dx_res,
+                                        void* dx_dense, float* dgamma, float* dbeta, float* dbias, int rows, int cols,
+                                        float p_drop, int drop_mode, const unsigned long long* rng_state,
+                                        unsigned long long stream_id, const int* row_map, void* stream) {
   if (int rc = check_ln_shape("layernorm_bwd", rows, cols)) return rc;
   UNIVL_CHECK_ARG(dy && x && gamma && mean && rstd, "layernorm_bwd: null pointer");
   UNIVL_CHECK_ARG(p_drop == 0.f || rng_state != nullptr, "layernorm_bwd: dropout needs rng_state");
@@ -370,7 +385,15 @@
   if (rows == 0) return UNIVL_OK;
   return launch_ln_bwd<bf16>(lnb_grid(rows), (cudaStream_t)stream, (const bf16*)dy, (const bf16*)dy2, (const bf16*)x,
                              (const bf16*)res, gamma, mean, rstd, (bf16*)dx_res, (bf16*)dx_dense, dgamma, dbeta, dbias,
-                             rows, cols, make_drop(drop_mode, p_drop, rng_state, stream_id));
+                             rows, cols, make_drop(drop_mode, p_drop, rng_state, stream_id), row_map);
+}
+extern "C" int univl_layernorm_bwd(const void* dy, const void* dy2, const void* x, const void* res,
+                                   const float* gamma, const float* mean, const float* rstd, void* dx_res,
+                                   void* dx_dense, float* dgamma, float* dbeta, float* dbias, int rows, int cols,
+                                   float p_drop, int drop_mode, const unsigned long long* rng_state,
+                                   unsigned long long stream_id, void* stream) {
+  return univl_layernorm_bwd_rows(dy, dy2, x, res, gamma, mean, rstd, dx_res, dx_dense, dgamma, dbeta, dbias, rows,
+                                  cols, p_drop, drop_mode, rng_state, stream_id, nullptr, stream);
 }
 
 extern "C" int univl_layernorm_f32_fwd(const float* x, const float* gamma, const float* beta, void* y, float* mean,
diff --git a/univl_b200/csrc/rowmap.cu b/univl_b200/csrc/rowmap.cu
--- /dev/null
+++ b/univl_b200/csrc/rowmap.cu
@@ -0,0 +1,199 @@
+#include "common.cuh"
+
+namespace univl {
+
+__device__ __forceinline__ bool row_kept(const long long* mask_a, const long long* mask_b, int Wa, int Fb,
+                                         long long i, long long j, int s) {
+  if (s == 0) return true;
+  return (s < Wa ? mask_a[i * Wa + s] : mask_b[j * Fb + (s - Wa)]) != 0;
+}
+
+constexpr int ROWMAP_SCAN_THREADS = 1024;
+
+__global__ void __launch_bounds__(ROWMAP_SCAN_THREADS)
+row_map_scan_kernel(const long long* __restrict__ mask_a, const long long* __restrict__ mask_b, int Wa, int Fb, int Nb,
+                    int groups, int n_seq, int* __restrict__ seq_off, int* __restrict__ counts) {
+  pdl_trigger();
+  pdl_wait();
+  __shared__ int warp_tot[ROWMAP_SCAN_THREADS / 32];
+  __shared__ int running;
+  const int S = Wa + Fb;
+  const int lane = threadIdx.x & 31, warp = threadIdx.x >> 5;
+  if (threadIdx.x == 0) running = 0;
+  __syncthreads();
+  for (int base = 0; base < n_seq; base += ROWMAP_SCAN_THREADS) {
+    const int p = base + threadIdx.x;
+    int cnt = 0;
+    if (p < n_seq) {
+      long long i, j;
+      pair_sources(p, groups, n_seq, Nb, i, j);
+      for (int s = 0; s < S; ++s) cnt += row_kept(mask_a, mask_b, Wa, Fb, i, j, s) ? 1 : 0;
+    }
+    int incl = cnt;
+#pragma unroll
+    for (int d = 1; d < 32; d <<= 1) {
+      const int v = __shfl_up_sync(0xffffffffu, incl, d);
+      if (lane >= d) incl += v;
+    }
+    if (lane == 31) warp_tot[warp] = incl;
+    __syncthreads();
+    int before = running;
+    for (int w = 0; w < warp; ++w) before += warp_tot[w];
+    if (p < n_seq) seq_off[p] = before + incl - cnt;
+    __syncthreads();
+    if (threadIdx.x == ROWMAP_SCAN_THREADS - 1) running = before + incl;
+    __syncthreads();
+  }
+  if (threadIdx.x == 0) {
+    const int V = running;
+    const long long T = (long long)n_seq * S;
+    const long long Tc = ((long long)V + 127) / 128 * 128;
+    seq_off[n_seq] = V;
+    counts[0] = (int)(Tc < T ? Tc : T);
+    counts[1] = V;
+  }
+}
+
+__global__ void __launch_bounds__(256)
+row_map_fill_kernel(const long long* __restrict__ mask_a, const long long* __restrict__ mask_b, int Wa, int Fb, int Nb,
+                    int groups, int n_seq, const int* __restrict__ seq_off, const int* __restrict__ counts,
+                    int* __restrict__ to_compact, int* __restrict__ to_dense, int* __restrict__ first) {
+  pdl_trigger();
+  pdl_wait();
+  const int S = Wa + Fb;
+  const int lane = threadIdx.x & 31;
+  const int p = blockIdx.x * 8 + (threadIdx.x >> 5);
+  if (p >= n_seq) return;
+  const int V = counts[1];
+  const int fillers = counts[0] - V;
+  long long i, j;
+  pair_sources(p, groups, n_seq, Nb, i, j);
+  int kept_before = seq_off[p];
+  int pad_before = p * S - kept_before;
+  for (int s0 = 0; s0 < S; s0 += 32) {
+    const int s = s0 + lane;
+    const bool in = s < S;
+    const bool kept = in && row_kept(mask_a, mask_b, Wa, Fb, i, j, s);
+    const unsigned km = __ballot_sync(0xffffffffu, kept);
+    const unsigned pm = __ballot_sync(0xffffffffu, in && !kept);
+    const unsigned below = (1u << lane) - 1u;
+    if (in) {
+      int c;
+      if (kept) c = kept_before + __popc(km & below);
+      else {
+        const int f = pad_before + __popc(pm & below);
+        c = f < fillers ? V + f : -1;
+      }
+      const int d = p * S + s;
+      to_compact[d] = c;
+      if (c >= 0) to_dense[c] = d;
+      if (s == 0) first[p] = c;
+    }
+    kept_before += __popc(km);
+    pad_before += __popc(pm);
+  }
+}
+
+__global__ void __launch_bounds__(256)
+rows_gather_kernel(const bf16* __restrict__ src, long long ld_src, const int* __restrict__ map, bf16* __restrict__ dst,
+                   long long ld_dst, int n_rows, int vecs, const int* __restrict__ rows_dev) {
+  pdl_trigger();
+  pdl_wait();
+  if (rows_dev != nullptr) n_rows = min(n_rows, *rows_dev);
+  const int lane = threadIdx.x & 31;
+  const int stride = gridDim.x * 8;
+  for (int r = blockIdx.x * 8 + (threadIdx.x >> 5); r < n_rows; r += stride) {
+    const int m = map[r];
+    uint4* d = reinterpret_cast<uint4*>(dst + (long long)r * ld_dst);
+    if (m >= 0) {
+      const uint4* s = reinterpret_cast<const uint4*>(src + (long long)m * ld_src);
+      for (int v = lane; v < vecs; v += 32) d[v] = s[v];
+    } else {
+      for (int v = lane; v < vecs; v += 32) d[v] = make_uint4(0, 0, 0, 0);
+    }
+  }
+}
+
+__global__ void __launch_bounds__(256)
+rows_add_kernel(bf16* __restrict__ dst, long long ld_dst, const int* __restrict__ map, const bf16* __restrict__ src,
+                long long ld_src, int n_rows, int vecs) {
+  pdl_trigger();
+  pdl_wait();
+  const int lane = threadIdx.x & 31;
+  const int stride = gridDim.x * 8;
+  for (int r = blockIdx.x * 8 + (threadIdx.x >> 5); r < n_rows; r += stride) {
+    const int m = map[r];
+    if (m < 0) continue;
+    uint4* d = reinterpret_cast<uint4*>(dst + (long long)m * ld_dst);
+    const uint4* s = reinterpret_cast<const uint4*>(src + (long long)r * ld_src);
+    for (int v = lane; v < vecs; v += 32) {
+      const uint4 a = d[v], b = s[v];
+      const uint32_t aw[4] = {a.x, a.y, a.z, a.w}, bw[4] = {b.x, b.y, b.z, b.w};
+      uint32_t o[4];
+#pragma unroll
+      for (int k = 0; k < 4; ++k) {
+        const float2 fa = unpack_bf16x2(aw[k]), fb = unpack_bf16x2(bw[k]);
+        o[k] = pack_bf16x2(__fadd_rn(fa.x, fb.x), __fadd_rn(fa.y, fb.y));
+      }
+      d[v] = make_uint4(o[0], o[1], o[2], o[3]);
+    }
+  }
+}
+
+static int row_grid(int n_rows) {
+  long long blocks = ((long long)n_rows + 7) / 8;
+  const long long cap = (long long)device_sms() * 8;
+  return (int)(blocks < 1 ? 1 : (blocks > cap ? cap : blocks));
+}
+
+static int check_rows(const char* what, const void* a, long long lda, const void* b, long long ldb, int cols) {
+  UNIVL_CHECK_ARG(cols > 0 && cols % 8 == 0 && lda % 8 == 0 && ldb % 8 == 0 && lda >= cols && ldb >= cols,
+                  "%s: rows must be whole 16-byte vectors (cols=%d ld=%lld, %lld)", what, cols, lda, ldb);
+  UNIVL_CHECK_ARG(((uintptr_t)a & 15) == 0 && ((uintptr_t)b & 15) == 0, "%s: 16-byte alignment", what);
+  return UNIVL_OK;
+}
+
+}
+
+using namespace univl;
+
+extern "C" int univl_row_map(const long long* mask_a, const long long* mask_b, int Wa, int Fb, int Na, int Nb,
+                             int all_pairs, int n_seq, int* seq_off, int* to_compact, int* to_dense, int* first,
+                             int* counts, void* stream_) {
+  cudaStream_t stream = reinterpret_cast<cudaStream_t>(stream_);
+  UNIVL_CHECK_ARG(mask_a && mask_b && seq_off && to_compact && to_dense && first && counts, "row_map: null pointer");
+  UNIVL_CHECK_ARG(Wa > 0 && Fb > 0 && Na > 0 && Nb > 0 && n_seq > 0, "row_map: empty problem");
+  UNIVL_CHECK_ARG(all_pairs >= 1 && Na % all_pairs == 0 && Nb % all_pairs == 0 &&
+                      (long long)n_seq * all_pairs == (long long)Na * Nb,
+                  "row_map: %d pairing groups over %d x %d rows do not give %d sequences", all_pairs, Na, Nb, n_seq);
+  UNIVL_CHECK_ARG((long long)n_seq * (Wa + Fb) <= 0x7fffffffLL, "row_map: too many rows");
+  launch_kernel(row_map_scan_kernel, dim3(1), dim3(ROWMAP_SCAN_THREADS), 0, stream, mask_a, mask_b, Wa, Fb, Nb,
+                all_pairs, n_seq, seq_off, counts);
+  UNIVL_CHECK_LAUNCH("row_map_scan");
+  launch_kernel(row_map_fill_kernel, dim3((n_seq + 7) / 8), dim3(256), 0, stream, mask_a, mask_b, Wa, Fb, Nb, all_pairs,
+                n_seq, (const int*)seq_off, (const int*)counts, to_compact, to_dense, first);
+  UNIVL_CHECK_LAUNCH("row_map_fill");
+  return UNIVL_OK;
+}
+
+extern "C" int univl_rows_gather_bf16(const void* src, long long ld_src, const int* map, void* dst, long long ld_dst,
+                                      int n_rows, int cols, const int* rows_dev, void* stream) {
+  UNIVL_CHECK_ARG(src && map && dst && n_rows >= 0, "rows_gather: bad arguments");
+  if (int rc = check_rows("rows_gather", src, ld_src, dst, ld_dst, cols)) return rc;
+  if (n_rows == 0) return UNIVL_OK;
+  launch_kernel(rows_gather_kernel, dim3(row_grid(n_rows)), dim3(256), 0, (cudaStream_t)stream, (const bf16*)src,
+                ld_src, map, (bf16*)dst, ld_dst, n_rows, cols / 8, rows_dev);
+  UNIVL_CHECK_LAUNCH("rows_gather_bf16");
+  return UNIVL_OK;
+}
+
+extern "C" int univl_rows_add_bf16(void* dst, long long ld_dst, const int* map, const void* src, long long ld_src,
+                                   int n_rows, int cols, void* stream) {
+  UNIVL_CHECK_ARG(src && map && dst && n_rows >= 0, "rows_add: bad arguments");
+  if (int rc = check_rows("rows_add", src, ld_src, dst, ld_dst, cols)) return rc;
+  if (n_rows == 0) return UNIVL_OK;
+  launch_kernel(rows_add_kernel, dim3(row_grid(n_rows)), dim3(256), 0, (cudaStream_t)stream, (bf16*)dst, ld_dst, map,
+                (const bf16*)src, ld_src, n_rows, cols / 8);
+  UNIVL_CHECK_LAUNCH("rows_add_bf16");
+  return UNIVL_OK;
+}
diff --git a/univl_b200/modules/transformer.py b/univl_b200/modules/transformer.py
--- a/univl_b200/modules/transformer.py
+++ b/univl_b200/modules/transformer.py
@@ -111,9 +111,19 @@
         return outs if keep_all else x2d
 
     def run_first_token(self, x2d, n_seq, S, mask, start=0):
-        for layer in self.layer[start:-1]:
+        last = self.layer[-1]
+        full = self.layer[start:-1]
+        if len(full) > 0 and mask.all_pairs >= 1 and mask.b is not None and ops.cross_compact_enabled():
+            rows = ops.RowMap(mask, n_seq, S)
+            for i, layer in enumerate(full):
+                x2d = ops.EncoderLayerCompactFn.apply(x2d, rows, i > 0, n_seq, S, mask, layer.attention.output.dropout.p,
+                                                      layer.attention.self.dropout.p, layer.training,
+                                                      *_layer_params(layer))
+            return ops.EncoderLayerClsCompactFn.apply(x2d, rows, n_seq, S, mask, last.attention.output.dropout.p,
+                                                      last.attention.self.dropout.p, last.training,
+                                                      *_layer_params(last))
+        for layer in full:
             x2d = layer.run(x2d, n_seq, S, mask)
-        last = self.layer[-1]
         return ops.EncoderLayerClsFn.apply(x2d, n_seq, S, mask, last.attention.output.dropout.p,
                                            last.attention.self.dropout.p, last.training, *_layer_params(last))
 
diff --git a/univl_b200/ops.py b/univl_b200/ops.py
--- a/univl_b200/ops.py
+++ b/univl_b200/ops.py
@@ -58,29 +58,30 @@
 
 
 def gemm(a, b, M, N, K, out, epi=EPI_BIAS, bias=None, aux_in=None, aux_out=None, a_mn=False, b_mn=False, alpha=1.0,
-         block_n=0, split_k=0):
+         block_n=0, split_k=0, rows=None):
     _check2d(a, "gemm A"); _check2d(b, "gemm B"); _check2d(out, "gemm out")
-    call("univl_gemm_bf16", a.data_ptr(), a.stride(0), int(a_mn), b.data_ptr(), b.stride(0), int(b_mn), M, N, K,
+    call("univl_gemm_bf16_rows", a.data_ptr(), a.stride(0), int(a_mn), b.data_ptr(), b.stride(0), int(b_mn), M, N, K,
          out.data_ptr(), out.stride(0), epi, ptr(bias), ptr(aux_in), aux_in.stride(0) if aux_in is not None else 0,
-         ptr(aux_out), aux_out.stride(0) if aux_out is not None else 0, float(alpha), block_n, split_k)
+         ptr(aux_out), aux_out.stride(0) if aux_out is not None else 0, float(alpha), block_n, split_k,
+         rows.counts.data_ptr() if rows is not None else None)
     return out
 
 
-def linear_fwd(x, w16, bias, epi=EPI_BIAS, aux_out=None, out_dtype=BF16, ld_out=None):
+def linear_fwd(x, w16, bias, epi=EPI_BIAS, aux_out=None, out_dtype=BF16, ld_out=None, rows=None):
     T, K = x.shape
     N = w16.shape[0]
     if ld_out is None:
         out = _empty((T, N), out_dtype, x)
     else:
         out = _empty((T, ld_out), out_dtype, x)[:, :N]
-    return gemm(x, w16, T, N, K, out, epi=epi, bias=bias, aux_out=aux_out)
-
-
-def linear_dgrad(dy, w16, epi=EPI_BIAS, aux_in=None):
+    return gemm(x, w16, T, N, K, out, epi=epi, bias=bias, aux_out=aux_out, rows=rows)
+
+
+def linear_dgrad(dy, w16, epi=EPI_BIAS, aux_in=None, rows=None):
     T, N = dy.shape
     K = w16.shape[1]
     out = _empty((T, K), BF16, dy)
-    return gemm(dy, w16, T, K, N, out, epi=epi, aux_in=aux_in, b_mn=True)
+    return gemm(dy, w16, T, K, N, out, epi=epi, aux_in=aux_in, b_mn=True, rows=rows)
 
 
 def linear_wgrad(dy, x, dw=None):
@@ -99,28 +100,29 @@
     return out
 
 
-def layernorm_fwd(x, res, gamma, beta, p=0.0, mode=0, seed=0, stream=0):
-    rows, cols = x.shape
-    y = _empty((rows, cols), BF16, x)
-    mean = _empty((rows,), F32, x)
-    rstd = _empty((rows,), F32, x)
-    call("univl_layernorm_fwd", x.data_ptr(), ptr(res), gamma.data_ptr(), beta.data_ptr(), y.data_ptr(),
-         mean.data_ptr(), rstd.data_ptr(), rows, cols, LN_EPS, float(p), mode, seed, stream)
+def layernorm_fwd(x, res, gamma, beta, p=0.0, mode=0, seed=0, stream=0, rows=None):
+    n, cols = x.shape
+    y = _empty((n, cols), BF16, x)
+    mean = _empty((n,), F32, x)
+    rstd = _empty((n,), F32, x)
+    call("univl_layernorm_fwd_rows", x.data_ptr(), ptr(res), gamma.data_ptr(), beta.data_ptr(), y.data_ptr(),
+         mean.data_ptr(), rstd.data_ptr(), n, cols, LN_EPS, float(p), mode, seed, stream,
+         rows.counts.data_ptr() if rows is not None else None, rows.to_dense.data_ptr() if rows is not None else None)
     return y, mean, rstd
 
 
 def layernorm_bwd(dy, dy2, x, res, gamma, mean, rstd, p=0.0, mode=0, seed=0, stream=0, want_dbias=True,
-                  want_dx=True, dgamma=None, dbeta=None, dbias=None):
-    rows, cols = x.shape
-    dx_res = _empty((rows, cols), BF16, x) if want_dx else None
-    dx_dense = _empty((rows, cols), BF16, x) if (want_dx and p > 0.0 and mode == 1) else dx_res
+                  want_dx=True, dgamma=None, dbeta=None, dbias=None, rows=None):
+    n, cols = x.shape
+    dx_res = _empty((n, cols), BF16, x) if want_dx else None
+    dx_dense = _empty((n, cols), BF16, x) if (want_dx and p > 0.0 and mode == 1) else dx_res
     dgamma = _zeros((cols,), F32, x) if dgamma is None else dgamma
     dbeta = _zeros((cols,), F32, x) if dbeta is None else dbeta
     if dbias is None and want_dbias:
         dbias = _zeros((cols,), F32, x)
-    call("univl_layernorm_bwd", dy.data_ptr(), ptr(dy2), x.data_ptr(), ptr(res), gamma.data_ptr(), mean.data_ptr(),
-         rstd.data_ptr(), ptr(dx_res), ptr(dx_dense), dgamma.data_ptr(), dbeta.data_ptr(), ptr(dbias), rows, cols,
-         float(p), mode, seed, stream)
+    call("univl_layernorm_bwd_rows", dy.data_ptr(), ptr(dy2), x.data_ptr(), ptr(res), gamma.data_ptr(),
+         mean.data_ptr(), rstd.data_ptr(), ptr(dx_res), ptr(dx_dense), dgamma.data_ptr(), dbeta.data_ptr(), ptr(dbias),
+         n, cols, float(p), mode, seed, stream, rows.to_compact.data_ptr() if rows is not None else None)
     return dx_res, dx_dense, dgamma, dbeta, dbias
 
 
@@ -146,6 +148,70 @@
     @property
     def Nb(self):
         return self.b.shape[0] if self.b is not None else 0
+
+
+def cross_compact_enabled():
+    return os.environ.get("UNIVL_CROSS_COMPACT", "1") != "0"
+
+
+class RowMap:
+
+    def __init__(self, mask, n_seq, S):
+        if mask.all_pairs < 1 or mask.a is None or mask.b is None or mask.Wa + mask.Fb != S:
+            raise RuntimeError("univl_b200: RowMap needs a pairing MaskSpec over Wa + Fb = S tokens")
+        dev = mask.a.device
+        self.T, self.n_seq, self.S = n_seq * S, n_seq, S
+        self.to_compact = torch.empty((self.T,), dtype=torch.int32, device=dev)
+        self.to_dense = torch.empty((self.T,), dtype=torch.int32, device=dev)
+        self.first = torch.empty((n_seq,), dtype=torch.int32, device=dev)
+        self.counts = torch.empty((2,), dtype=torch.int32, device=dev)
+        seq_off = torch.empty((n_seq + 1,), dtype=torch.int32, device=dev)
+        call("univl_row_map", mask.a.data_ptr(), mask.b.data_ptr(), mask.Wa, mask.Fb, mask.a.shape[0], mask.Nb,
+             mask.all_pairs, n_seq, seq_off.data_ptr(), self.to_compact.data_ptr(), self.to_dense.data_ptr(),
+             self.first.data_ptr(), self.counts.data_ptr())
+
+
+def row_map_host(mask_a, mask_b, groups):
+    import numpy as np
+    a = np.asarray(mask_a) != 0
+    b = np.asarray(mask_b) != 0
+    (Na, W), (Nb, F) = a.shape, b.shape
+    Gt, Gv = Na // groups, Nb // groups
+    kept = []
+    for g in range(groups):
+        for i in range(g * Gt, (g + 1) * Gt):
+            for j in range(g * Gv, (g + 1) * Gv):
+                kept.append(np.concatenate([a[i], b[j]]))
+    kept = np.stack(kept)
+    kept[:, 0] = True
+    n_seq, S = kept.shape
+    flat = kept.reshape(-1)
+    T, V = flat.size, int(flat.sum())
+    T_c = min(T, (V + 127) // 128 * 128)
+    to_dense = np.concatenate([np.flatnonzero(flat), np.flatnonzero(~flat)[:T_c - V]]).astype(np.int32)
+    to_compact = np.full(T, -1, dtype=np.int32)
+    to_compact[to_dense] = np.arange(T_c, dtype=np.int32)
+    return to_compact, to_dense, to_compact[::S].copy(), T_c, V
+
+
+def _gather_rows(src, index, n_out, rows_dev):
+    _check2d(src, "gather_rows src")
+    out = _empty((n_out, src.shape[1]), BF16, src)
+    call("univl_rows_gather_bf16", src.data_ptr(), src.stride(0), index.data_ptr(), out.data_ptr(), out.stride(0),
+         n_out, src.shape[1], ptr(rows_dev))
+    return out
+
+
+def to_compact_rows(x, rows):
+    return _gather_rows(x, rows.to_dense, rows.T, rows.counts)
+
+
+def to_dense_rows(x_c, rows):
+    return _gather_rows(x_c, rows.to_compact, rows.T, None)
+
+
+def first_token_rows(x_c, rows):
+    return _gather_rows(x_c, rows.first, rows.n_seq, None)
 
 
 SHORT_ATTN_MAX_S = 256
@@ -348,11 +414,12 @@
         return self.arena.next_stream()
 
 
-def attn_block_fwd(xq, xkv, n_seq, Sq, Sk, mask, w, drop, need_bwd=True):
+def attn_block_fwd(xq, xkv, n_seq, Sq, Sk, mask, w, drop, need_bwd=True, rows=None, res_c=None):
     arena = rt.current()
     H = xq.shape[1]
     self_attn = xkv is xq
-    sv = {"self": self_attn, "fused": False}
+    post = rows if self_attn else None
+    sv = {"self": self_attn, "fused": False, "rows": rows, "post": post}
     wqkv = arena.bf16_qkv(w["q"], w["k"], w["v"])
     ctx = None
     if self_attn and fused_attention_supported(n_seq, Sq, H):
@@ -367,15 +434,20 @@
         sv["qkv"] = qkv
     else:
         q = linear_fwd(xq, wqkv[:H], w["bq"])
-        kv = linear_fwd(xkv, wqkv[H:], rt.packed_bias(w["bk"], w["bv"]))
+        kv = linear_fwd(xkv, wqkv[H:], rt.packed_bias(w["bk"], w["bv"]), rows=rows)
+        if rows is not None:
+            kv = to_dense_rows(kv, rows)
         k, v = kv[:, :H], kv[:, H:]
         sv["q"], sv["kv"] = q, kv
     if ctx is None:
         sa, sd = drop.stream(), drop.stream()
         ctx, lse = attention_fwd(q, k, v, n_seq, Sq, Sk, mask, drop.pa, drop.seed, sa)
-    ao = linear_fwd(ctx, arena.bf16(w["o"]), w["bo"])
-    y, mean, rstd = layernorm_fwd(ao, xq, w["gamma"], w["beta"], drop.ph, 1, drop.seed, sd)
-    sv.update(xq=xq, xkv=xkv, ctx=ctx, lse=lse, ao=ao, mean=mean, rstd=rstd, sa=sa, sd=sd, n_seq=n_seq, Sq=Sq, Sk=Sk,
+    ctx_t = to_compact_rows(ctx, post) if post is not None else ctx
+    res = xq if post is None else (res_c if res_c is not None else to_compact_rows(xq, post))
+    ao = linear_fwd(ctx_t, arena.bf16(w["o"]), w["bo"], rows=post)
+    y, mean, rstd = layernorm_fwd(ao, res, w["gamma"], w["beta"], drop.ph, 1, drop.seed, sd, rows=post)
+    sv.update(xq=xq, xkv=xkv, ctx=ctx, res=res, lse=lse, ao=ao, mean=mean, rstd=rstd, sa=sa, sd=sd,
+              n_seq=n_seq, Sq=Sq, Sk=Sk,
               mask=mask, pa=drop.pa, ph=drop.ph, seed=drop.seed, wqkv=wqkv, wo=arena.bf16(w["o"]),
               gamma=w["gamma"], w=w, sink=GradSink(), arena=arena, epoch=drop.epoch)
     return y, sv
@@ -388,11 +460,16 @@
     dgamma, r_gamma = sink.one(w["gamma"])
     dbeta, r_beta = sink.one(w["beta"])
     dbo, r_bo = sink.one(w["bo"])
-    g, gd, _, _, _ = layernorm_bwd(dy, dy2, sv["ao"], sv["xq"], sv["gamma"], sv["mean"], sv["rstd"], sv["ph"], 1,
-                                   sv["seed"], sv["sd"], dgamma=dgamma, dbeta=dbeta, dbias=dbo)
+    rows, post = sv["rows"], sv["post"]
+    g, gd, _, _, _ = layernorm_bwd(dy, dy2, sv["ao"], sv["res"], sv["gamma"], sv["mean"], sv["rstd"], sv["ph"], 1,
+                                   sv["seed"], sv["sd"], dgamma=dgamma, dbeta=dbeta, dbias=dbo, rows=post)
     dwo, r_o = sink.one(w["o"])
+    dctx = linear_dgrad(gd, sv["wo"], rows=post)
+    if post is not None:
+        dctx = to_dense_rows(dctx, post)
+        g = to_dense_rows(g, post)
+        gd = to_dense_rows(gd, post)
     linear_wgrad(gd, sv["ctx"], dwo)
-    dctx = linear_dgrad(gd, sv["wo"])
     T, Tk = sv["xq"].shape[0], sv["xkv"].shape[0]
     dwqkv, r_w = sink.packed((w["q"], w["k"], w["v"]))
     dbqkv, r_b = sink.packed((w["bq"], w["bk"], w["bv"]))
@@ -418,24 +495,28 @@
                       sv["Sq"], sv["Sk"], sv["mask"], sv["pa"], sv["seed"], sv["sa"],
                       dbias=(dbqkv[:H], dbqkv[H:2 * H], dbqkv[2 * H:]))
         linear_wgrad(dq, sv["xq"], dwqkv[:H])
-        linear_wgrad(dkv, sv["xkv"], dwqkv[H:])
+        if rows is not None:
+            linear_wgrad(dkv, to_dense_rows(sv["xkv"], rows), dwqkv[H:])
+            dkv = to_compact_rows(dkv, rows)
+        else:
+            linear_wgrad(dkv, sv["xkv"], dwqkv[H:])
         dxq = linear_dgrad(dq, sv["wqkv"][:H], epi=EPI_ADD, aux_in=g)
-        dxkv = linear_dgrad(dkv, sv["wqkv"][H:]) if need_dxkv else None
+        dxkv = linear_dgrad(dkv, sv["wqkv"][H:], rows=rows) if need_dxkv else None
     rets = {"q": r_w[0], "k": r_w[1], "v": r_w[2], "bq": r_b[0], "bk": r_b[1], "bv": r_b[2], "o": r_o, "bo": r_bo,
             "gamma": r_gamma, "beta": r_beta}
     return dxq, dxkv, rets
 
 
-def ffn_block_fwd(x, w, drop):
+def ffn_block_fwd(x, w, drop, rows=None):
     arena = rt.current()
     w1, w2 = arena.bf16(w["w1"]), arena.bf16(w["w2"])
     T = x.shape[0]
     pre = _empty((T, w1.shape[0]), BF16, x)
-    h = linear_fwd(x, w1, w["b1"], epi=EPI_GELU, aux_out=pre)
-    fo = linear_fwd(h, w2, w["b2"])
+    h = linear_fwd(x, w1, w["b1"], epi=EPI_GELU, aux_out=pre, rows=rows)
+    fo = linear_fwd(h, w2, w["b2"], rows=rows)
     sd = drop.stream()
-    y, mean, rstd = layernorm_fwd(fo, x, w["gamma"], w["beta"], drop.ph, 1, drop.seed, sd)
-    sv = dict(x=x, pre=pre, h=h, fo=fo, mean=mean, rstd=rstd, sd=sd, ph=drop.ph, seed=drop.seed, w1=w1, w2=w2,
+    y, mean, rstd = layernorm_fwd(fo, x, w["gamma"], w["beta"], drop.ph, 1, drop.seed, sd, rows=rows)
+    sv = dict(rows=rows, x=x, pre=pre, h=h, fo=fo, mean=mean, rstd=rstd, sd=sd, ph=drop.ph, seed=drop.seed, w1=w1, w2=w2,
               gamma=w["gamma"], w=w, sink=GradSink(), arena=arena, epoch=drop.epoch)
     return y, sv
 
@@ -446,16 +527,20 @@
     dgamma, r_gamma = sink.one(w["gamma"])
     dbeta, r_beta = sink.one(w["beta"])
     db2, r_b2 = sink.one(w["b2"])
+    rows = sv["rows"]
     g, gd, _, _, _ = layernorm_bwd(dy, None, sv["fo"], sv["x"], sv["gamma"], sv["mean"], sv["rstd"], sv["ph"], 1,
-                                   sv["seed"], sv["sd"], dgamma=dgamma, dbeta=dbeta, dbias=db2)
+                                   sv["seed"], sv["sd"], dgamma=dgamma, dbeta=dbeta, dbias=db2, rows=rows)
+    dense = (lambda t: to_dense_rows(t, rows)) if rows is not None else (lambda t: t)
     dw2, r_w2 = sink.one(w["w2"])
-    linear_wgrad(gd, sv["h"], dw2)
-    dpre = linear_dgrad(gd, sv["w2"], epi=EPI_GELU_BWD, aux_in=sv["pre"])
+    linear_wgrad(dense(gd), dense(sv["h"]), dw2)
+    dpre = linear_dgrad(gd, sv["w2"], epi=EPI_GELU_BWD, aux_in=sv["pre"], rows=rows)
+    dpre_d = dense(dpre)
     db1, r_b1 = sink.one(w["b1"])
-    colsum(dpre, db1)
+    colsum(dpre_d, db1)
     dw1, r_w1 = sink.one(w["w1"])
-    linear_wgrad(dpre, sv["x"], dw1)
-    dx = linear_dgrad(dpre, sv["w1"])
+    linear_wgrad(dpre_d, dense(sv["x"]), dw1)
+    del dpre_d
+    dx = linear_dgrad(dpre, sv["w1"], rows=rows)
     return g, dx, {"w1": r_w1, "b1": r_b1, "w2": r_w2, "b2": r_b2, "gamma": r_gamma, "beta": r_beta}
 
 
@@ -510,6 +595,57 @@
         ctx.sva = ctx.svf = None
         return (dxkv, None, None, None, None, None, None) + tuple(ga[k] for k in ATT_KEYS) + \
             tuple(gf[k] for k in FFN_KEYS)
+
+
+class EncoderLayerCompactFn(torch.autograd.Function):
+
+    @staticmethod
+    def forward(ctx, x, rows, compact_in, n_seq, S, mask, p_hidden, p_attn, training, *params):
+        wa = dict(zip(ATT_KEYS, params[:10]))
+        wf = dict(zip(FFN_KEYS, params[10:16]))
+        drop = _Drop(p_hidden, p_attn, training)
+        xd = to_dense_rows(x, rows) if compact_in else x
+        y1_c, sva = attn_block_fwd(xd, xd, n_seq, S, S, mask, wa, drop, need_bwd=any(ctx.needs_input_grad), rows=rows,
+                                   res_c=x if compact_in else None)
+        y2_c, svf = ffn_block_fwd(y1_c, wf, drop, rows=rows)
+        ctx.sva, ctx.svf = sva, svf
+        ctx.rows_in = rows if compact_in else None
+        return y2_c
+
+    @staticmethod
+    def backward(ctx, dy_c):
+        dy_c = dy_c.contiguous()
+        g2_c, dy1_c, gf = ffn_block_bwd(dy_c, ctx.svf)
+        dx, _, ga = attn_block_bwd(dy1_c, g2_c, ctx.sva)
+        if ctx.rows_in is not None:
+            dx = to_compact_rows(dx, ctx.rows_in)
+        ctx.sva = ctx.svf = None
+        return (dx,) + (None,) * 8 + tuple(ga[k] for k in ATT_KEYS) + tuple(gf[k] for k in FFN_KEYS)
+
+
+class EncoderLayerClsCompactFn(torch.autograd.Function):
+
+    @staticmethod
+    def forward(ctx, x_c, rows, n_seq, S, mask, p_hidden, p_attn, training, *params):
+        wa = dict(zip(ATT_KEYS, params[:10]))
+        wf = dict(zip(FFN_KEYS, params[10:16]))
+        drop = _Drop(p_hidden, p_attn, training)
+        xq = first_token_rows(x_c, rows)
+        y1, sva = attn_block_fwd(xq, x_c, n_seq, 1, S, mask, wa, drop, rows=rows)
+        y2, svf = ffn_block_fwd(y1, wf, drop)
+        ctx.sva, ctx.svf, ctx.rows = sva, svf, rows
+        return y2
+
+    @staticmethod
+    def backward(ctx, dy):
+        dy = dy.contiguous()
+        rows = ctx.rows
+        g2, dy1, gf = ffn_block_bwd(dy, ctx.svf)
+        dxq, dxkv_c, ga = attn_block_bwd(dy1, g2, ctx.sva)
+        call("univl_rows_add_bf16", dxkv_c.data_ptr(), dxkv_c.stride(0), rows.first.data_ptr(), dxq.data_ptr(),
+             dxq.stride(0), rows.n_seq, dxq.shape[1])
+        ctx.sva = ctx.svf = None
+        return (dxkv_c,) + (None,) * 7 + tuple(ga[k] for k in ATT_KEYS) + tuple(gf[k] for k in FFN_KEYS)
 
 
 class DecoderLayerFn(torch.autograd.Function):
```
